# jayleicn/ClipBERT

Hardware: AMD Instinct MI355X
Metric: clips/sec/node (2×2 frames, 224px, L_txt=32) at 1/2/4/8 MI355X (higher is better)
Workload: dtype bf16; 1 GPU; MSRVTT retrieval training step (msrvtt_ret_base_resnet50.json; BASELINE configs[1]/[2] family) at the metric's shape: 16 videos x N_clip=2 x N_frame=2 uint8 frames 224px + 2 texts/video (pos+neg, r=2) L_txt=32 per GPU = 32 clips, 64 frames, 64 (text, clip) pairs per step; ImageNorm + fwd + lse-pooling loss + bwd + all-reduce + clip + AdamW in the timed step; clips folded into one forward; mode=train, videos_per_gpu=16, n_clips=2, n_frames=2, img_size=224, txt_len=32, texts_per_video=2, pairs_per_gpu=64, score_agg_func=lse, clips_folded=True, input=uint8 frames in HBM, parallelism=dp1, hip_graph=True, replay_plan=eager hyper-parameter upload + one hipGraph, n_graphs=1, dropout=True

## Files before the change

clipbert_amd/_lib.py:

```python
import ctypes as C
import os

HERE = os.path.dirname(os.path.abspath(__file__))
LIB_PATH = os.path.join(HERE, "lib", "libclipbert_hip.so")

CB_F32, CB_BF16 = 0, 1
ACT_NONE, ACT_RELU, ACT_GELU, ACT_TANH = 0, 1, 2, 3
SPLITK_WS_COUNTER_BYTES = 65536
ACT_GELU_SAVE_GRAD, ACT_SAVED_GRAD = 4, 5
ROWK, ROWK_GATHER, KROW, KROW_TAPS, KROW_GATHER = 0, 1, 2, 3, 4
(HP_LR, HP_BETA1, HP_BETA2, HP_EPS, HP_WD, HP_BC1, HP_BC2, HP_MAX_NORM, HP_GRAD_SCALE, HP_SKIP, HP_COUNT) = range(11)
OPT_ADAMW, OPT_ADAM, OPT_ADAMAX = 0, 1, 2

vp, i32, i64, f32, u64 = C.c_void_p, C.c_int32, C.c_int64, C.c_float, C.c_uint64


class GemmDesc(C.Structure):
    _fields_ = [
        ("dtype", i32), ("M", i32), ("N", i32), ("K", i32), ("a_mode", i32), ("b_mode", i32),
        ("A", vp), ("B", vp), ("lda", i64), ("ldb", i64), ("a_tab", vp), ("b_tab", vp),
        ("R", i32), ("S", i32), ("Cin", i32), ("H", i32), ("W", i32),
        ("sH", i64), ("sW", i64), ("flip_taps", i32), ("schedule", i32),
        ("C", vp), ("ldc", i64), ("c_rowmap", vp), ("c_f32", i32), ("accumulate", i32),
        ("split_k", i32), ("act", i32), ("scale", vp), ("shift", vp), ("residual", vp), ("ldr", i64),
        ("relu_after", i32), ("zero_fill_pitch", i32), ("mask", vp), ("ldm", i64), ("C2", vp), ("ldc2", i64),
        ("alpha", f32), ("dropout_p", f32), ("dropout_seed", u64), ("dropout_seed_ptr", vp), ("tile", i32),
        ("xcd_order", i32), ("a_bytes", i64), ("b_bytes", i64), ("gelu_grad_pre", vp), ("ld_gelu", i64), ("a_rowsum", vp),
        ("batch", i32), ("relu_bwd", i32), ("batch_stride_a", i64), ("batch_stride_b", i64), ("batch_stride_c", i64),
        ("batch_stride_rowsum", i64), ("post_scale", vp), ("post_scale2", vp), ("splitk_ws", vp), ("splitk_ws_bytes", i64),
        ("sq_slots", vp), ("sq_slots_n", i64),
    ]


class Res2Desc(C.Structure):
    _fields_ = [("x", vp), ("out", vp), ("w1", vp), ("w2", vp), ("w3", vp), ("wsc", vp),
                ("scale1", vp), ("shift1", vp), ("scale2", vp), ("shift2", vp), ("scale3", vp), ("shift3", vp),
                ("scale_sc", vp), ("shift_sc", vp), ("N", i32), ("H", i32), ("W", i32), ("cin", i32)]


_SIGNATURES = {
    "cb_gemm": [C.POINTER(GemmDesc), vp],
    "cb_res2_block": [C.POINTER(Res2Desc), vp],
    "cb_stem_pool": [vp, vp, vp, vp, vp, i32, i32, i32, i32, i32, i32, i32, vp],
    "cb_stem_pool_u8": [vp, vp, vp, vp, vp, vp, vp, i32, i32, i32, i32, i32, i32, i32, vp],
    "cb_gemm_plan": [vp, i32, vp],
    "cb_gemm_group": [vp, i32, vp],
    "cb_gemm_workspace_bytes": [vp, vp],
    "cb_build_pixel_table": [vp, i32, i32, i32, i32, i32, i64, i64, i64, vp],
    "cb_stem_pack": [i32, vp, i32, vp, vp, vp, i32, i32, i32, i32, i32, i32, vp],
    "cb_resize_pack_u8": [i32, vp, i64, vp, vp, i32, i32, vp, vp, vp, i32, i32, i32, i32, vp],
    "cb_image_norm": [vp, vp, vp, vp, i64, i64, vp],
    "cb_maxpool_fwd": [i32, vp, vp, i32, i32, i32, i32, i32, i32, i32, i32, i32, i32, vp],
    "cb_maxpool2_bwd": [i32, vp, vp, vp, vp, i32, i32, i32, i32, i32, i32, i32, vp],
    "cb_relu_scale_bwd": [i32, vp, vp, vp, vp, vp, vp, vp, i64, i32, vp],
    "cb_layernorm_fwd": [i32, vp, vp, vp, vp, vp, vp, i64, i32, f32, i32, i32, i32, vp],
    "cb_layernorm_bwd": [i32, vp, vp, vp, vp, vp, vp, vp, vp, i64, i32, vp, f32, u64, vp, i32, i32, i32, vp],
    "cb_layernorm_bwd_part": [i32, vp, vp, vp, vp, vp, vp, vp, i32, i64, i32, vp, f32, u64, vp, i32, i32, i32, vp],
    "cb_ln_partials_reduce": [vp, vp, vp, vp, i32, i32, i32, vp],
    "cb_comm_unique_id": [vp],
    "cb_comm_init": [i32, i32, vp],
    "cb_comm_info": [vp, vp],
    "cb_allreduce_bucket": [vp, i64, i32, vp],
    "cb_reduce_scatter_bucket": [vp, vp, i64, i32, vp],
    "cb_allgather_bucket": [vp, vp, i64, i32, vp],
    "cb_broadcast_bucket": [vp, i64, i32, i32, vp],
    "cb_comm_destroy": [],
    "cb_text_embed_fwd": [i32, vp, vp, vp, vp, vp, vp, vp, vp, vp, vp, i32, i32, i32, i32, f32, vp, vp, i32, vp],
    "cb_visual_embed_fwd": [i32, vp, vp, vp, vp, vp, vp, vp, vp, vp, vp, vp, vp, i32, i32, i32, i32, i32,
                            i32, i32, i32, f32, vp, vp],
    "cb_text_embed_bwd": [i32, vp, vp, vp, vp, vp, i32, i32, i32, i32, i64, i32, vp],
    "cb_head_loss": [i32, vp, vp, vp, vp, vp, i64, i32, f32, vp],
    "cb_retrieval_scores": [vp, vp, i64, i32, vp],
    "cb_sq_sum_fold": [vp, vp, i32, vp, i64, vp, vp, i32, vp],
    "cb_mean_fwd": [vp, i64, vp, vp],
    "cb_mean_bwd": [vp, i64, vp, vp],
    "cb_counter_add": [vp, i64, vp],
    "cb_zero": [vp, i64, vp],
    "cb_zero_ranges": [vp, vp, i32, vp],
    "cb_visual_embed_bwd": [i32, vp, vp, vp, vp, vp, vp, vp, i32, i32, i32, i32, i32, i32, i32, i32, vp],
    "cb_attention_fwd": [i32, vp, vp, vp, vp, i32, i32, i32, f32, u64, vp, vp],
    "cb_attention_bwd": [i32, vp, vp, vp, vp, vp, vp, vp, i32, i32, i32, f32, u64, vp, vp],
    "cb_cross_entropy": [vp, i64, vp, vp, vp, vp, i64, i32, i64, vp],
    "cb_colsum": [i32, vp, i64, vp, i64, i32, vp],
    "cb_cast": [i32, vp, i32, vp, i64, vp],
    "cb_act_bwd": [i32, i32, vp, vp, vp, i64, vp],
    "cb_adamw": [vp, vp, vp, vp, vp, i64, vp, vp, vp],
    "cb_dropout": [i32, vp, vp, i64, f32, u64, vp, vp],
    "cb_clip_aggregate_fwd": [vp, i32, i64, i32, vp, vp, vp],
    "cb_clip_aggregate_bwd": [vp, vp, vp, vp, i32, i64, i32, vp, vp],
    "cb_lse_loss": [vp, vp, i32, i32, i32, vp, vp, vp, vp],
    "cb_sq_sum": [vp, i64, vp, vp],
    "cb_sq_sum_det": [vp, i64, vp, vp, i32, vp],
    "cb_sq_sum_det_bf16": [vp, i64, vp, vp, i32, vp],
    "cb_adamw_g16": [vp, vp, vp, vp, vp, i64, vp, vp, vp],
    "cb_optim_step": [i32, i32, vp, vp, vp, vp, vp, i64, vp, vp, vp],
    "cb_elu_bn1d_fwd": [i32, vp, vp, vp, vp, vp, vp, vp, vp, i32, i32, i32, f32, f32, vp],
    "cb_elu_bn1d_bwd": [i32, vp, vp, vp, vp, vp, vp, vp, vp, i32, i32, i32, vp],
}

EXPORTED_SYMBOLS = tuple(_SIGNATURES) + ("cb_last_error", "cb_version")


def bind(cdll, strict: bool = True):
    for name, args in _SIGNATURES.items():
        if not strict and not hasattr(cdll, name):
            continue
        fn = getattr(cdll, name)
        fn.argtypes = args
        fn.restype = C.c_int
    cdll.cb_last_error.argtypes = []
    cdll.cb_last_error.restype = C.c_char_p
    cdll.cb_version.argtypes = []
    cdll.cb_version.restype = C.c_int
    return cdll


_LIB = None


def load(path: str = LIB_PATH):
    if not os.path.exists(path):
        raise RuntimeError(
            f"{path} not found: the HIP library is required (no fallback path exists). "
            "Build it with `python -m clipbert_amd.build`.")
    import torch
    return bind(C.CDLL(path))


# ... 13 lines not shown
```

clipbert_amd/csrc/common.hip:

```cpp
#include "common.h"

#include <stdarg.h>
#include <stdio.h>

namespace {
thread_local char g_err[512] = "";
}

int cb_fail(const char* fmt, ...) {
    va_list ap;
    va_start(ap, fmt);
    vsnprintf(g_err, sizeof(g_err), fmt, ap);
    va_end(ap);
    return -1;
}

int cb_launch_status(const char* what) {
    hipError_t e = hipGetLastError();
    if (e != hipSuccess) return cb_fail("%s: kernel launch failed: %s", what, hipGetErrorString(e));
    return 0;
}

extern "C" const char* cb_last_error(void) { return g_err; }
extern "C" int cb_version(void) { return 9; }
```

clipbert_amd/csrc/gemm.hip:

```cpp

#include "gemm8_impl.h"
#include "gemm_stream_impl.h"
#include <stdio.h>
#include <vector>

using namespace cbgemm;

namespace cbgemm {
extern template int launch_gemm<float, 64, 64, 2>(const GP&, bool, hipStream_t);
extern template int launch_gemm<bf16, 128, 128, 2>(const GP&, bool, hipStream_t);
extern template int launch_gemm<bf16, 128, 64, 2>(const GP&, bool, hipStream_t);
extern template int launch_gemm<bf16, 64, 64, 3>(const GP&, bool, hipStream_t);
extern template int launch_gemm<bf16, 128, 128, 1, 2>(const GP&, bool, hipStream_t);
extern template int launch_gemm_group<float, 64, 64, 2, 1>(const GroupArgs&, int, hipStream_t);
extern template int launch_gemm_group<bf16, 64, 64, 3, 1>(const GroupArgs&, int, hipStream_t);
extern template int launch_gemm_group<bf16, 128, 128, 1, 2>(const GroupArgs&, int, hipStream_t);
#define CB_G8_DECL(BM, BN, WGM, WGN, NST)                                                             \
    extern template int launch_gemm8_fwd<BM, BN, WGM, WGN, NST>(const GP&, int, float*, hipStream_t);   \
    extern template int launch_gemm8_dgrad<BM, BN, WGM, WGN, NST>(const GP&, int, float*, hipStream_t); \
    extern template int launch_gemm8_wgrad<BM, BN, WGM, WGN, NST>(const GP&, int, float*, hipStream_t);
CB_G8_DECL(256, 256, 2, 4, 2)
CB_G8_DECL(128, 256, 2, 4, 3)
CB_G8_DECL(256, 128, 4, 2, 3)
#undef CB_G8_DECL
int launch_gemm_skinny(const cb_gemm_desc* d, GP& p, hipStream_t st);
}

#include "gemm_choose.h"

#ifdef CB_STAMPS
#include <string>
namespace {
struct StampState {
    unsigned long long* buf = nullptr;
    int64_t areas = 0;
    std::vector<std::string> desc;
} g_stamps;
void stamp_assign(GP& p, const cb_gemm_desc* d, int tile, int split, int sched, int group_i, int group_n) {
    p.stamps = nullptr;
    if (!g_stamps.buf || (int64_t)g_stamps.desc.size() >= g_stamps.areas) return;
    p.stamps = g_stamps.buf + (int64_t)g_stamps.desc.size() * cbgemm::CB_STAMP_AREA;
    char line[512];
    snprintf(line, sizeof line,
             "{\"M\":%d,\"N\":%d,\"K\":%d,\"a_mode\":%d,\"b_mode\":%d,\"batch\":%d,\"tile\":%d,\"split\":%d,\"sched\":%d,\"taps\":%d,"
             "\"act\":%d,\"c2\":%d,\"residual\":%d,\"dropout\":%d,\"mask\":%d,\"gelu_grad\":%d,\"relu_bwd\":%d,\"c_f32\":%d,\"group_i\":%d,\"group_n\":%d}",
             d->M, d->N, d->K, d->a_mode, d->b_mode, d->batch > 1 ? d->batch : 1, tile, split, sched, (d->R > 0 ? d->R : 1) * (d->S > 0 ? d->S : 1), d->act,
             d->C2 != nullptr, d->residual != nullptr, d->dropout_p > 0.f, d->mask != nullptr, d->gelu_grad_pre != nullptr, d->relu_bwd != 0, d->c_f32, group_i, group_n);
    g_stamps.desc.push_back(line);
}
}
extern "C" int cb_debug_stamps_begin(void* buf, int64_t bytes) {
    g_stamps.buf = reinterpret_cast<unsigned long long*>(buf);
    g_stamps.areas = buf ? bytes / (8 * (int64_t)cbgemm::CB_STAMP_AREA) : 0;
    g_stamps.desc.clear();
    return 0;
}
extern "C" int64_t cb_debug_stamps_area_words() { return cbgemm::CB_STAMP_AREA; }
extern "C" int64_t cb_debug_stamps_count() { return (int64_t)g_stamps.desc.size(); }
extern "C" int cb_debug_stamps_desc(int64_t i, char* out, int64_t cap) {
    if (i < 0 || i >= (int64_t)g_stamps.desc.size() || cap <= 0) return -1;
    snprintf(out, (size_t)cap, "%s", g_stamps.desc[(size_t)i].c_str());
    return 0;
}
#define CB_STAMP_ASSIGN(p, d, tile, split, sched, gi, gn) stamp_assign(p, d, tile, split, sched, gi, gn)
#else
#define CB_STAMP_ASSIGN(p, d, tile, split, sched, gi, gn) do {} while (0)
#endif

namespace {

__global__ void __launch_bounds__(256) pixel_table_kernel(cb_pixel* tab, int total, int OH, int OW, int stride,
                                                          int pad, int64_t sN, int64_t sH, int64_t sW) {
    int m = blockIdx.x * 256 + threadIdx.x;
    if (m >= total) return;
    int ow = m % OW, t = m / OW;
    int oh = t % OH, n = t / OH;
    int ih0 = oh * stride - pad, iw0 = ow * stride - pad;
    cb_pixel px;
    px.off = (int32_t)((int64_t)n * sN + (int64_t)ih0 * sH + (int64_t)iw0 * sW);
    px.ih0 = (int16_t)ih0;
    px.iw0 = (int16_t)iw0;
    tab[m] = px;
}

__global__ void __launch_bounds__(256) splitk_reduce_kernel(GP p, const float* ws, int S) {
    using T = bf16;
    const int cpr = p.N >> 3;
    const int64_t total = (int64_t)p.M * cpr;
    const int64_t idx = (int64_t)blockIdx.x * 256 + threadIdx.x;
    if (p.batch > 1) {
        const int b = blockIdx.y;
        p.C = reinterpret_cast<unsigned char*>(p.C) + b * p.bs_c;
        ws += (int64_t)b * S * p.M * p.N;
    }
    if (idx >= total) return;
    if (p.dropout_p > 0.f && p.seed_ptr) p.seed += *p.seed_ptr;
    const int m = (int)(idx / cpr), n = (int)(idx - (int64_t)m * cpr) * 8;
    float v[8], t[8], sc[8], sh[8];
    const float* src = ws + (int64_t)m * p.N + n;
    load8(src, v);
    for (int s = 1; s < S; ++s) {
        load8(src + (int64_t)s * p.M * p.N, t);
#pragma unroll
        for (int r = 0; r < 8; ++r) v[r] += t[r];
    }
    if (p.scale) load8(p.scale + n, sc);
    if (p.shift) load8(p.shift + n, sh);
    const int64_t orow = p.c_rowmap ? (int64_t)p.c_rowmap[m] : (int64_t)m;
    epilogue8<T>(p, v, sc, sh, m, orow, n);
}

template <int BM, int BN, int WGM, int WGN, int NST>
int launch8(int form, const GP& p, int mode, float* ws, hipStream_t st) {
    if (form == 1) return launch_gemm8_fwd<BM, BN, WGM, WGN, NST>(p, mode, ws, st);
    if (form == 2) return launch_gemm8_dgrad<BM, BN, WGM, WGN, NST>(p, mode, ws, st);
    return launch_gemm8_wgrad<BM, BN, WGM, WGN, NST>(p, mode, ws, st);
}

int gemm_prepare(const cb_gemm_desc* d, Prepared& out) {
    CB_REQUIRE(d != nullptr, "cb_gemm: null descriptor");
    CB_REQUIRE(d->dtype == CB_F32 || d->dtype == CB_BF16, "cb_gemm: bad dtype %d", d->dtype);
    CB_REQUIRE(d->M >= 0 && d->N >= 0 && d->K >= 0, "cb_gemm: negative dims");
    CB_REQUIRE(d->A && d->B && d->C, "cb_gemm: null operand");
    const int esz = d->dtype == CB_BF16 ? 2 : 4;
    const int eps = 16 / esz;
    GP& p = out.p;
    p = GP{};
    p.A = d->A; p.B = d->B; p.C = d->C; p.C2 = d->C2; p.residual = d->residual; p.mask = d->mask;
    p.dact_pre = d->gelu_grad_pre; p.ldd = d->ld_gelu; p.a_rowsum = d->a_rowsum;
    p.relu_bwd = d->relu_bwd != 0; p.post_scale = d->post_scale; p.post_scale2 = d->post_scale2;
    if (p.relu_bwd) {
        CB_REQUIRE(d->mask && (!d->c_f32 || d->dtype == CB_F32) && !d->scale && !d->shift && d->act == CB_ACT_NONE && d->dropout_p <= 0.f && !d->relu_after &&
                   !d->gelu_grad_pre && (d->split_k <= 1),
                   "cb_gemm: relu_bwd needs a mask and excludes scale/shift/act/dropout/relu_after/gelu_grad_pre/split_k and an fp32 C next to bf16 operands");
        CB_REQUIRE((!d->post_scale || aligned16(d->post_scale)) && (!d->post_scale2 || aligned16(d->post_scale2)),
                   "cb_gemm: post_scale vectors must be 16-byte aligned");
    } else {
        CB_REQUIRE(!d->post_scale && !d->post_scale2, "cb_gemm: post_scale / post_scale2 need relu_bwd");
    }
    p.batch = d->batch > 1 ? d->batch : 1;
    p.bs_a = d->batch_stride_a * esz; p.bs_b = d->batch_stride_b * esz;
    p.bs_c = d->batch_stride_c * (d->c_f32 ? 4 : esz); p.bs_r = d->batch_stride_rowsum;
    if (p.batch > 1) {
        CB_REQUIRE(!d->C2 && !d->residual && !d->mask && !d->gelu_grad_pre && !d->a_tab && !d->b_tab && !d->c_rowmap,
                   "cb_gemm: batch > 1 supports plain operands only (no residual / mask / second output / gather / row map)");
        CB_REQUIRE((d->batch_stride_a * esz) % 16 == 0 && (d->batch_stride_b * esz) % 16 == 0 && (p.bs_c % 16) == 0,
                   "cb_gemm: batch strides must keep 16-byte alignment");
    }
    CB_REQUIRE(!d->a_rowsum || (d->a_mode == CB_KROW && d->b_mode == CB_KROW), "cb_gemm: a_rowsum needs the weight-gradient form (A and B both CB_KROW)");
    p.scale = d->scale; p.shift = d->shift; p.a_tab = d->a_tab; p.b_tab = d->b_tab; p.c_rowmap = d->c_rowmap; p.zfill = d->zero_fill_pitch;
    p.lda = d->lda; p.ldb = d->ldb; p.ldc = d->ldc; p.ldc2 = d->ldc2; p.ldr = d->ldr; p.ldm = d->ldm;
    p.sH = d->sH; p.sW = d->sW;
    p.M = d->M; p.N = d->N; p.K = d->K;
    p.a_mode = d->a_mode; p.b_mode = d->b_mode;
    p.R = d->R > 0 ? d->R : 1; p.S = d->S > 0 ? d->S : 1; p.Ct = d->Cin; p.H = d->H; p.W = d->W; p.flip = d->flip_taps;
    CB_REQUIRE(d->accumulate >= 0 && d->accumulate <= 2 && (d->accumulate != 2 || d->dtype == CB_BF16), "cb_gemm: bad accumulate %d (2 = first writer: bf16 problems)", d->accumulate);
    p.c_f32 = d->c_f32; p.accumulate = d->accumulate == 1; p.split_k = d->split_k > 0 ? d->split_k : 1;
    p.act = d->act; p.relu_after = d->relu_after;
    p.alpha = d->alpha == 0.f ? 1.f : d->alpha;
    p.dropout_p = d->dropout_p; p.seed = d->dropout_seed; p.seed_ptr = d->dropout_seed_ptr;
    const int bk = d->dtype == CB_BF16 ? Tr<bf16>::BK : Tr<float>::BK;
    p.ktiles = (d->K + bk - 1) / bk;
    {
        const bool ok = d->dtype == CB_BF16 && !d->c_f32 && (int64_t)d->M * (d->ldc > d->ldc2 ? d->ldc : d->ldc2) * 2 * (p.batch) < 0xffffffffll && !d->c_rowmap;
        p.wt = ok ? switches().wt : 0;
    }
    {
        const bool fe_off = switches().fast_epi_off;
        p.fast_epi = 0;
        auto rows_ok = [&](const void* q, int64_t ld) { return q == nullptr || (ld % 8 == 0 && aligned16(q) && (int64_t)d->M * ld * 2 < 0x7fffffffll); };
        const bool wg_store = !fe_off && d->dtype == CB_BF16 && d->c_f32 && d->a_mode == CB_KROW && d->accumulate != 1 && p.alpha == 1.f && !d->scale && !d->shift &&
                              d->act == CB_ACT_NONE && !d->C2 && !d->residual && !d->mask && !d->gelu_grad_pre && d->dropout_p <= 0.f && !d->relu_after && !d->c_rowmap &&
                              !d->zero_fill_pitch && !d->relu_bwd && d->N % 8 == 0 && d->ldc % 8 == 0 && aligned16(d->C) && (int64_t)d->M * d->ldc * 4 < 0xffffffffll;
        if (wg_store) p.fast_epi = FAST_EPI_F32;
        p.sq_slots = nullptr;
        if (d->sq_slots) {
            const int64_t need = (int64_t)((d->M + 63) / 64) * ((d->N + 63) / 64) * p.batch;
            CB_REQUIRE(wg_store, "cb_gemm: sq_slots needs a bf16 weight-gradient form storing an aligned fp32 C with a plain epilogue (accumulate 0 / 2)");
            CB_REQUIRE(d->sq_slots_n >= need, "cb_gemm: sq_slots_n %lld < %lld (one slot per 64x64 tile and batch member)", (long long)d->sq_slots_n, (long long)need);
            p.sq_slots = d->sq_slots;
        }
        const bool plain = !wg_store && !fe_off && p.wt == 1 && p.batch == 1 && d->accumulate != 1 && p.alpha == 1.f && !d->zero_fill_pitch && !d->a_rowsum &&
                           d->N % 8 == 0 && d->ldc % 8 == 0 && aligned16(d->C) && (!d->shift || aligned16(d->shift)) && (!d->scale || aligned16(d->scale)) &&
                           rows_ok(d->residual, d->ldr) && rows_ok(d->mask, d->ldm) && rows_ok(d->gelu_grad_pre, d->ld_gelu) &&
                           !(d->mask && d->gelu_grad_pre);
        if (plain && d->relu_bwd) {
            const bool ok = d->C2 && d->post_scale && d->ldc2 % 8 == 0 && aligned16(d->C2) && (int64_t)d->M * d->ldc2 * 2 < 0xffffffffll;
            const int flags = EF_RBWD | (d->residual ? EF_RES : 0) | (d->post_scale2 ? EF_PS2 : 0);
            if (ok)
                for (int i = 1; i < FAST_EPI_N; ++i)
                    if (FAST_EPI_COMBOS[i] == flags) { p.fast_epi = i; break; }
        } else if (plain) {
            int flags = 0;
            bool ok = true;
            if (d->scale) flags |= EF_SCALE;
            if (d->shift) flags |= EF_SHIFT;
            if (d->act == CB_ACT_RELU) flags |= EF_RELU;
            else if (d->act == CB_ACT_GELU_SAVE_GRAD && d->C2) flags |= EF_GELU2;
            else if (d->act == CB_ACT_GELU && !d->C2) flags |= EF_GELU1;
            else if (d->act == CB_ACT_SAVED_GRAD && d->gelu_grad_pre) flags |= EF_MULAUX;
            else if (d->act != CB_ACT_NONE) ok = false;
            if (d->C2 && !(flags & EF_GELU2)) ok = false;
            if (d->C2) ok = ok && d->ldc2 % 8 == 0 && aligned16(d->C2) && (int64_t)d->M * d->ldc2 * 2 < 0xffffffffll;
            if (d->gelu_grad_pre && !(flags & EF_MULAUX)) ok = false;
            if (d->dropout_p > 0.f) flags |= EF_DROP;
            if (d->residual) flags |= EF_RES;
            if (d->relu_after) flags |= EF_RELU_AFTER;
            if (d->mask) flags |= EF_MASK;
            if (ok)
                for (int i = 1; i < FAST_EPI_N; ++i)
                    if (FAST_EPI_COMBOS[i] == flags) { p.fast_epi = i; break; }
        }
    }
    const bool a_krow = d->a_mode == CB_KROW;
    const bool b_krow = d->b_mode == CB_KROW || d->b_mode == CB_KROW_TAPS || d->b_mode == CB_KROW_GATHER;
    CB_REQUIRE(d->a_mode == CB_ROWK || d->a_mode == CB_ROWK_GATHER || d->a_mode == CB_KROW, "cb_gemm: bad a_mode %d", d->a_mode);
    CB_REQUIRE(d->b_mode == CB_ROWK || b_krow, "cb_gemm: bad b_mode %d", d->b_mode);
    const int taps = p.R * p.S;
    const bool tapped = d->a_mode == CB_ROWK_GATHER || d->b_mode == CB_KROW_TAPS || d->b_mode == CB_KROW_GATHER;
    if (tapped) {
        CB_REQUIRE(p.Ct > 0, "cb_gemm: Cin (channels per tap) must be set for conv modes");
        CB_REQUIRE(p.Ct % eps == 0, "cb_gemm: channels per tap (%d) must be a multiple of %d", p.Ct, eps);
    }
    const int64_t lim = 0x7fffffffll;
    bool fast = d->a_bytes > 0 && d->b_bytes > 0 && d->a_bytes < lim && d->b_bytes < lim && aligned16(d->A) && aligned16(d->B);
    if (d->a_mode == CB_ROWK_GATHER) {
        CB_REQUIRE(d->a_tab, "cb_gemm: a_tab missing");
        CB_REQUIRE(d->K == taps * p.Ct, "cb_gemm: K (%d) != R*S*Cin (%d)", d->K, taps * p.Ct);
        fast = fast && (p.R == 1 || d->sH % eps == 0) && (p.S == 1 || d->sW % eps == 0);
    } else if (d->a_mode == CB_ROWK) {
        fast = fast && (d->lda % eps == 0) && (d->K % eps == 0);
    } else {
        const int64_t need = ((int64_t)(d->K - 1) * d->lda + (d->M + eps - 1) / eps * eps) * esz;
        fast = fast && (d->lda % eps == 0) && (d->M % eps == 0 || need <= d->a_bytes);
    }
    if (d->b_mode == CB_ROWK) {
        fast = fast && (d->ldb % eps == 0) && (d->K % eps == 0);
    } else if (d->b_mode == CB_KROW) {
        const int64_t need = ((int64_t)(d->K - 1) * d->ldb + (d->N + eps - 1) / eps * eps) * esz;
        fast = fast && (d->ldb % eps == 0) && (d->N % eps == 0 || need <= d->b_bytes);
    } else if (d->b_mode == CB_KROW_TAPS) {
        CB_REQUIRE(d->K == taps * p.Ct, "cb_gemm: K (%d) != R*S*Ct (%d)", d->K, taps * p.Ct);
        fast = fast && (d->ldb % eps == 0) && (d->N % eps == 0);
    } else {
        CB_REQUIRE(d->b_tab, "cb_gemm: b_tab missing");
        CB_REQUIRE(d->N == taps * p.Ct, "cb_gemm: N (%d) != R*S*Cin (%d)", d->N, taps * p.Ct);
        fast = fast && (p.R == 1 || d->sH % eps == 0) && (p.S == 1 || d->sW % eps == 0);
    }
    p.a_bytes = (uint32_t)(fast ? d->a_bytes : 0);
    p.b_bytes = (uint32_t)(fast ? d->b_bytes : 0);
    CB_REQUIRE(d->tile >= 0 && d->tile <= 9, "cb_gemm: bad tile %d", d->tile);
    CB_REQUIRE(d->xcd_order >= 0 && d->xcd_order <= 2, "cb_gemm: bad xcd_order %d", d->xcd_order);
    CB_REQUIRE(d->dropout_p >= 0.f && d->dropout_p < 1.f, "cb_gemm: dropout_p out of range");
    const int cesz = d->c_f32 ? 4 : esz;
    bool cv = (d->ldc % 4 == 0) && ((reinterpret_cast<uintptr_t>(d->C) % (4 * cesz)) == 0);
    if (d->C2) cv = cv && (d->ldc2 % 4 == 0) && ((reinterpret_cast<uintptr_t>(d->C2) % (4 * esz)) == 0);
    if (d->residual) cv = cv && (d->ldr % 4 == 0) && ((reinterpret_cast<uintptr_t>(d->residual) % (4 * esz)) == 0);
    if (d->mask) cv = cv && (d->ldm % 4 == 0) && ((reinterpret_cast<uintptr_t>(d->mask) % (4 * esz)) == 0);
    if (d->gelu_grad_pre) cv = cv && (d->ld_gelu % 4 == 0) && ((reinterpret_cast<uintptr_t>(d->gelu_grad_pre) % (4 * esz)) == 0);
    if (d->scale) cv = cv && aligned16(d->scale);
    if (d->shift) cv = cv && aligned16(d->shift);
    p.c_vec = cv;
    bool cv8 = cv && (d->N % 8 == 0) && (d->ldc % 8 == 0) && aligned16(d->C);
    if (d->C2) cv8 = cv8 && (d->ldc2 % 8 == 0) && aligned16(d->C2);
    if (d->residual) cv8 = cv8 && (d->ldr % 8 == 0) && aligned16(d->residual);
    if (d->mask) cv8 = cv8 && (d->ldm % 8 == 0) && aligned16(d->mask);
    if (d->gelu_grad_pre) cv8 = cv8 && (d->ld_gelu % 8 == 0) && aligned16(d->gelu_grad_pre);
    out.fast = fast; out.cv8 = cv8;
    out.form = operand_form(d->a_mode, d->b_mode, taps); out.taps = taps;
    out.epi_scale_only = !d->C2 && !d->residual && !d->mask && !d->gelu_grad_pre && d->act == CB_ACT_NONE && !d->relu_after && !d->shift && d->dropout_p <= 0.f;
    out.atomics_ok = out.epi_scale_only && d->c_f32 && d->accumulate == 1;
    return 0;
}

int gemm_validate(const cb_gemm_desc* d, Prepared& pr, bool& empty) {
    empty = false;
    CB_REQUIRE(d != nullptr, "cb_gemm: null descriptor");
    CB_REQUIRE(d->M >= 0 && d->N >= 0 && d->K >= 0, "cb_gemm: negative dims");
    empty = d->M == 0 || d->N == 0;
    return empty ? 0 : gemm_prepare(d, pr);
}

void trace_plan(const cb_gemm_desc* d, const Prepared& pr, const LaunchPlan& lp) {
    if (lp.tile == 9)
        fprintf(stderr, "cb_gemm: M=%d N=%d K=%d modes=%d/%d tile=9 (asked %d) few rows\n", d->M, d->N, d->K, d->a_mode, d->b_mode, d->tile);
    else if (lp.tile == 8)
        fprintf(stderr, "cb_gemm: M=%d N=%d K=%d modes=%d/%d tile=8 (asked %d) stream variant %d\n", d->M, d->N, d->K, d->a_mode, d->b_mode, d->tile, lp.sched);
    else
        fprintf(stderr, "cb_gemm: M=%d N=%d K=%d modes=%d/%d tile=%d (asked %d) form8=%d split=%d ws=%d\n", d->M, d->N, d->K, d->a_mode, d->b_mode,
                lp.picked, d->tile, lp.form8, lp.tile >= 5 ? lp.split_k : pr.p.split_k, (int)lp.slab);
}

int gemm_launch(const cb_gemm_desc* d, const Prepared& pr, const LaunchPlan& lp, hipStream_t st) {
    GP p = pr.p;
    if (lp.tile == 9) return launch_gemm_skinny(d, p, st);
    p.split_k = lp.split_k;
    p.c_vec8 = lp.c_vec8;
    p.xcd_remap = lp.xcd_remap;
    if (lp.tile == 8) return launch_gemm_stream(p, lp.sched, st);
    if (lp.tile >= 5) {
        float* ws = lp.slab ? reinterpret_cast<float*>(d->splitk_ws) : nullptr;
        CB_STAMP_ASSIGN(p, d, lp.tile, p.split_k, lp.sched, 0, 1);
        int rc;
        if (lp.tile == 5) rc = launch8<256, 256, 2, 4, 2>(lp.form8, p, lp.sched - 1, ws, st);
        else if (lp.tile == 6) rc = launch8<128, 256, 2, 4, 3>(lp.form8, p, lp.sched - 1, ws, st);
        else rc = launch8<256, 128, 4, 2, 3>(lp.form8, p, lp.sched - 1, ws, st);
        if (rc != 0 || !ws) return rc;
        GP q = p;
        q.split_k = 1;
        const int64_t chunks = (int64_t)d->M * (d->N / 8);
        hipLaunchKernelGGL(splitk_reduce_kernel, dim3((unsigned)((chunks + 255) / 256), (unsigned)p.batch), dim3(256), 0, st, q, ws, p.split_k);
        return cb_launch_status("cb_gemm (split-K reduce)");
    }
    if (d->dtype == CB_F32) return launch_gemm<float, 64, 64, 2>(p, pr.fast, st);
    CB_STAMP_ASSIGN(p, d, lp.tile, p.split_k, 0, 0, 1);
    if (lp.tile == 4) return launch_gemm<bf16, 128, 128, 1, 2>(p, pr.fast, st);
    if (lp.tile == 1) return launch_gemm<bf16, 128, 128, 2>(p, pr.fast, st);
    if (lp.tile == 3) return launch_gemm<bf16, 128, 64, 2>(p, pr.fast, st);
    return launch_gemm<bf16, 64, 64, 3>(p, pr.fast, st);
}

int gemm_run(const cb_gemm_desc* d, const Prepared& pr, void* stream) {
    LaunchPlan lp;
    const int rc = gemm_choose(d, pr, true, false, lp);
    if (lp.tile != 0 && switches().trace) trace_plan(d, pr, lp);
    return rc != 0 ? rc : gemm_launch(d, pr, lp, cb_stream(stream));
}
}

extern "C" int cb_gemm(const cb_gemm_desc* d, void* stream) {
    Prepared pr;
    bool empty;
    if (int rc = gemm_validate(d, pr, empty)) return rc;
    return empty ? 0 : gemm_run(d, pr, stream);
}

extern "C" int cb_gemm_plan(const cb_gemm_desc* d, int32_t use_table, int32_t* out4) {
    CB_REQUIRE(out4 != nullptr, "cb_gemm_plan: null output");
    out4[0] = out4[1] = out4[2] = out4[3] = 0;
    Prepared pr;
    LaunchPlan lp;
    bool empty;
    if (int rc = gemm_validate(d, pr, empty)) return rc;
    if (empty) return 0;
    if (int rc = gemm_choose(d, pr, use_table != 0, false, lp)) return rc;
    out4[0] = lp.tile; out4[1] = lp.split_k; out4[2] = lp.sched; out4[3] = lp.xcd_remap ? 1 : 2;
    return 0;
}

extern "C" int cb_gemm_workspace_bytes(const cb_gemm_desc* d, int64_t* bytes) {
    CB_REQUIRE(d != nullptr && bytes != nullptr, "cb_gemm_workspace_bytes: null argument");
    *bytes = 0;
    Prepared pr;
    LaunchPlan lp;
    bool empty;
    if (int rc = gemm_validate(d, pr, empty)) return rc;
    if (empty) return 0;
    if (int rc = gemm_choose(d, pr, true, true, lp)) return rc;
    if (lp.slab) *bytes = (int64_t)lp.split_k * pr.p.batch * d->M * d->N * 4 + CB_SPLITK_WS_COUNTER_BYTES;
    return 0;
}

namespace {
int group_class(const cb_gemm_desc* d, const Prepared& pr) {
    if (!pr.fast || d->zero_fill_pitch || d->tile >= 5 || d->tile == 1 || d->tile == 3) return -1;
    if (d->batch > 1 || d->a_rowsum) {
        const bool ok = d->dtype == CB_BF16 && pr.form == FORM_WGRAD && d->split_k <= 1 && d->tile != 2 && !d->c_rowmap;
        return ok ? GC_WGRAD_RS : -1;
    }
    return GROUP_CLASS_OF[pr.form];
}

struct GroupItem { const cb_gemm_desc* d; Prepared pr; int cls; };

bool group_split_free(const GroupItem& it) { return a_reduction_major(it.pr.form) && it.d->c_f32 && it.d->accumulate != 0 && it.pr.epi_scale_only; }
inline int64_t group_tiles(const cb_gemm_desc* d, int B) { return (int64_t)((d->M + B - 1) / B) * ((d->N + B - 1) / B); }

double group_cost(const std::vector<GroupItem*>& g, int tile, int s, int* splits) {
    const int B = tile == 4 ? 128 : 64;
    int maxkt = 1;
    for (auto* it : g) maxkt = it->pr.p.ktiles > maxkt ? it->pr.p.ktiles : maxkt;
    const int kt_target = (maxkt + s - 1) / s;
    int64_t W = 0;
    int kt_per_max = 1;
    double atom = 0.0;
    for (size_t i = 0; i < g.size(); ++i) {
        const cb_gemm_desc* d = g[i]->d;
        const int kt = g[i]->pr.p.ktiles;
        int si = g[i]->pr.p.split_k;
        if (group_split_free(*g[i])) {
            si = (kt + kt_target / 2) / kt_target;
            if (si < 1) si = 1;
            while (si > 1 && kt / si < 4) --si;
        }
        if (si > kt) si = kt > 0 ? kt : 1;
        splits[i] = si;
        W += group_tiles(d, B) * si;
        const int per = (kt + si - 1) / si;
        kt_per_max = per > kt_per_max ? per : kt_per_max;
        if (si > 1) atom += (double)d->M * d->N * 4.0 * si;
    }
    static const int cus = [] {
        int dev = 0, n = 0;
        return (hipGetDevice(&dev) == hipSuccess && hipDeviceGetAttribute(&n, hipDeviceAttributeMultiprocessorCount, dev) == hipSuccess && n > 0) ? n : 256;
    }();
    const int64_t per_cu = (W + cus - 1) / cus;
    double unit;
    if (tile == 4) unit = per_cu <= 1 ? 1.0 : 0.77;
    else unit = per_cu <= 1 ? 0.45 : (per_cu == 2 ? 0.35 : 0.30);
    return 8.0 + (double)per_cu * kt_per_max * unit + atom / 2.0e6;
}

struct GroupPlan {
    int tile = 2;
    int splits[GROUP_MAX];
    float* slab = nullptr;
    int* cnt = nullptr;
};
void group_choose(const std::vector<GroupItem*>& g, int dtype, int cls, GroupPlan& gp) {
    int* splits = gp.splits;
    auto callers_splits = [&] { for (size_t i = 0; i < g.size(); ++i) splits[i] = g[i]->pr.p.split_k; };
    if (dtype == CB_F32) {
        callers_splits();
    } else {
        const int asked = g[0]->d->tile;
        if (cls == GC_WGRAD_RS) {
            gp.tile = 4;
            for (size_t i = 0; i < g.size(); ++i) splits[i] = 1;
        } else if (asked == 2 || asked == 4) {
            gp.tile = asked;
            callers_splits();
        } else {
            static const int SPLITS[] = {1, 2, 3, 4, 6, 8, 12, 16, 24, 32};
            bool narrow = false, any_free = false;
            for (auto* it : g) { narrow = narrow || it->d->N <= 64; any_free = any_free || group_split_free(*it); }
            double best = 1e300;
            int tmp[GROUP_MAX];
            for (int t : {2, 4}) {
                if (t == 4 && narrow) continue;
                for (int s : SPLITS) {
                    if (s > 1 && !any_free) break;
                    const double c = group_cost(g, t, s, tmp);
                    if (c < best) { best = c; gp.tile = t; for (size_t i = 0; i < g.size(); ++i) splits[i] = tmp[i]; }
                }
            }
        }
    }
    if (dtype == CB_BF16 && !switches().group_slab_off && (cls == GC_WGRAD || cls == GC_WGRAD_GATHER)) {
// ... 125 lines not shown
```

clipbert_amd/csrc/gemm_choose.h:

```cpp
#pragma once
#include "gemm_impl.h"
#include <cmath>
#include "gemm_tuned.h"
#include "gemm_model.h"

namespace cbgemm {
bool skinny_covers(const cb_gemm_desc* d, const GP& p);
}
using namespace cbgemm;

namespace {
inline int env_int(const char* name, int dflt) { const char* v = getenv(name); return v != nullptr ? atoi(v) : dflt; }
struct Switches {
    bool trace = getenv("CB_GEMM_TRACE") != nullptr;
    bool no_tuned = getenv("CB_GEMM_NO_TUNED") != nullptr;
    bool no_model = getenv("CB_GEMM_NO_MODEL") != nullptr;
    bool no_xcd_remap = getenv("CB_GEMM_NO_XCD_REMAP") != nullptr;
    bool no_stream = getenv("CB_GEMM_NO_STREAM") != nullptr;
    bool no_group = getenv("CB_GEMM_NO_GROUP") != nullptr;
    bool no_skinny = getenv("CB_GEMM_NO_SKINNY") != nullptr;
    bool group_slab_off = env_int("CB_GROUP_SLAB", 1) == 0;
    bool fast_epi_off = env_int("CB_GEMM_FAST_EPI", 1) == 0;
    int wt = env_int("CB_GEMM_WT", 1);
};
inline const Switches& switches() { static const Switches s; return s; }

enum Form {
    FORM_FWD = 0,
    FORM_FWD_GATHER,
    FORM_DGRAD,
    FORM_DGRAD_TAPS,
    FORM_DGRAD_OTHER,
    FORM_WGRAD,
    FORM_WGRAD_GATHER,
    FORM_WGRAD_OTHER
};
Form operand_form(int a_mode, int b_mode, int taps) {
    if (a_mode == CB_KROW) return b_mode == CB_KROW ? FORM_WGRAD : (b_mode == CB_KROW_GATHER ? FORM_WGRAD_GATHER : FORM_WGRAD_OTHER);
    if (b_mode == CB_ROWK) return a_mode == CB_ROWK ? FORM_FWD : FORM_FWD_GATHER;
    if (a_mode == CB_ROWK && (b_mode == CB_KROW || (b_mode == CB_KROW_TAPS && taps == 1))) return FORM_DGRAD;
    if (a_mode == CB_ROWK_GATHER && b_mode == CB_KROW_TAPS) return FORM_DGRAD_TAPS;
    return FORM_DGRAD_OTHER;
}
inline bool a_reduction_major(Form f) { return f >= FORM_WGRAD; }
inline int model_form(Form f) { return f >= FORM_WGRAD ? 2 : (f >= FORM_DGRAD ? 1 : 0); }
const int FORM8_OF[8] = {1, 1, 2, 2, 0, 3, 3, 0};
const int GROUP_CLASS_OF[8] = {GC_FWD, GC_FWD_GATHER, -1, -1, -1, GC_WGRAD, GC_WGRAD_GATHER, -1};

struct Prepared {
    GP p;
    bool fast, cv8;
    Form form;
    int taps;
    bool epi_scale_only;
    bool atomics_ok;
};
constexpr int GROUP_COUNTERS = CB_SPLITK_WS_COUNTER_BYTES / (int)sizeof(int);
inline int64_t splitk_payload_bytes(int64_t ws_bytes) { return ws_bytes > CB_SPLITK_WS_COUNTER_BYTES ? ws_bytes - CB_SPLITK_WS_COUNTER_BYTES : 0; }
inline int* splitk_counters(void* ws, int64_t ws_bytes) {
    return ws && ws_bytes > CB_SPLITK_WS_COUNTER_BYTES ? reinterpret_cast<int*>(reinterpret_cast<unsigned char*>(ws) + (ws_bytes - CB_SPLITK_WS_COUNTER_BYTES)) : nullptr;
}

struct ModelPick { int tile = 0, split = 0, sched = 0; double us = 1e300; };
const int MODEL_TILE_ID[7] = {2, 3, 1, 4, 5, 6, 7};
const int MODEL_BM[7] = {64, 128, 128, 128, 256, 128, 256};
const int MODEL_BN[7] = {64, 64, 128, 128, 256, 256, 128};

double model_us(int ti, int form, int64_t M, int64_t N, int64_t K, int64_t batch, int s, bool taps, bool m2, int c_esz) {
    using namespace cbgemm;
    const double* g = MODEL_G;
    const int64_t wg = ((M + MODEL_BM[ti] - 1) / MODEL_BM[ti]) * ((N + MODEL_BN[ti] - 1) / MODEL_BN[ti]) * batch * s;
    const int64_t kt = ((K + 63) / 64 + s - 1) / s;
    const double r = (double)wg / (256.0 * MODEL_OCC[ti]);
    const double q = ti >= 4 ? g[7] : g[3];
    const double rounds = q * std::ceil(r - 1e-9) + (1.0 - q) * (r > 1.0 ? r : 1.0);
    const double ck = MODEL_C[ti][form] * (1.0 + g[4] * (taps ? 1 : 0)) * (1.0 + g[8] * (m2 ? 1 : 0));
    const double ab = (double)(M * K + N * K) * 2.0 * batch, cb = (double)M * N * batch * c_esz;
    const double red = (ti >= 4 && s > 1) ? (double)M * N * batch * s * 8.0 : 0.0;
    const double atom = (ti < 4 && s > 1) ? (double)M * N * batch * s * 4.0 : 0.0;
    return MODEL_A[ti] + rounds * (MODEL_B[ti][form] + kt * ck) + ab / (g[0] * 1e6) + cb / (g[5] * 1e6) + red / (g[1] * 1e6) + atom / (g[2] * 1e6) +
           g[6] * (m2 ? 1 : 0);
}

ModelPick model_pick(const cb_gemm_desc* d, const Prepared& pr, bool can8, int64_t ws_bytes, bool free_split) {
    const GP& p = pr.p;
    const int form = model_form(pr.form), split_caller = p.split_k;
    const bool taps = pr.taps > 1;
    const int c_esz = d->c_f32 ? 4 : 2;
    const int64_t M = d->M, N = d->N, K = d->K, batch = p.batch;
    ModelPick best;
    auto consider = [&](int ti, int s, int sched) {
        const double us = model_us(ti, form, M, N, K, batch, s, taps, sched == 3, c_esz);
        if (us < best.us) { best.us = us; best.tile = MODEL_TILE_ID[ti]; best.split = s; best.sched = sched; }
    };
    static const int SPLITS4[] = {1, 2, 3, 4, 6, 8, 12, 16, 24, 32, 48};
    for (int ti = 0; ti < 4; ++ti) {
        if (N <= 64 && ti >= 2) continue;
        consider(ti, split_caller, 0);
        if (free_split)
            for (int s : SPLITS4)
                if (s != split_caller && s <= (p.ktiles / 4 > 1 ? p.ktiles / 4 : 1)) consider(ti, s, 0);
    }
    if (can8)
        for (int ti = 4; ti < 7; ++ti) {
            const int64_t tiles = ((M + MODEL_BM[ti] - 1) / MODEL_BM[ti]) * ((N + MODEL_BN[ti] - 1) / MODEL_BN[ti]) * batch;
            int cand[3] = {1, 0, 0};
            int n = 1;
            for (int target : {256, 512}) {
                const int s = (int)std::lround((double)target / (double)tiles);
                if (s > 1 && p.ktiles / s >= 2 && (int64_t)s * batch * M * N * 4 <= ws_bytes && s != cand[1]) cand[n++] = s;
            }
            for (int i = 0; i < n; ++i) { consider(ti, cand[i], 1); consider(ti, cand[i], 3); }
        }
    return best;
}

int stream_variant(const cb_gemm_desc* d, const Prepared& pr) {
    const GP& p = pr.p;
    if (!pr.fast || !pr.cv8 || d->dtype != CB_BF16 || pr.form != FORM_FWD || p.batch > 1 || p.split_k > 1) return -1;
    if (d->c_f32 || d->accumulate || d->c_rowmap || d->zero_fill_pitch || d->a_rowsum || d->gelu_grad_pre || d->dropout_p > 0.f || d->mask || d->relu_bwd ||
        d->C2) return -1;
    if (d->K % 8 != 0 || d->M < 64) return -1;
    if ((int64_t)d->M * (d->N > d->K ? d->N : d->K) * 2 >= 0x7fffffffll) return -1;
    if (p.ktiles == 1 && d->N % 256 == 0) return 0;
    if (p.ktiles == 2 && d->N % 128 == 0) return 1;
    return -1;
}

struct LaunchPlan {
    int tile = 0;
    int split_k = 1;
    int sched = 0;
    bool xcd_remap = false;
    bool slab = false;
    bool c_vec8 = false;
    int form8 = 0;
    int picked = 0;
};
struct Pick { int tile = 0, split = 0, sched = 0; };
constexpr int64_t WS_UNLIMITED = (int64_t)1 << 60;
constexpr int STREAM_MIN_ROWS = 32768;

int gemm_choose(const cb_gemm_desc* d, const Prepared& pr, bool use_table, bool assume_ws, LaunchPlan& lp) {
    const Switches& sw = switches();
    const GP& p = pr.p;
    const bool bf = d->dtype == CB_BF16, explicit_tile = d->tile != 0;
    const int split_caller = p.split_k;
    lp = LaunchPlan{};
    const bool covers9 = skinny_covers(d, p);
    CB_REQUIRE(d->tile != 9 || covers9, "cb_gemm: tile 9 (few rows) does not cover this problem (bf16, A k-contiguous, B k-contiguous or aligned reduction-major, no batch / K split / row sums)");
    if (d->tile == 9 || (!explicit_tile && use_table && !sw.no_skinny && covers9 && d->M <= 64)) { lp.tile = 9; return 0; }
    const int sv = stream_variant(d, pr);
    CB_REQUIRE(d->tile != 8 || sv >= 0, "cb_gemm: tile 8 (streaming) does not cover this problem (M=%d N=%d K=%d modes %d/%d)", d->M, d->N, d->K, d->a_mode, d->b_mode);
    const cbgemm::TunedEntry* tabled =
        (bf && use_table && !sw.no_tuned) ? cbgemm::tuned_lookup(d->a_mode, d->b_mode, d->M, d->N, d->K, p.batch, pr.taps, split_caller) : nullptr;
    if (d->tile == 8 || (!explicit_tile && use_table && !sw.no_stream && !tabled && sv >= 0 && d->M >= STREAM_MIN_ROWS && d->N <= 512)) {
        lp.tile = 8; lp.sched = sv; lp.c_vec8 = true;
        return 0;
    }

    const int form8 = (bf && pr.fast && pr.cv8 && (pr.form != FORM_DGRAD_TAPS || p.Ct % 64 == 0)) ? FORM8_OF[pr.form] : 0;
    const int64_t ws_room = assume_ws ? splitk_payload_bytes(WS_UNLIMITED)
                                      : (d->splitk_ws && aligned16(d->splitk_ws) ? splitk_payload_bytes(d->splitk_ws_bytes) : 0);
    const bool free_split = !explicit_tile && a_reduction_major(pr.form) && pr.atomics_ok;
    const int xcd = d->xcd_order != 0 ? d->xcd_order : (tabled ? tabled->xcd : 0);
    auto model = [&](bool allow8) {
        Pick k;
        if (!bf || sw.no_model) return k;
        const ModelPick mp = model_pick(d, pr, allow8 && form8 != 0, ws_room, free_split && !d->a_rowsum && p.batch == 1);
        k.tile = mp.tile; k.split = (mp.tile >= 5 || mp.split != split_caller) ? mp.split : 0; k.sched = mp.sched;
        return k;
    };
    auto split8 = [&](const Pick& k) { return explicit_tile ? split_caller : (k.split > 0 ? k.split : 1); };
    Pick pick;
    if (explicit_tile) pick.tile = d->tile;
    else if (tabled) pick = Pick{tabled->tile, tabled->new_split, tabled->sched};
    if (pick.tile >= 5 && form8 == 0) pick = Pick{};
    if (pick.tile == 0) pick = model(true);
    if (pick.tile >= 5 && d->sq_slots && split8(pick) > 1) pick = model(false);
    if (pick.tile >= 5) {
        int split = split8(pick);
        if (split > p.ktiles) split = p.ktiles;
        if (split > 1) {
            const int per = (p.ktiles + split - 1) / split;
            split = (p.ktiles + per - 1) / per;
            if ((int64_t)split * p.batch * d->M * d->N * 4 > ws_room) {
                pick = model(!explicit_tile);
                split = pick.split > 0 ? pick.split : 1;
            }
        }
        if (pick.tile >= 5) {
            lp.tile = lp.picked = pick.tile; lp.form8 = form8;
            lp.split_k = split; lp.slab = split > 1;
            lp.sched = d->schedule > 0 ? d->schedule : (pick.sched > 0 ? pick.sched : 3);
            lp.c_vec8 = true;
            lp.xcd_remap = !sw.no_xcd_remap && xcd != 2;
            CB_REQUIRE(d->schedule >= 0 && d->schedule <= 3, "cb_gemm: bad schedule %d", d->schedule);
            return 0;
        }
    }

    lp.picked = pick.tile; lp.form8 = form8;
    lp.tile = pick.tile == 0 ? 2 : pick.tile;
    if (!bf) lp.tile = 2;
    else if ((lp.tile == 1 || lp.tile == 4) && d->N <= 64) lp.tile = 3;
    lp.xcd_remap = !sw.no_xcd_remap && xcd != 2;
    int split = split_caller;
    if (d->tile >= 5 && split > 1 && !pr.atomics_ok) split = 1;
    if (d->accumulate == 2 || d->sq_slots) split = 1;
    if (pick.split > 0 && free_split) split = pick.split;
    if (split > 1) {
        CB_REQUIRE(d->c_f32 && d->accumulate == 1, "cb_gemm: split_k > 1 needs an fp32 output that is accumulated into (accumulate = 1)");
        CB_REQUIRE(pr.epi_scale_only, "cb_gemm: split_k > 1 supports only scale/alpha in the epilogue");
        if (split > p.ktiles) split = p.ktiles;
    }
    lp.split_k = split;
    lp.c_vec8 = pr.cv8 && split == 1;
    if (d->zero_fill_pitch != 0)
        CB_REQUIRE(d->zero_fill_pitch > 0 && d->c_rowmap && lp.c_vec8 && d->batch <= 1,
                   "cb_gemm: zero_fill_pitch needs c_rowmap and 16-byte-aligned 8-column chunks (N, ldc %% 8 == 0)");
    return 0;
}
}
```

clipbert_amd/csrc/gemm_impl.h:

```cpp
#pragma once
#include "common.h"
#include <stdlib.h>
#include <type_traits>

namespace cbgemm {


constexpr int NTHREADS = 256;

template <typename T> struct Tr;
template <> struct Tr<bf16> { static constexpr int EPS = 8, BK = 64, SEGS = 8, ROWB = 128, RB = 8; };
template <> struct Tr<float> { static constexpr int EPS = 4, BK = 32, SEGS = 8, ROWB = 144, RB = 4; };

template <typename T> __device__ __forceinline__ int lds_off(int row, int seg);
template <> __device__ __forceinline__ int lds_off<bf16>(int row, int seg) { return row * 128 + ((seg ^ (row & 7)) << 4); }
template <> __device__ __forceinline__ int lds_off<float>(int row, int seg) { return row * 144 + (seg << 4); }

struct GP {
    const void* A; const void* B; void* C; void* C2; const void* residual; const void* mask;
    const void* dact_pre; float* a_rowsum; int64_t ldd;
    int relu_bwd; const float* post_scale; const float* post_scale2;
    int batch; int64_t bs_a, bs_b, bs_c, bs_r;
    const float* scale; const float* shift;
    const cb_pixel* a_tab; const cb_pixel* b_tab; const int32_t* c_rowmap;
    int64_t lda, ldb, ldc, ldc2, ldr, ldm, sH, sW;
    int M, N, K;
    int a_mode, b_mode;
    int R, S, Ct, H, W, flip;
    int c_f32, accumulate, split_k, act, relu_after;
    float alpha, dropout_p;
    uint64_t seed;
    const uint64_t* seed_ptr;
    short c_vec, c_vec8;
    short xcd_remap;
    short wt;
    int zfill;
    uint32_t a_bytes, b_bytes;
    int ktiles;
    int slab_base, cnt_base;
    int fast_epi;
    float* sq_slots;
#ifdef CB_STAMPS
    unsigned long long* stamps;
#endif
};

enum { EF_SCALE = 1, EF_SHIFT = 2, EF_RELU = 4, EF_GELU2 = 8, EF_DROP = 16, EF_RES = 32, EF_RELU_AFTER = 64, EF_MASK = 128, EF_MULAUX = 256,
       EF_RBWD = 512,
       EF_PS2 = 1024,
       EF_F32 = 2048,
       EF_GELU1 = 4096 };
constexpr int FAST_EPI_COMBOS[] = {
    -1,
    0,
    EF_SHIFT,
    EF_SHIFT | EF_GELU2,
    EF_SHIFT | EF_DROP | EF_RES,
    EF_SHIFT | EF_RES,
    EF_MULAUX,
    EF_RES,
    EF_SCALE | EF_SHIFT | EF_RELU,
    EF_SCALE | EF_SHIFT,
    EF_SCALE | EF_SHIFT | EF_RES | EF_RELU_AFTER,
    EF_SCALE | EF_MASK,
    EF_RBWD,
    EF_RBWD | EF_RES,
    EF_RBWD | EF_PS2,
    EF_RBWD | EF_PS2 | EF_RES,
    EF_F32,
    EF_SHIFT | EF_GELU1,
};
constexpr int FAST_EPI_F32 = 16;
constexpr int FAST_EPI_N = sizeof(FAST_EPI_COMBOS) / sizeof(int);

#ifdef CB_STAMPS
constexpr int CB_STAMP_WGS = 512, CB_STAMP_REC = 6, CB_STAMP_HDR = 3;
constexpr int CB_STAMP_AREA = CB_STAMP_HDR + CB_STAMP_WGS * CB_STAMP_REC;
struct Stamps {
    unsigned long long t[5];
    __device__ __forceinline__ void mark(int i) { t[i] = __builtin_amdgcn_s_memrealtime(); }
    __device__ __forceinline__ void flush(unsigned long long* area, unsigned lin, int tid) {
        if (!area || tid != 0) return;
        asm volatile("s_waitcnt vmcnt(0)" ::: "memory");
        const unsigned long long t4 = __builtin_amdgcn_s_memrealtime();
// ... 1234 lines not shown
                    const int64_t orow = p.c_rowmap ? (int64_t)p.c_rowmap[m] : (int64_t)m;
                    float v[8];
                    load8(reinterpret_cast<const float*>(smem + rl * SROW + cc * 32), v);
                    if constexpr (EPF == 2) {
                        if (use_pre) epilogue8<T, 2>(p, v, sc, sh, m, orow, n, rp, ap);
                        else epilogue8<T>(p, v, sc, sh, m, orow, n);
                    } else if constexpr (EPF == 1) {
                        if (use_pre) epilogue8<T, 1>(p, v, sc, sh, m, orow, n, bf16x8{}, ap);
                        else epilogue8<T>(p, v, sc, sh, m, orow, n);
                    } else epilogue8<T>(p, v, sc, sh, m, orow, n);
                }
            }
        }
    } else if (p.split_k > 1 && p.c_vec) {
        constexpr int SROW = BN * 4 + 16;
        static_assert(WM * SROW <= SMEM_BYTES, "staging does not fit");
        float* cbase = reinterpret_cast<float*>(p.C);
#pragma unroll
        for (int h = 0; h < 2; ++h) {
            __syncthreads();
            if (wm == h) {
#pragma unroll
                for (int i = 0; i < FM; ++i)
#pragma unroll
                    for (int j = 0; j < FN; ++j)
                        *reinterpret_cast<f32x4*>(smem + (i * 16 + (lane & 15)) * SROW + (wn * WN + j * 16 + 4 * (lane >> 4)) * 4) = acc[i][j];
            }
            __syncthreads();
#pragma unroll 4
            for (int idx = tid; idx < WM * BN; idx += NTHREADS) {
                const int rl = idx / BN, cl = idx % BN;
                const int m = m0 + h * WM + rl, n = n0 + cl;
                if (m < p.M && n < p.N) {
                    const int64_t orow = p.c_rowmap ? (int64_t)p.c_rowmap[m] : (int64_t)m;
                    float x = *reinterpret_cast<const float*>(smem + rl * SROW + cl * 4) * p.alpha;
                    if (p.scale) x *= p.scale[n];
#ifdef CB_EPI_NOATOMIC
                    cbase[orow * p.ldc + n] = x;
#else
                    atomicAdd(cbase + orow * p.ldc + n, x);
#endif
                }
            }
        }
    } else if (fast) {
#pragma unroll
        for (int i = 0; i < FM; ++i) {
            const int m = m0 + wm * WM + i * 16 + (lane & 15);
            const bool mok = m < p.M;
            const int64_t orow = (mok && p.c_rowmap) ? (int64_t)p.c_rowmap[m] : (int64_t)m;
#pragma unroll
            for (int j = 0; j < FN; ++j) {
                const int nb = n0 + wn * WN + j * 16 + 4 * (lane >> 4);
                if (mok) epilogue_vec<T>(p, acc[i][j], m, orow, nb);
            }
        }
    } else {
        float* stage = reinterpret_cast<float*>(smem);
        static_assert(WM * BN * 4 <= SMEM_BYTES, "staging does not fit");
#pragma unroll
        for (int h = 0; h < 2; ++h) {
            __syncthreads();
            if (wm == h) {
#pragma unroll
                for (int i = 0; i < FM; ++i)
#pragma unroll
                    for (int j = 0; j < FN; ++j)
                        *reinterpret_cast<f32x4*>(stage + (i * 16 + (lane & 15)) * BN + wn * WN + j * 16 + 4 * (lane >> 4)) = acc[i][j];
            }
            __syncthreads();
            for (int idx = tid; idx < WM * BN; idx += NTHREADS) {
                const int rl = idx / BN, cl = idx % BN;
                const int m = m0 + h * WM + rl, n = n0 + cl;
                if (m < p.M && n < p.N) {
                    const int64_t orow = p.c_rowmap ? (int64_t)p.c_rowmap[m] : (int64_t)m;
                    epilogue_elem<T>(p, stage[idx], m, orow, n);
                }
            }
        }
    }
}


template <typename T, int BM, int BN, typename LA, typename LB, int PF, bool RS, int OCC>
__device__ __forceinline__ void gemm_tile(GP& p, TileId bid, float* slab = nullptr, int* cnt = nullptr) {
    using X = Tr<T>;
    constexpr int BK = X::BK;
    constexpr int WM = BM / 2, WN = BN / 2, FM = WM / 16, FN = WN / 16;
    constexpr int TILE_A = BM * X::ROWB, TILE_B = BN * X::ROWB;
    constexpr int SMEM_BYTES = 2 * (TILE_A + TILE_B);
    __shared__ __attribute__((aligned(16))) unsigned char smem[SMEM_BYTES];

    const int tid = threadIdx.x, lane = tid & 63, wave = tid >> 6;
    const int wm = wave >> 1, wn = wave & 1;
    CB_STAMP_DECL();
    CB_STAMP(0);
#ifdef CB_STAMPS
    const unsigned stamp_lin = (unsigned)bid.bx + (unsigned)((p.N + BN - 1) / BN) * ((unsigned)bid.by + (unsigned)((p.M + BM - 1) / BM) * (unsigned)bid.bz);
#endif
    const int tile_lin = ((p.batch > 1 ? bid.bz / p.split_k : 0) * ((p.M + BM - 1) / BM) + bid.by) * ((p.N + BN - 1) / BN) + bid.bx;
    apply_batch(p, bid);
    const int m0 = bid.by * BM, n0 = bid.bx * BN;
    const int kt_per = (p.ktiles + p.split_k - 1) / p.split_k;
    const int kt0 = bid.bz * kt_per;
    const int nt = ((kt0 + kt_per < p.ktiles) ? kt0 + kt_per : p.ktiles) - kt0;
    if (nt <= 0) return;

    LA la;
    LB lb;
    {
        Opnd oa = {p.A, p.a_tab, p.lda, p.a_mode, p.a_bytes};
        Opnd ob = {p.B, p.b_tab, p.ldb, p.b_mode, p.b_bytes};
        la.init(p, oa, m0, p.M, kt0, tid);
        lb.init(p, ob, n0, p.N, kt0, tid);
    }
    typename LA::Stage sa[PF];
    typename LB::Stage sb[PF];

    auto load_tiles = [&](typename LA::Stage& xa, typename LB::Stage& xb) {
        la.template load<false>(xa, p);
        lb.template load<false>(xb, p);
    };
    auto load_tiles_checked = [&](typename LA::Stage& xa, typename LB::Stage& xb) {
        la.template load<true>(xa, p);
        lb.template load<true>(xb, p);
    };
    auto store_tiles = [&](const typename LA::Stage& xa, const typename LB::Stage& xb, int buf) {
        unsigned char* As = smem + buf * (TILE_A + TILE_B);
        la.store(xa, As, tid);
        lb.store(xb, As + TILE_A, tid);
    };

    f32x4 acc[FM][FN];
#pragma unroll
    for (int i = 0; i < FM; ++i)
#pragma unroll
        for (int j = 0; j < FN; ++j) { f32x4 z = {0.f, 0.f, 0.f, 0.f}; acc[i][j] = z; }
    f32x4 accr[RS ? FM : 1];
#pragma unroll
    for (int i = 0; i < (RS ? FM : 1); ++i) { f32x4 z = {0.f, 0.f, 0.f, 0.f}; accr[i] = z; }
    const bool rs_on = RS && p.a_rowsum != nullptr && bid.bx == 0 && wn == 0;

#pragma unroll
    for (int s = 0; s < PF; ++s)
        if (s < nt) load_tiles_checked(sa[s], sb[s]);
    constexpr bool DGRAD = sizeof(T) == 2 && !LA::KROW && LB::KROW;
    constexpr int EPF = !DGRAD ? 0 : (BM * BN <= 128 * 64 ? 2 : (OCC >= 2 ? 1 : 0));
    EpiPre<BM, BN, EPF != 1> epre;
    const bool epf_on = EPF != 0 && p.c_vec8 && (EPF == 2 ? p.relu_bwd != 0 : (p.dact_pre != nullptr && !p.relu_bwd));
    if constexpr (EPF != 0) {
        if (epf_on) epi_prefetch<T, BM, BN, EPF != 1>(p, epre, m0, n0, tid);
    }
    store_tiles(sa[0], sb[0], 0);
    if (PF < nt) load_tiles_checked(sa[0], sb[0]);
    __syncthreads();
    CB_STAMP(1);

    auto compute_tile = [&](int buf) {
        const unsigned char* As = smem + buf * (TILE_A + TILE_B);
        const unsigned char* Bs = As + TILE_A;
        if constexpr (sizeof(T) == 2) {
#pragma unroll
            for (int kk = 0; kk < BK / 32; ++kk) {
                bf16x8 af[FM], bfr[FN];
#pragma unroll
                for (int i = 0; i < FM; ++i) {
                    if constexpr (LA::TR) af[i] = tr_frag<BM>(As, wm * WM + i * 16, kk, lane);
                    else af[i] = *reinterpret_cast<const bf16x8*>(As + lds_off<T>(wm * WM + i * 16 + (lane & 15), kk * 4 + (lane >> 4)));
// ... 49 lines not shown
        for (int s = 0; s < PF; ++s) {
            const int S1 = (s + 1) % PF;
            compute_tile(t & 1);
            store_tiles(sa[S1], sb[S1], (t + 1) & 1);
            load_tiles(sa[S1], sb[S1]);
            __syncthreads();
            ++t;
        }
    }
    while (t < nt) {
#pragma unroll
        for (int s = 0; s < PF; ++s) {
            if (t < nt) {
                const int S1 = (s + 1) % PF;
                compute_tile(t & 1);
                if (t + 1 < nt) {
                    store_tiles(sa[S1], sb[S1], (t + 1) & 1);
                    if (t + 1 + PF < nt) load_tiles_checked(sa[S1], sb[S1]);
                }
                __syncthreads();
                ++t;
            }
        }
    }

    if constexpr (RS) {
        if (rs_on && (lane >> 4) == 0) {
#pragma unroll
            for (int i = 0; i < FM; ++i) {
                const int m = m0 + wm * WM + i * 16 + lane;
                if (m < p.M) atomicAdd(p.a_rowsum + m, accr[i][0]);
            }
        }
    }
    CB_STAMP(2);
    if (slab != nullptr && p.split_k > 1) {
        __shared__ int s_last;
        constexpr int SC1 = 16;
        const int tile_lin = bid.by * ((p.N + BN - 1) / BN) + bid.bx;
        const int parts = (p.ktiles + kt_per - 1) / kt_per;
        float* const base = slab + ((int64_t)p.slab_base + (int64_t)tile_lin * p.split_k) * (BM * BN);
        {
            const rsrc_t rs = __builtin_amdgcn_make_buffer_rsrc(base + (int64_t)bid.bz * (BM * BN), (short)0, BM * BN * 4, 0x00020000);
#pragma unroll
            for (int i = 0; i < BM / 32; ++i)
#pragma unroll
                for (int j = 0; j < BN / 32; ++j) {
                    union { f32x4 f; u32x4 r; } u;
                    u.f = acc[i][j];
                    __builtin_amdgcn_raw_buffer_store_b128(u.r, rs, (uint32_t)(((i * (BN / 32) + j) * NTHREADS + tid) * 16), 0, SC1);
                }
        }
        __builtin_amdgcn_s_waitcnt(0x0f70);
        __syncthreads();
        if (tid == 0) s_last = atomicAdd(cnt + p.cnt_base + tile_lin, 1) == parts - 1;
        __syncthreads();
        if (!s_last) {
            CB_STAMP(3);
            CB_STAMP_FLUSH(p, stamp_lin, tid);
            return;
        }
#pragma unroll
        for (int i = 0; i < BM / 32; ++i)
#pragma unroll
            for (int j = 0; j < BN / 32; ++j) { f32x4 z = {0.f, 0.f, 0.f, 0.f}; acc[i][j] = z; }
#pragma unroll 2
        for (int z = 0; z < parts; ++z) {
            const rsrc_t rs = __builtin_amdgcn_make_buffer_rsrc(base + (int64_t)z * (BM * BN), (short)0, BM * BN * 4, 0x00020000);
#pragma unroll
            for (int i = 0; i < BM / 32; ++i)
#pragma unroll
                for (int j = 0; j < BN / 32; ++j) {
                    union { u32x4 r; f32x4 f; } u;
                    u.r = __builtin_amdgcn_raw_buffer_load_b128(rs, (uint32_t)(((i * (BN / 32) + j) * NTHREADS + tid) * 16), 0, SC1);
                    acc[i][j] += u.f;
                }
        }
        if (tid == 0) atomicExch(cnt + p.cnt_base + tile_lin, 0);
        p.split_k = 1;
    }
    constexpr int FORM_ = LA::KROW ? 0 : (LB::KROW ? 2 : 1);
    if constexpr (EPF != 0) tile_epilogue<T, BM, BN, SMEM_BYTES, EPF, false, FORM_>(p, acc, smem, m0, n0, tid, epre, epf_on);
    else tile_epilogue<T, BM, BN, SMEM_BYTES, 0, LA::KROW, FORM_>(p, acc, smem, m0, n0, tid, EpiPre<BM, BN, true>{}, false, tile_lin);
    CB_STAMP(3);
    CB_STAMP_FLUSH(p, stamp_lin, tid);
}

template <typename T, int BM, int BN, typename LA, typename LB, int PF, bool RS = false, int OCC = 1>
__global__ void __launch_bounds__(256, OCC) gemm_kernel(GP p) {
    gemm_tile<T, BM, BN, LA, LB, PF, RS, OCC>(p, tile_id(p));
}

#ifdef CB_STAMPS
constexpr int GROUP_MAX = 9;
#else
constexpr int GROUP_MAX = 10;
#endif
struct GroupArgs {
    int n, xcd_remap;
    int tile_end[GROUP_MAX];
    float* slab;
    int* cnt;
    GP g[GROUP_MAX];
};
static_assert(sizeof(GroupArgs) + 256 <= 4096, "kernel arguments (+ the hidden ones) are limited to 4 KiB");

template <int BM, int BN>
__device__ __forceinline__ int group_locate(const GroupArgs& ga, TileId& bid) {
    const unsigned total = gridDim.x;
    unsigned lin = blockIdx.x;
    if (ga.xcd_remap) {
        const unsigned xcd = lin & 7u, i = lin >> 3;
        const unsigned q = total >> 3, r = total & 7u;
        lin = (xcd < r ? xcd * (q + 1) : r * (q + 1) + (xcd - r) * q) + i;
    }
    int pi = 0;
    while (pi + 1 < ga.n && lin >= (unsigned)ga.tile_end[pi]) ++pi;
    const unsigned local = lin - (pi > 0 ? (unsigned)ga.tile_end[pi - 1] : 0u);
    const unsigned gx = (unsigned)((ga.g[pi].N + BN - 1) / BN), gy = (unsigned)((ga.g[pi].M + BM - 1) / BM);
    bid.bx = (int)(local % gx);
    const unsigned rest = local / gx;
    bid.by = (int)(rest % gy);
    bid.bz = (int)(rest / gy);
    return pi;
}

template <typename T, int BM, int BN, typename LA, typename LB, int PF, bool RS = false, int OCC = 1>
__global__ void __launch_bounds__(256, OCC) gemm_group_kernel(GroupArgs ga) {
    TileId bid;
    const int pi = group_locate<BM, BN>(ga, bid);
    GP p = ga.g[pi];
    gemm_tile<T, BM, BN, LA, LB, PF, RS, OCC>(p, bid, ga.slab, ga.cnt);
}

__device__ __forceinline__ void dma16(rsrc_t rs, unsigned char* lds_wave_base, uint32_t voff) {
    __builtin_amdgcn_raw_ptr_buffer_load_lds(rs, (__attribute__((address_space(3))) void*)lds_wave_base, 16, voff, 0, 0, 0);
}
#define CB_WAIT_VMCNT(N) __builtin_amdgcn_s_waitcnt((((N) & 15) | (7 << 4) | (15 << 8) | ((((N) >> 4) & 3) << 14)))

#define CB_LDS_BARRIER() do { asm volatile("" ::: "memory"); __builtin_amdgcn_s_waitcnt(0xc07f); __builtin_amdgcn_s_barrier(); asm volatile("" ::: "memory"); } while (0)

template <int ROWS, bool GATHER> struct RowkDma {
    using X = Tr<bf16>;
    static constexpr bool TR = false;
    static constexpr int NI = ROWS / 8 / 4;
    rsrc_t rs;
    uint32_t voff[NI];
    int ih[NI], iw[NI];
    int c, rr, ss, krem;

    __device__ __forceinline__ void init(const GP& p, const Opnd& o, int row0, int bound, int kt0, int tid) {
        rs = make_rsrc(o.base, o.bytes);
        const int lane = tid & 63, wave = tid >> 6;
        const int rin = lane >> 3;
        const int lseg = (lane & 7) ^ rin;
        const int k = kt0 * X::BK + lseg * 8;
        c = k; rr = 0; ss = 0; krem = p.K - k;
        if constexpr (GATHER) {
            int tap = k / p.Ct;
            c = k - tap * p.Ct;
            rr = tap / p.S; ss = tap - rr * p.S;
        }
#pragma unroll
        for (int i = 0; i < NI; ++i) {
            const int row = row0 + (i * 4 + wave) * 8 + rin;
            const bool ok = row < bound;
            ih[i] = 0; iw[i] = 0;
            if constexpr (GATHER) {
                cb_pixel px = {0, 0, 0};
                if (ok) px = o.tab[row];
                ih[i] = px.ih0; iw[i] = px.iw0;
                voff[i] = ok ? (uint32_t)px.off * 2u : OOB;
            } else {
// ... 2 lines not shown
        }
    }
    template <bool CHECK> __device__ __forceinline__ void issue(const GP& p, unsigned char* tile, int wave) {
        if constexpr (GATHER) {
            const bool kv = rr < p.R;
            const uint32_t koff = (uint32_t)(rr * (int)p.sH + ss * (int)p.sW + c) * 2u;
#pragma unroll
            for (int i = 0; i < NI; ++i) {
                const bool v = kv && (unsigned)(ih[i] + rr) < (unsigned)p.H && (unsigned)(iw[i] + ss) < (unsigned)p.W;
                dma16(rs, tile + (i * 4 + wave) * 1024, v ? voff[i] + koff : OOB);
            }
            if (p.Ct >= X::BK) {
                c += X::BK;
                if (c >= p.Ct) { c -= p.Ct; if (++ss == p.S) { ss = 0; ++rr; } }
            } else {
                ss += X::BK / p.Ct;
                while (ss >= p.S) { ss -= p.S; ++rr; }
            }
        } else {
#pragma unroll
            for (int i = 0; i < NI; ++i) {
                uint32_t o32 = voff[i];
                if (CHECK && krem <= 0) o32 = OOB;
                dma16(rs, tile + (i * 4 + wave) * 1024, o32);
                voff[i] += X::BK * 2u;
            }
            krem -= X::BK;
        }
    }
};

inline bool aligned16(const void* p) { return (reinterpret_cast<uintptr_t>(p) & 15) == 0; }

template <typename T, int BM, int BN, int PF, int OCC, typename LA, typename LB, bool RS = false>
int launch_k(const GP& p, hipStream_t st) {
    dim3 grid((p.N + BN - 1) / BN, (p.M + BM - 1) / BM, p.split_k * (p.batch > 1 ? p.batch : 1));
    hipLaunchKernelGGL((gemm_kernel<T, BM, BN, LA, LB, PF, RS, OCC>), grid, dim3(NTHREADS), 0, st, p);
    return cb_launch_status("cb_gemm");
}
template <typename T, int BM, int BN, int PF, int OCC, typename LA, typename LB>
int launch_wgrad(const GP& p, hipStream_t st) {
    if (p.a_rowsum) return launch_k<T, BM, BN, PF, OCC, LA, LB, true>(p, st);
    return launch_k<T, BM, BN, PF, OCC, LA, LB, false>(p, st);
}

template <typename T, int BM, int BN, int PF, int OCC = 1>
int launch_gemm(const GP& p, bool fast, hipStream_t st) {
    const bool a_krow = p.a_mode == CB_KROW;
    const bool b_krow = p.b_mode != CB_ROWK;
    if (a_krow && !b_krow) return cb_fail("cb_gemm: unsupported operand mode combination (A KROW with B ROWK)");
    if (fast) {
        const int taps = p.R * p.S;
        if constexpr (sizeof(T) == 2) {
            if constexpr (BN < 128) {
                if (p.a_mode == CB_ROWK && (p.b_mode == CB_KROW || (p.b_mode == CB_KROW_TAPS && taps == 1)))
                    return launch_k<T, BM, BN, PF, OCC, RowkFast<T, BM, false>, KrowTr<BN, KM_PLAIN>>(p, st);
                if (p.a_mode == CB_ROWK_GATHER && p.b_mode == CB_KROW_TAPS && p.Ct % Tr<bf16>::BK == 0)
                    return launch_k<T, BM, BN, PF, OCC, RowkFast<T, BM, true>, KrowTr<BN, KM_TAPS>>(p, st);
            }
            if (p.a_mode == CB_KROW && p.b_mode == CB_KROW)
                return launch_wgrad<T, BM, BN, PF, OCC, KrowTr<BM, KM_PLAIN>, KrowTr<BN, KM_PLAIN>>(p, st);
            if (p.a_mode == CB_KROW && p.b_mode == CB_KROW_GATHER)
                return launch_k<T, BM, BN, PF, OCC, KrowTr<BM, KM_PLAIN>, KrowTr<BN, KM_GATHER>>(p, st);
        }
        if (p.a_mode == CB_ROWK && p.b_mode == CB_ROWK)
            return launch_k<T, BM, BN, PF, OCC, RowkFast<T, BM, false>, RowkFast<T, BN, false>>(p, st);
        if (p.a_mode == CB_ROWK_GATHER && p.b_mode == CB_ROWK)
            return launch_k<T, BM, BN, PF, OCC, RowkFast<T, BM, true>, RowkFast<T, BN, false>>(p, st);
        constexpr int KB1B = BN >= 128 ? 4 : 2;
        constexpr int KB2A = BM >= 128 ? 8 : 4, KB2B = BN >= 128 ? 8 : 4;
        if (p.a_mode == CB_ROWK && (p.b_mode == CB_KROW || (p.b_mode == CB_KROW_TAPS && taps == 1)))
            return launch_k<T, BM, BN, PF, OCC, RowkFast<T, BM, false>, KrowFast<T, BN, KM_PLAIN, KB1B, 0>>(p, st);
        if (p.a_mode == CB_ROWK_GATHER && p.b_mode == CB_KROW_TAPS)
            return launch_k<T, BM, BN, PF, OCC, RowkFast<T, BM, true>, KrowFast<T, BN, KM_TAPS, KB1B, 0>>(p, st);
        if (p.a_mode == CB_KROW && p.b_mode == CB_KROW)
            return launch_wgrad<T, BM, BN, PF, OCC, KrowFast<T, BM, KM_PLAIN, KB2A, 0>, KrowFast<T, BN, KM_PLAIN, KB2B, 128>>(p, st);
        if (p.a_mode == CB_KROW && p.b_mode == CB_KROW_GATHER)
            return launch_k<T, BM, BN, PF, OCC, KrowFast<T, BM, KM_PLAIN, KB2A, 0>, KrowFast<T, BN, KM_GATHER, KB2B, 128>>(p, st);
    }
    if (!a_krow && !b_krow) return launch_k<T, BM, BN, PF, OCC, RowkLoader<T, BM, false>, RowkLoader<T, BN, false>>(p, st);
    if (!a_krow) return launch_k<T, BM, BN, PF, OCC, RowkLoader<T, BM, false>, KrowLoader<T, BN, false>>(p, st);
    if (p.b_mode == CB_KROW) return launch_wgrad<T, BM, BN, PF, OCC, KrowLoader<T, BM, false>, KrowLoader<T, BN, false>>(p, st);
    return launch_k<T, BM, BN, PF, OCC, KrowLoader<T, BM, false>, KrowLoader<T, BN, false>>(p, st);
}

enum { GC_WGRAD = 0,
       GC_WGRAD_GATHER = 1,
       GC_FWD = 2,
       GC_FWD_GATHER = 3,
       GC_WGRAD_RS = 4,
       GC_COUNT = 5 };

template <typename T, int BM, int BN, int PF, int OCC>
int launch_gemm_group(const GroupArgs& ga, int cls, hipStream_t st) {
    const dim3 grid((unsigned)ga.tile_end[ga.n - 1]);
    if constexpr (sizeof(T) == 2 && BM == 128 && BN == 128 && OCC == 2) {
        if (cls == GC_WGRAD_RS) {
            hipLaunchKernelGGL((gemm_group_kernel<T, BM, BN, KrowTr<BM, KM_PLAIN>, KrowTr<BN, KM_PLAIN>, PF, true, OCC>), grid, dim3(NTHREADS), 0, st, ga);
            return cb_launch_status("cb_gemm_group");
        }
    }
#define CB_LAUNCH_GROUP(LA_, LB_)                                                                                     \
    do {                                                                                                              \
        hipLaunchKernelGGL((gemm_group_kernel<T, BM, BN, LA_, LB_, PF, false, OCC>), grid, dim3(NTHREADS), 0, st, ga); \
        return cb_launch_status("cb_gemm_group");                                                                     \
    } while (0)
    using RA0 = RowkFast<T, BM, false>; using RA1 = RowkFast<T, BM, true>; using RB0 = RowkFast<T, BN, false>;
    if constexpr (sizeof(T) == 2) {
        using KA = KrowTr<BM, KM_PLAIN>; using KB0 = KrowTr<BN, KM_PLAIN>; using KB2 = KrowTr<BN, KM_GATHER>;
        if (cls == GC_WGRAD) CB_LAUNCH_GROUP(KA, KB0);
        if (cls == GC_WGRAD_GATHER) CB_LAUNCH_GROUP(KA, KB2);
    } else {
        constexpr int KB2A = BM >= 128 ? 8 : 4, KB2B = BN >= 128 ? 8 : 4;
        using KA = KrowFast<T, BM, KM_PLAIN, KB2A, 0>; using KB0 = KrowFast<T, BN, KM_PLAIN, KB2B, 128>; using KB2 = KrowFast<T, BN, KM_GATHER, KB2B, 128>;
        if (cls == GC_WGRAD) CB_LAUNCH_GROUP(KA, KB0);
        if (cls == GC_WGRAD_GATHER) CB_LAUNCH_GROUP(KA, KB2);
    }
    if (cls == GC_FWD) CB_LAUNCH_GROUP(RA0, RB0);
    if (cls == GC_FWD_GATHER) CB_LAUNCH_GROUP(RA1, RB0);
#undef CB_LAUNCH_GROUP
    return cb_fail("cb_gemm_group: unknown kernel class %d", cls);
}

}
```

clipbert_amd/csrc/gemm_inst_bf16_128x64.hip:

```cpp
#include "gemm_impl.h"

namespace cbgemm {
template int launch_gemm<bf16, 128, 64, 2>(const GP&, bool, hipStream_t);
}
```

clipbert_amd/csrc/gemm_inst_bf16_64x64.hip:

```cpp
#include "gemm_impl.h"

namespace cbgemm {
template int launch_gemm<bf16, 64, 64, 3>(const GP&, bool, hipStream_t);
template int launch_gemm_group<bf16, 64, 64, 3, 1>(const GroupArgs&, int, hipStream_t);
}
```

clipbert_amd/csrc/norm.hip:

```cpp
#include "common.h"

#include <stdlib.h>

namespace {

constexpr int MAXD = 2048;

template <int MAXCH, typename T>
__device__ __forceinline__ void load_row(const T* p, int D, int lane, f32x4 (&v)[MAXCH]) {
#pragma unroll
    for (int c = 0; c < MAXCH; ++c) {
        int e = (lane + 64 * c) * 4;
        f32x4 z = {0.f, 0.f, 0.f, 0.f};
        v[c] = (e < D) ? load4(p + e) : z;
    }
}

template <int MAXCH>
__device__ __forceinline__ void row_stats(const f32x4 (&v)[MAXCH], int D, int lane, float eps, float& mean, float& rstd) {
    float s = 0.f;
#pragma unroll
    for (int c = 0; c < MAXCH; ++c) s += v[c][0] + v[c][1] + v[c][2] + v[c][3];
    mean = wave_sum(s) / (float)D;
    float q = 0.f;
#pragma unroll
    for (int c = 0; c < MAXCH; ++c) {
        int e = (lane + 64 * c) * 4;
        if (e < D) {
#pragma unroll
            for (int i = 0; i < 4; ++i) { float d = v[c][i] - mean; q += d * d; }
        }
    }
    rstd = rsqrtf(wave_sum(q) / (float)D + eps);
}

template <int MAXCH, typename T>
__device__ __forceinline__ void norm_store(const f32x4 (&v)[MAXCH], const float* gamma, const float* beta, T* y, int D,
                                           int lane, float mean, float rstd) {
#pragma unroll
    for (int c = 0; c < MAXCH; ++c) {
        int e = (lane + 64 * c) * 4;
        if (e < D) {
            f32x4 g = load4(gamma + e), b = load4(beta + e), o;
#pragma unroll
            for (int i = 0; i < 4; ++i) o[i] = (v[c][i] - mean) * rstd * g[i] + b[i];
            store4(y + e, o);
        }
    }
}

template <typename T, int MAXCH, bool FULL = false>
__global__ void __launch_bounds__(256) layernorm_fwd_kernel(const T* x, const float* gamma, const float* beta, T* y,
                                                            float* mean_out, float* rstd_out, int64_t rows, int D, float eps,
                                                            int seg_len, int seg_stride, int seg_off) {
    const int lane = threadIdx.x & 63;
    int64_t row = (int64_t)blockIdx.x * 4 + (threadIdx.x >> 6);
    if (row >= rows) return;
    if (seg_len > 0) row = (row / seg_len) * seg_stride + seg_off + row % seg_len;
    f32x4 v[MAXCH];
    if constexpr (FULL) {
        f32x4 gm[MAXCH], bt[MAXCH];
        load_row(x + row * D, MAXCH * 256, lane, v);
#pragma unroll
        for (int c = 0; c < MAXCH; ++c) { gm[c] = load4(gamma + (lane + 64 * c) * 4); bt[c] = load4(beta + (lane + 64 * c) * 4); }
        float s = 0.f;
#pragma unroll
        for (int c = 0; c < MAXCH; ++c) s += v[c][0] + v[c][1] + v[c][2] + v[c][3];
        const float inv_d = 1.0f / (float)(MAXCH * 256);
        const float mean = wave_sum(s) * inv_d;
        float q = 0.f;
#pragma unroll
        for (int c = 0; c < MAXCH; ++c)
#pragma unroll
            for (int i = 0; i < 4; ++i) { const float d = v[c][i] - mean; q += d * d; }
        const float rstd = rsqrtf(wave_sum(q) * inv_d + eps);
#pragma unroll
        for (int c = 0; c < MAXCH; ++c) {
            f32x4 o;
#pragma unroll
            for (int i = 0; i < 4; ++i) o[i] = (v[c][i] - mean) * rstd * gm[c][i] + bt[c][i];
            store4(y + row * D + (lane + 64 * c) * 4, o);
        }
        if (lane == 0) {
            if (mean_out) mean_out[row] = mean;
            if (rstd_out) rstd_out[row] = rstd;
        }
        return;
    }
    load_row(x + row * D, D, lane, v);
    float mean, rstd;
    row_stats(v, D, lane, eps, mean, rstd);
    norm_store(v, gamma, beta, y + row * D, D, lane, mean, rstd);
    if (lane == 0) {
        if (mean_out) mean_out[row] = mean;
        if (rstd_out) rstd_out[row] = rstd;
    }
}

template <typename T, int MAXCH, int NW>
__global__ void __launch_bounds__(NW * 64) layernorm_bwd_kernel(const T* dy, const T* x, const float* gamma, const float* mean,
                                                               const float* rstd, T* dx, float* dgamma, float* dbeta,
                                                               int64_t rows, int D, T* dx2, float drop_p, uint64_t seed,
                                                               const uint64_t* seed_ptr, int seg_len, int seg_stride, int seg_off,
                                                               float* part) {
    __shared__ float red[2][NW][256];
    if (dx2 && seed_ptr) seed += *seed_ptr;
    const int lane = threadIdx.x & 63, wave = threadIdx.x >> 6;
    f32x4 ag[MAXCH], ab[MAXCH];
#pragma unroll
    for (int c = 0; c < MAXCH; ++c) { f32x4 z = {0.f, 0.f, 0.f, 0.f}; ag[c] = z; ab[c] = z; }
    const int64_t stride = (int64_t)gridDim.x * NW;
    auto phys = [&](int64_t lrow) { return seg_len > 0 ? (lrow / seg_len) * seg_stride + seg_off + lrow % seg_len : lrow; };
    int64_t lrow = (int64_t)blockIdx.x * NW + wave;
    f32x4 g[MAXCH], xv[MAXCH], gn[MAXCH], xn[MAXCH];
    float mu = 0.f, rs = 0.f, mun = 0.f, rsn = 0.f;
    int64_t row = 0, rown = 0;
    if (lrow < rows) {
        row = phys(lrow);
        load_row(dy + row * D, D, lane, g);
        load_row(x + row * D, D, lane, xv);
        mu = mean[row]; rs = rstd[row];
    }
    for (; lrow < rows; lrow += stride) {
        const bool more = lrow + stride < rows;
        if (more) {
            rown = phys(lrow + stride);
            load_row(dy + rown * D, D, lane, gn);
            load_row(x + rown * D, D, lane, xn);
            mun = mean[rown]; rsn = rstd[rown];
        }
        float s1 = 0.f, s2 = 0.f;
#pragma unroll
        for (int c = 0; c < MAXCH; ++c) {
            int e = (lane + 64 * c) * 4;
            if (e < D) {
                f32x4 gm = load4(gamma + e);
#pragma unroll
                for (int i = 0; i < 4; ++i) {
                    float xh = (xv[c][i] - mu) * rs;
                    float dg = g[c][i] * gm[i];
                    ag[c][i] += g[c][i] * xh;
                    ab[c][i] += g[c][i];
                    s1 += dg; s2 += dg * xh;
                    xv[c][i] = xh; g[c][i] = dg;
                }
            }
        }
        const float c1 = wave_sum(s1) / (float)D, c2 = wave_sum(s2) / (float)D;
#pragma unroll
        for (int c = 0; c < MAXCH; ++c) {
            int e = (lane + 64 * c) * 4;
            if (e < D) {
                f32x4 o;
#pragma unroll
                for (int i = 0; i < 4; ++i) o[i] = rs * (g[c][i] - c1 - xv[c][i] * c2);
                store4(dx + row * D + e, o);
                if (dx2) {
                    o = o * dropout_mult4(seed, ((uint64_t)row * D + e) >> 2, drop_p);
                    store4(dx2 + row * D + e, o);
                }
            }
        }
        if (more) {
#pragma unroll
            for (int c = 0; c < MAXCH; ++c) { g[c] = gn[c]; xv[c] = xn[c]; }
// ... 1 lines not shown
        }
    }
#pragma unroll
    for (int c = 0; c < MAXCH; ++c) {
        if (c * 256 >= D) break;
        __syncthreads();
#pragma unroll
        for (int i = 0; i < 4; ++i) {
            red[0][wave][lane * 4 + i] = ag[c][i];
            red[1][wave][lane * 4 + i] = ab[c][i];
        }
        __syncthreads();
        if constexpr (NW * 64 >= 512) {
            if (threadIdx.x < 512) {
                const int e = threadIdx.x & 255, kind = threadIdx.x >> 8;
                const int col = c * 256 + e;
                if (col < D) {
                    float sacc = 0.f;
#pragma unroll
                    for (int w = 0; w < NW; ++w) sacc += red[kind][w][e];
                    if (part) part[((int64_t)blockIdx.x * 2 + kind) * D + col] = sacc;
                    else atomicAdd((kind ? dbeta : dgamma) + col, sacc);
                }
            }
        } else {
            const int e = threadIdx.x, col = c * 256 + e;
            if (col < D) {
                float sg = 0.f, sb = 0.f;
#pragma unroll
                for (int w = 0; w < NW; ++w) { sg += red[0][w][e]; sb += red[1][w][e]; }
                if (part) {
                    part[((int64_t)blockIdx.x * 2 + 0) * D + col] = sg;
                    part[((int64_t)blockIdx.x * 2 + 1) * D + col] = sb;
                } else {
                    atomicAdd(dgamma + col, sg);
                    atomicAdd(dbeta + col, sb);
                }
            }
        }
    }
}

template <typename T, int MAXCH, int NW, int RPW, bool FULL>
__global__ void __launch_bounds__(NW * 64) layernorm_bwd_rows_kernel(const T* dy, const T* x, const float* gamma, const float* mean,
                                                                    const float* rstd, T* dx, float* dgamma, float* dbeta,
                                                                    int64_t rows, int D, T* dx2, float drop_p, uint64_t seed,
                                                                    const uint64_t* seed_ptr, int seg_len, int seg_stride, int seg_off,
                                                                    float* part) {
    constexpr int GC = MAXCH < 4 ? MAXCH : 4;
    __shared__ float red[2][NW][GC * 256];
    if (dx2 && seed_ptr) seed += *seed_ptr;
    const int lane = threadIdx.x & 63, wave = threadIdx.x >> 6;
    f32x4 ag[MAXCH], ab[MAXCH], gm[MAXCH];
#pragma unroll
    for (int c = 0; c < MAXCH; ++c) {
        f32x4 z = {0.f, 0.f, 0.f, 0.f};
        ag[c] = z; ab[c] = z;
        const int e = (lane + 64 * c) * 4;
        gm[c] = (FULL || e < D) ? load4(gamma + e) : z;
    }
    auto phys = [&](int64_t lrow) { return seg_len > 0 ? (lrow / seg_len) * seg_stride + seg_off + lrow % seg_len : lrow; };
    constexpr int RPB = NW * RPW;
    const float inv_d = 1.0f / (float)D;
    for (int64_t base = (int64_t)blockIdx.x * RPB; base < rows; base += (int64_t)gridDim.x * RPB) {
        f32x4 g[RPW][MAXCH], xv[RPW][MAXCH];
        float mu[RPW], rs[RPW];
        int64_t row[RPW];
        bool ok[RPW];
#pragma unroll
        for (int j = 0; j < RPW; ++j) {
            const int64_t lrow = base + wave + NW * j;
            ok[j] = lrow < rows;
            row[j] = ok[j] ? phys(lrow) : 0;
            if (ok[j]) {
                load_row(dy + row[j] * D, FULL ? MAXCH * 256 : D, lane, g[j]);
                load_row(x + row[j] * D, FULL ? MAXCH * 256 : D, lane, xv[j]);
                mu[j] = mean[row[j]]; rs[j] = rstd[row[j]];
            } else {
#pragma unroll
                for (int c = 0; c < MAXCH; ++c) { f32x4 z = {0.f, 0.f, 0.f, 0.f}; g[j][c] = z; xv[j][c] = z; }
                mu[j] = 0.f; rs[j] = 0.f;
            }
        }
        float s1[RPW], s2[RPW];
#pragma unroll
        for (int j = 0; j < RPW; ++j) {
            s1[j] = 0.f; s2[j] = 0.f;
#pragma unroll
            for (int c = 0; c < MAXCH; ++c) {
                const int e = (lane + 64 * c) * 4;
                if (FULL || e < D) {
#pragma unroll
                    for (int i = 0; i < 4; ++i) {
                        const float xh = (xv[j][c][i] - mu[j]) * rs[j];
                        const float dgv = g[j][c][i] * gm[c][i];
                        ag[c][i] += g[j][c][i] * xh;
                        ab[c][i] += g[j][c][i];
                        s1[j] += dgv; s2[j] += dgv * xh;
                        xv[j][c][i] = xh; g[j][c][i] = dgv;
                    }
                }
            }
        }
#pragma unroll
        for (int o = 32; o > 0; o >>= 1) {
#pragma unroll
            for (int j = 0; j < RPW; ++j) { s1[j] += __shfl_xor(s1[j], o); s2[j] += __shfl_xor(s2[j], o); }
        }
#pragma unroll
        for (int j = 0; j < RPW; ++j) {
            if (!ok[j]) continue;
            const float c1 = s1[j] * inv_d, c2 = s2[j] * inv_d;
#pragma unroll
            for (int c = 0; c < MAXCH; ++c) {
                const int e = (lane + 64 * c) * 4;
                if (FULL || e < D) {
                    f32x4 o;
#pragma unroll
                    for (int i = 0; i < 4; ++i) o[i] = rs[j] * (g[j][c][i] - c1 - xv[j][c][i] * c2);
                    store4(dx + row[j] * D + e, o);
                    if (dx2) {
                        o = o * dropout_mult4(seed, ((uint64_t)row[j] * D + e) >> 2, drop_p);
                        store4(dx2 + row[j] * D + e, o);
                    }
                }
            }
        }
    }
#pragma unroll
    for (int c0 = 0; c0 < MAXCH; c0 += GC) {
        if (c0 * 256 >= D) break;
        if (c0 > 0) __syncthreads();
#pragma unroll
        for (int c = 0; c < GC; ++c) {
            if (c0 + c < MAXCH) {
                *reinterpret_cast<f32x4*>(&red[0][wave][c * 256 + lane * 4]) = ag[c0 + c];
                *reinterpret_cast<f32x4*>(&red[1][wave][c * 256 + lane * 4]) = ab[c0 + c];
            }
        }
        __syncthreads();
        for (int idx = threadIdx.x; idx < 2 * GC * 256; idx += NW * 64) {
            const int kind = idx / (GC * 256), e = idx - kind * (GC * 256);
            const int col = c0 * 256 + e;
            if (col < D) {
                float sacc = 0.f;
#pragma unroll
                for (int w = 0; w < NW; ++w) sacc += red[kind][w][e];
                if (part) part[((int64_t)blockIdx.x * 2 + kind) * D + col] = sacc;
                else atomicAdd((kind ? dbeta : dgamma) + col, sacc);
            }
        }
    }
}

__global__ void __launch_bounds__(1024) ln_partials_reduce_kernel(const float* part, float* grad, const int64_t* off_gamma,
                                                                  const int64_t* off_beta, int nblocks, int D) {
    __shared__ float red[16][256];
    const int lane = threadIdx.x & 63, wave = threadIdx.x >> 6;
    const int kind = blockIdx.y, job = blockIdx.z;
    const int col = blockIdx.x * 256 + lane * 4;
    f32x4 s = {0.f, 0.f, 0.f, 0.f};
    if (col < D) {
        const float* q = part + ((int64_t)job * nblocks * 2 + kind) * D + col;
        int b = wave;
        for (; b + 48 < nblocks; b += 64) {
            f32x4 v0 = load4(q + (int64_t)(b + 0) * 2 * D), v1 = load4(q + (int64_t)(b + 16) * 2 * D);
            f32x4 v2 = load4(q + (int64_t)(b + 32) * 2 * D), v3 = load4(q + (int64_t)(b + 48) * 2 * D);
            s = s + ((v0 + v1) + (v2 + v3));
        }
        for (; b < nblocks; b += 16) s = s + load4(q + (int64_t)b * 2 * D);
    }
#pragma unroll
    for (int i = 0; i < 4; ++i) red[wave][lane * 4 + i] = s[i];
    __syncthreads();
    if (threadIdx.x < 256) {
        const int c = blockIdx.x * 256 + threadIdx.x;
        if (c < D) {
            float t = 0.f;
#pragma unroll
            for (int w = 0; w < 16; ++w) t += red[w][threadIdx.x];
            grad[(kind ? off_beta : off_gamma)[job] + c] += t;
        }
    }
}

template <typename T, int MAXCH>
__global__ void __launch_bounds__(256) text_embed_fwd_kernel(const int64_t* ids, const T* word, const T* pos, const T* type0,
                                                             const float* gamma, const float* beta, T* out, T* pre,
                                                             float* mean_out, float* rstd_out, int B, int Lt, int Ltot, int D,
                                                             float eps, const int64_t* attn_mask, float* key_mask, int period) {
    const int lane = threadIdx.x & 63;
    const int64_t tok = (int64_t)blockIdx.x * 4 + (threadIdx.x >> 6);
    if (tok >= (int64_t)B * Lt) return;
    const int b = (int)(tok / Lt), t = (int)(tok % Lt);
    const int64_t orow = (int64_t)b * Ltot + t;
    const int64_t irow = (int64_t)(b % period) * Lt + t;
    const int64_t id = ids[irow];
    if (key_mask && lane == 0) key_mask[orow] = attn_mask ? (float)attn_mask[irow] : 1.0f;
    f32x4 v[MAXCH], a[MAXCH];
    load_row(word + id * D, D, lane, v);
    load_row(pos + (int64_t)t * D, D, lane, a);
#pragma unroll
    for (int c = 0; c < MAXCH; ++c) v[c] = v[c] + a[c];
    load_row(type0, D, lane, a);
#pragma unroll
    for (int c = 0; c < MAXCH; ++c) v[c] = v[c] + a[c];
    if (pre) {
#pragma unroll
        for (int c = 0; c < MAXCH; ++c) { int e = (lane + 64 * c) * 4; if (e < D) store4(pre + orow * D + e, v[c]); }
    }
    float mean, rstd;
    row_stats(v, D, lane, eps, mean, rstd);
    norm_store(v, gamma, beta, out + orow * D, D, lane, mean, rstd);
    if (lane == 0) {
        if (mean_out) mean_out[orow] = mean;
        if (rstd_out) rstd_out[orow] = rstd;
    }
}

template <typename T, int MAXCH>
__global__ void __launch_bounds__(256) visual_embed_fwd_kernel(const T* grid, const int32_t* src_row, const int32_t* sel,
                                                               const T* row_emb, const T* col_emb, const T* type0,
                                                               const float* gamma, const float* beta, T* out, T* pre,
                                                               float* mean_out, float* rstd_out, int B, int Tf, int Hg, int Wg,
                                                               int Lv, int Lt, int Ltot, int D, float eps, float* key_mask) {
    const int lane = threadIdx.x & 63;
    const int64_t tok = (int64_t)blockIdx.x * 4 + (threadIdx.x >> 6);
    if (tok >= (int64_t)B * Lv) return;
    const int b = (int)(tok / Lv), pidx = (int)(tok % Lv);
    const int q = sel ? sel[pidx] : pidx;
    const int h = q / Wg, w = q % Wg;
    const int64_t src = src_row ? src_row[b] : b;
    const int64_t orow = (int64_t)b * Ltot + Lt + pidx;
    if (key_mask && lane == 0) key_mask[orow] = 1.0f;
    f32x4 v[MAXCH], a[MAXCH];
// ... 256 lines not shown
```

clipbert_amd/modeling/encoder.py:

```python
from collections import namedtuple
from types import SimpleNamespace
from typing import Optional

import numpy as np
import torch
from torch import nn

from .. import ops
from ..ops import ACT_GELU, ACT_TANH, KROW
from .modules import BertEmbeddings, BertEncoder, BertPooler, VisualInputEmbedding, _cfg_get, as_config
from .runtime import _SITE_ATTN, _SITE_EMB, _SITE_OUT, _SITE_POOL, _SITE_SELF_OUT, Runtime, _pick_split, _seed


class ClipBertBaseModel(nn.Module):
    def __init__(self, config):
        super().__init__()
        config = as_config(config)
        assert _cfg_get(config, "hidden_act", "gelu") == "gelu", "only the exact-erf GELU of base_model.json is implemented"
        assert config.hidden_size // config.num_attention_heads == 64, "attention kernels are built for head size 64"
        self.config = config
        self.embeddings = BertEmbeddings(config)
        self.visual_embeddings = VisualInputEmbedding(config)
        self.encoder = BertEncoder(config)
        self.pooler = BertPooler(config)
        self.rt: Optional[Runtime] = None

    def get_input_embeddings(self):
        return self.embeddings.word_embeddings

    def forward(self, text_input_ids, visual_inputs, attention_mask, src_row=None, pooled_dropout=False, text_repeat=1):
        seq, pooled = _EncoderFn.apply(self.rt.anchor, visual_inputs, self, text_input_ids, attention_mask, src_row,
                                       pooled_dropout, text_repeat)
        b = text_input_ids.shape[0] * text_repeat
        return seq.view(b, -1, self.config.hidden_size), pooled


_LayerSaved = namedtuple("_LayerSaved", "qkv ctx lse a_pre mean1 rstd1 hsave o_pre mean2 rstd2")


def _drop_p(model, training, key="hidden_dropout_prob"):
    return float(_cfg_get(model.config, key, 0.0)) if training else 0.0


def encoder_forward(model: ClipBertBaseModel, grid, ids, mask, src_row, pooled_dropout, save, text_repeat=1):
    rt, cfg = model.rt, model.config
    bank, dt, dev = rt.bank, rt.dtype, ids.device
    d, nh, eps = cfg.hidden_size, cfg.num_attention_heads, cfg.layer_norm_eps
    training = model.training
    p_h = _drop_p(model, training)
    p_a = _drop_p(model, training, "attention_probs_dropout_prob")
    fwd_i = 0
    if p_h > 0 or p_a > 0:
        fwd_i = rt.forward_count
        rt.forward_count += 1
    bsz, lt = ids.shape[0] * text_repeat, ids.shape[1]
    bv, t, hg, wg, _ = grid.shape
    sel = None
    lv = hg * wg
    nsamp = int(_cfg_get(cfg, "pixel_random_sampling_size", 0) or 0)
    if nsamp > 0 and training and nsamp < lv:
        idx = np.sort(np.random.choice(lv, size=nsamp, replace=False))
        sel = torch.from_numpy(idx.astype(np.int32)).to(dev)
        lv = nsamp
    L = lt + lv
    M = bsz * L
    if src_row is None:
        assert bv == bsz, "visual batch and text batch differ: pass src_row (n_examples_list)"
    key_mask = torch.empty(bsz, L, dtype=torch.float32, device=dev)
    mask_c = mask if (mask.dtype == torch.int64 and mask.is_contiguous()) else mask.to(torch.int64).contiguous()
    nl, ff = len(model.encoder.layer), cfg.intermediate_size
    stk = None
    if save:
        stk = SimpleNamespace(x=torch.empty(nl, M, d, dtype=dt, device=dev), ctx=torch.empty(nl, M, d, dtype=dt, device=dev),
                              a=torch.empty(nl, M, d, dtype=dt, device=dev), hact=torch.empty(nl, M, ff, dtype=dt, device=dev))
    x = stk.x[0] if save else torch.empty(M, d, dtype=dt, device=dev)
    pre = torch.empty(M, d, dtype=dt, device=dev) if save else None
    mean0, rstd0 = torch.empty(2, M, dtype=torch.float32, device=dev) if save else (None, None)
    emb, vemb = model.embeddings, model.visual_embeddings
    ids_c = ids.contiguous()
    ops.text_embed_fwd(ids_c, bank.compute(emb.word_embeddings.weight), bank.compute(emb.position_embeddings.weight),
                       bank.compute(emb.token_type_embeddings.weight)[0], emb.LayerNorm.weight, emb.LayerNorm.bias, x, pre,
                       mean0, rstd0, lt, L, eps, attn_mask=mask_c, key_mask=key_mask, repeat=text_repeat)
    grid_c = grid.contiguous()
    ops.visual_embed_fwd(grid_c, src_row, sel, bank.compute(vemb.row_position_embeddings.weight),
                         bank.compute(vemb.col_position_embeddings.weight), bank.compute(vemb.token_type_embeddings.weight)[0],
                         vemb.LayerNorm.weight, vemb.LayerNorm.bias, x, pre, mean0, rstd0, bsz, lv, lt, L, eps, key_mask=key_mask)
    if p_h > 0:
        ops.dropout(x, p_h, _seed(_SITE_EMB, 0, fwd_i), rt.seed_dev, out=x)
    layers = []
    for li, layer in enumerate(model.encoder.layer):
        att, so, it, ou = layer.attention.self, layer.attention.output, layer.intermediate, layer.output
        wqkv = bank.compute_span(att.query.weight, att.value.weight, (3 * d, d))
        bqkv = bank.master_span(att.query.bias, att.value.bias, (3 * d,))
        qkv = torch.empty(M, 3 * d, dtype=dt, device=dev)
        ops.gemm(x, wqkv, M, 3 * d, d, out=qkv, shift=bqkv)
        ctx, lse = ops.attention_fwd(qkv, key_mask, bsz, L, nh, save_lse=save, dropout_p=p_a,
                                     dropout_seed=_seed(_SITE_ATTN, li, fwd_i), seed_ptr=rt.seed_dev, out=stk.ctx[li] if save else None)
        a_pre = torch.empty(M, d, dtype=dt, device=dev)
        ops.gemm(ctx, bank.compute(so.dense.weight), M, d, d, out=a_pre, shift=so.dense.bias, residual=x, dropout_p=p_h,
                 dropout_seed=_seed(_SITE_SELF_OUT, li, fwd_i), seed_ptr=rt.seed_dev)
        a, mean1, rstd1 = ops.layernorm_fwd(a_pre, so.LayerNorm.weight, so.LayerNorm.bias, eps, save_stats=save,
                                            out=stk.a[li] if save else None)
        hact = stk.hact[li] if save else torch.empty(M, ff, dtype=dt, device=dev)
        hsave = torch.empty(M, ff, dtype=dt, device=dev) if save else None
        ops.gemm(a, bank.compute(it.dense.weight), M, ff, d, out=hact, shift=it.dense.bias,
                 act=ops.ACT_GELU_SAVE_GRAD if save else ACT_GELU, out2=hsave)
        o_pre = torch.empty(M, d, dtype=dt, device=dev)
        ops.gemm(hact, bank.compute(ou.dense.weight), M, d, ff, out=o_pre, shift=ou.dense.bias, residual=a, dropout_p=p_h,
                 dropout_seed=_seed(_SITE_OUT, li, fwd_i), seed_ptr=rt.seed_dev)
        out, mean2, rstd2 = ops.layernorm_fwd(o_pre, ou.LayerNorm.weight, ou.LayerNorm.bias, eps, save_stats=save,
                                              out=stk.x[li + 1] if (save and li + 1 < nl) else None)
        if save:
            layers.append(_LayerSaved(qkv, ctx, lse, a_pre, mean1, rstd1, hsave, o_pre, mean2, rstd2))
        x = out
    pooled = torch.empty(bsz, d, dtype=dt, device=dev)
    p_pool = p_h if pooled_dropout else 0.0
    pooled_raw = torch.empty(bsz, d, dtype=dt, device=dev) if (save and p_pool > 0) else None
    pw = model.pooler.dense
    drop = dict(dropout_p=p_pool, dropout_seed=_seed(_SITE_POOL, 0, fwd_i), seed_ptr=rt.seed_dev) if pooled_raw is None else {}
    ops.gemm(x, bank.compute(pw.weight), bsz, d, d, out=pooled if pooled_raw is None else pooled_raw, lda=L * d, shift=pw.bias, act=ACT_TANH, **drop)
    if pooled_raw is not None:
        ops.dropout(pooled_raw, p_pool, _seed(_SITE_POOL, 0, fwd_i), rt.seed_dev, out=pooled)
    pack = None
    if save:
        pack = SimpleNamespace(layers=layers, x_final=x, pooled=pooled, pooled_raw=pooled_raw, p_pool=p_pool, pre=pre,
                               mean0=mean0, rstd0=rstd0, ids=ids_c, key_mask=key_mask, src_row=src_row, sel=sel, bsz=bsz,
                               lt=lt, lv=lv, L=L, grid_shape=tuple(grid.shape), p_h=p_h, p_a=p_a, stk=stk, fwd_i=fwd_i, text_repeat=text_repeat)
    return x, pooled, pack


def _linear_wgrad(g, x, m, n, k, gw, gb, ldx=None, gather=None, defer_bias=False):
    rides = gw is not None and gather is None
    if gw is not None:
        split, tile = _pick_split(n, k, m)
        xkw = gather if gather is not None else dict(b_mode=KROW, ldb=ldx if ldx is not None else x.stride(0), a_rowsum=gb)
        ops.gemm(g, x, n, k, m, out=gw, a_mode=KROW, lda=g.stride(0), **xkw, accumulate=True, split_k=split, tile=tile)
    owed = None if rides else gb
    if owed is not None and not defer_bias:
        ops.colsum(g, owed, m, n)
        owed = None
    return owed


def _uniform_stride(tensors):
    if any(t is None for t in tensors):
        return None
    if len(tensors) == 1:
        return 0
    steps = {b.data_ptr() - a.data_ptr() for a, b in zip(tensors, tensors[1:])}
    step, esz = steps.pop(), tensors[0].element_size()
    return step // esz if (not steps and step > 0 and step % esz == 0) else None


def _encoder_wgrads(model, pk, gs, M):
    rt, cfg = model.rt, model.config
    bank = rt.bank
    d, ff = cfg.hidden_size, cfg.intermediate_size
    layers = list(model.encoder.layer)
    nl, stk = len(layers), pk.stk

    def qkv(l, name, shape):
        q, v = getattr(l.attention.self.query, name), getattr(l.attention.self.value, name)
        return bank.grad_span(q, v, shape) if bank.is_trainable(q) else None

    def imgs(lin):
        return [bank.grad_image(lin(l).weight) for l in layers], [bank.grad_image(lin(l).bias) for l in layers]

    kinds = [
        (gs.out, stk.hact, d, ff, imgs(lambda l: l.output.dense), "out"),
        (gs.hp, stk.a, ff, d, imgs(lambda l: l.intermediate.dense), "ffn"),
        (gs.att, stk.ctx, d, d, imgs(lambda l: l.attention.output.dense), "att"),
        (gs.qkv, stk.x, 3 * d, d, ([qkv(l, "weight", (3 * d, d)) for l in layers], [qkv(l, "bias", (3 * d,)) for l in layers]), "qkv"),
    ]
    def batch_strides(n, k, gws, gbs):
        st = (_uniform_stride(gws), _uniform_stride(gbs))
        return st if (None not in st and n % 8 == 0 and k % 8 == 0) else None

    strides = [batch_strides(n, k, *im) for _g, _x, n, k, im, _kd in kinds]
    all_batched = None not in strides
    fresh = bank.take_fresh()
    if fresh and not all_batched:
        a, b = bank.lazy_span
        bank.grad[a:b].zero_()
        fresh = False
    if not fresh:
        bank.fold_invalidate()
    bf16 = rt.dtype == torch.bfloat16
    group = [] if (all_batched and bf16) else None
    for (g, x, n, k, (gws, gbs), kind), st in zip(kinds, strides):
        if st is None:
            for li in range(nl):
                _linear_wgrad(g[li], x[li], M, n, k, gws[li], gbs[li])
            continue
        slots = bank.fold_take(ops.sq_slot_count(n, k, nl), "enc:" + kind) if (fresh and bf16) else None
        desc = dict(out=gws[0], a_mode=KROW, lda=n, b_mode=KROW, ldb=k, ldc=k, accumulate=not fresh, a_rowsum=gbs[0], batch=nl,
                    batch_strides=(M * n, M * k, *st), sq_slots=slots)
        if group is None:
            ops.gemm(g, x, n, k, M, **desc)
        else:
            group.append(ops.gemm_desc(g, x, n, k, M, tile=4, **desc))
    if group:
        ops.gemm_group(group, gs.out)


def _ln_offsets(model, dev):
    rt = model.rt
    cached = rt._ln_off
    if cached is not None and cached[0] is rt.bank:
        return cached[1]
    bank, offs = rt.bank, ([], [])
    for layer in model.encoder.layer:
        for ln in (layer.attention.output.LayerNorm, layer.output.LayerNorm):
            gw, gb = bank.grad_image(ln.weight), bank.grad_image(ln.bias)
            if gw is None or gb is None:
                rt._ln_off = (bank, None)
                return None
            offs[0].append((gw.data_ptr() - bank.grad.data_ptr()) // 4)
            offs[1].append((gb.data_ptr() - bank.grad.data_ptr()) // 4)
    t = torch.tensor(offs, dtype=torch.int64).to(dev)
    rt._ln_off = (bank, t)
    return t


def encoder_backward(model: ClipBertBaseModel, pk, d_seq, d_pooled):
    rt, cfg = model.rt, model.config
    bank, dt = rt.bank, rt.dtype
    d, nh, ff = cfg.hidden_size, cfg.num_attention_heads, cfg.intermediate_size
    bsz, L, lt, lv = pk.bsz, pk.L, pk.lt, pk.lv
    M = bsz * L
    dev = pk.x_final.device
    if d_seq is None:
        dx = ops.zeros((M, d), dt, dev)
    else:
        dx = d_seq.reshape(M, d)
        if dx.dtype != dt or not dx.is_contiguous():
            dx = ops.cast(dx.contiguous(), torch.empty(M, d, dtype=dt, device=dev))
    if d_pooled is not None:
        g = d_pooled.to(dt).contiguous()
        if pk.pooled_raw is not None:
            g = ops.dropout(g, pk.p_pool, _seed(_SITE_POOL, 0, pk.fwd_i), rt.seed_dev)
            g = ops.act_bwd(ACT_TANH, g, pk.pooled_raw)
        else:
            g = ops.act_bwd(ACT_TANH, g, pk.pooled)
        pw = model.pooler.dense
        _linear_wgrad(g, pk.x_final, bsz, d, d, bank.grad_image(pw.weight), bank.grad_image(pw.bias), ldx=L * d)
        ops.gemm(g, bank.compute(pw.weight), bsz, d, d, out=dx, b_mode=KROW, ldc=L * d, accumulate=True)
    nl, stk = len(pk.layers), pk.stk
    ln_off = _ln_offsets(model, dev)
    nb = ops.ln_part_blocks(M)
    ln_part = torch.empty(2 * nl, nb, 2, d, dtype=torch.float32, device=dev) if ln_off is not None else None

    def ln_bwd(slot, dy, xpre, ln, mean, rstd, seed, g_out):
        keep = dict(dx2=g_out) if pk.p_h > 0 else dict(dx=g_out)
        if ln_part is not None:
            d_pre, d_drop = ops.layernorm_bwd_part(dy, xpre, ln.weight, mean, rstd, ln_part[slot], pk.p_h, seed, rt.seed_dev, **keep)
        else:
            d_pre, d_drop = ops.layernorm_bwd(dy, xpre, ln.weight, mean, rstd, bank.grad_image(ln.weight), bank.grad_image(ln.bias), pk.p_h,
                                              seed, rt.seed_dev, **keep)
        return d_pre, d_drop if d_drop is not None else d_pre

    gs = SimpleNamespace(out=torch.empty(nl, M, d, dtype=dt, device=dev), hp=torch.empty(nl, M, ff, dtype=dt, device=dev),
                         att=torch.empty(nl, M, d, dtype=dt, device=dev), qkv=torch.empty(nl, M, 3 * d, dtype=dt, device=dev))
    for li in range(nl - 1, -1, -1):
        layer = model.encoder.layer[li]
        att, so, it, ou = layer.attention.self, layer.attention.output, layer.intermediate, layer.output
        sv = pk.layers[li]
        d_o_pre, g = ln_bwd(2 * li + 1, dx, sv.o_pre, ou.LayerNorm, sv.mean2, sv.rstd2, _seed(_SITE_OUT, li, pk.fwd_i), gs.out[li])
        dhp = gs.hp[li]
        ops.gemm(g, bank.compute(ou.dense.weight), M, ff, d, out=dhp, b_mode=KROW, gelu_grad_pre=sv.hsave,
                 act=ops.ACT_SAVED_GRAD)
        da = torch.empty(M, d, dtype=dt, device=dev)
        ops.gemm(dhp, bank.compute(it.dense.weight), M, d, ff, out=da, b_mode=KROW, residual=d_o_pre)
        d_a_pre, g = ln_bwd(2 * li, da, sv.a_pre, so.LayerNorm, sv.mean1, sv.rstd1, _seed(_SITE_SELF_OUT, li, pk.fwd_i), gs.att[li])
        dctx = torch.empty(M, d, dtype=dt, device=dev)
        ops.gemm(g, bank.compute(so.dense.weight), M, d, d, out=dctx, b_mode=KROW)
        dqkv = ops.attention_bwd(sv.qkv, pk.key_mask, sv.ctx, dctx, sv.lse, bsz, L, nh, pk.p_a, _seed(_SITE_ATTN, li, pk.fwd_i), rt.seed_dev,
                                 out=gs.qkv[li])
        wqkv = bank.compute_span(att.query.weight, att.value.weight, (3 * d, d))
        dx = torch.empty(M, d, dtype=dt, device=dev)
        ops.gemm(dqkv, wqkv, M, d, 3 * d, out=dx, b_mode=KROW, residual=d_a_pre)
    if ln_part is not None:
        ops.ln_partials_reduce(ln_part, bank.grad, ln_off[0], ln_off[1])
    _encoder_wgrads(model, pk, gs, M)
    if pk.p_h > 0:
        dx = ops.dropout(dx, pk.p_h, _seed(_SITE_EMB, 0, pk.fwd_i), rt.seed_dev)
    emb, vemb = model.embeddings, model.visual_embeddings
    dpre = torch.empty(M, d, dtype=dt, device=dev)
    ops.layernorm_bwd(dx, pk.pre, emb.LayerNorm.weight, pk.mean0, pk.rstd0, bank.grad_image(emb.LayerNorm.weight),
                      bank.grad_image(emb.LayerNorm.bias), dx=dpre, rows=bsz * lt, seg=(lt, L, 0))
    ops.layernorm_bwd(dx, pk.pre, vemb.LayerNorm.weight, pk.mean0, pk.rstd0, bank.grad_image(vemb.LayerNorm.weight),
                      bank.grad_image(vemb.LayerNorm.bias), dx=dpre, rows=bsz * lv, seg=(lv, L, lt))
    we = emb.word_embeddings
    ops.text_embed_bwd(dpre, pk.ids, bank.grad_image(we.weight), bank.grad_image(emb.position_embeddings.weight),
                       bank.grad_image(emb.token_type_embeddings.weight)[0], lt, L,
                       we.padding_idx if we.padding_idx is not None else -1, repeat=pk.text_repeat)
    dgrid = ops.zeros(pk.grid_shape, torch.float32, dev)
    ops.visual_embed_bwd(dpre, pk.src_row, pk.sel, dgrid, bank.grad_image(vemb.row_position_embeddings.weight),
                         bank.grad_image(vemb.col_position_embeddings.weight), bank.grad_image(vemb.token_type_embeddings.weight)[0],
                         bsz, lv, lt, L)
    return dgrid if dt == torch.float32 else ops.cast(dgrid, torch.empty(pk.grid_shape, dtype=dt, device=dev))


class _EncoderFn(torch.autograd.Function):
    @staticmethod
    def forward(ctx, anchor, grid, model, ids, mask, src_row, pooled_dropout, text_repeat=1):
        save = ctx.needs_input_grad[0]
        ctx.set_materialize_grads(False)
        seq, pooled, pack = encoder_forward(model, grid, ids, mask, src_row, pooled_dropout, save, text_repeat)
        ctx.model, ctx.pack = model, pack
        if save:
            model.rt.pending_encoder_nodes += 1
        return seq, pooled

    @staticmethod
    def backward(ctx, d_seq, d_pooled):
        dgrid = encoder_backward(ctx.model, ctx.pack, d_seq, d_pooled)
        ctx.pack = None
        ctx.model.rt.node_done("encoder", fire=True)
        return None, dgrid, None, None, None, None, None, None
```

clipbert_amd/modeling/runtime.py:

```python
from typing import Optional

import torch

from .. import ops
from ..params import ParamBank

_HOOK = {"encoder": "after_encoder_backward", "cnn": "after_res5_backward"}


class Runtime:
    def __init__(self):
        self.bank: Optional[ParamBank] = None
        self.dtype = torch.bfloat16
        self.tables = {}
        self.rowmaps = {}
        self.seed_dev: Optional[torch.Tensor] = None
        self.anchor: Optional[torch.Tensor] = None
        self.stem_w = None
        self.after_encoder_backward = None
        self.pending_encoder_nodes = 0
        self.after_res5_backward = None
        self.pending_cnn_nodes = 0
        self.prepare_args = None
        self._ln_off = None
        self.forward_count = 0

    def begin_step(self):
        self.pending_encoder_nodes = self.pending_cnn_nodes = 0

    def fire_if_last(self, kind, left=1):
        hook = getattr(self, _HOOK[kind])
        if hook is not None and getattr(self, f"pending_{kind}_nodes") <= left:
            hook()

    def node_done(self, kind, fire=False):
        setattr(self, f"pending_{kind}_nodes", max(0, getattr(self, f"pending_{kind}_nodes") - 1))
        if fire:
            self.fire_if_last(kind, left=0)

    def table(self, n, oh, ow, stride, pad, sN, sH, sW, device):
        key = (n, oh, ow, stride, pad, sN, sH, sW, str(device))
        t = self.tables.get(key)
        if t is None:
            t = ops.build_pixel_table(n, oh, ow, stride, pad, sN, sH, sW, device)
            self.tables[key] = t
        return t

    def strided_rowmap(self, n, h, w, oh, ow, stride, device):
        key = (n, h, w, oh, ow, stride, str(device))
        t = self.rowmaps.get(key)
        if t is None:
            t = (torch.arange(n).view(n, 1, 1) * (h * w) + (torch.arange(oh) * stride).view(1, oh, 1) * w
                 + (torch.arange(ow) * stride).view(1, 1, ow)).reshape(-1).to(torch.int32).to(device)
            self.rowmaps[key] = t
        return t


def _pick_split(mo, no, kred):
    ktiles = (kred + 63) // 64
    b64 = ((mo + 63) // 64) * ((no + 63) // 64)
    if b64 >= 200 or ktiles < 64:
        return 1, 0
    split = max(1, min(ktiles // 8, (400 + b64 // 2) // b64))
    return split, 0


_SITE_EMB, _SITE_ATTN, _SITE_SELF_OUT, _SITE_OUT, _SITE_POOL, _SITE_REG = 1, 2, 3, 4, 5, 6


def _seed(site, layer=0, fwd=0):
    return ((site * 1000003 + layer * 7919) * 2654435761 + fwd * 0x9E3779B97F4A7C15) % (1 << 62)
```

clipbert_amd/ops.py:

```python
import ctypes as C
import os
from typing import Optional

import torch

from . import _lib
from ._lib import (ACT_GELU, ACT_GELU_SAVE_GRAD, ACT_NONE, ACT_RELU, ACT_SAVED_GRAD, ACT_TANH, CB_BF16, CB_F32, KROW, KROW_GATHER,
                   KROW_TAPS, ROWK, ROWK_GATHER, GemmDesc)

_ALLOW_HOST_POINTERS = False


def dtype_code(t: torch.dtype) -> int:
    if t == torch.bfloat16:
        return CB_BF16
    if t == torch.float32:
        return CB_F32
    raise TypeError(f"unsupported dtype {t}")


def _ptr(t: Optional[torch.Tensor]):
    if t is None:
        return None
    if not t.is_cuda and not _ALLOW_HOST_POINTERS:
        raise RuntimeError("clipbert_amd ops need CUDA(HIP) tensors: there is no CPU path")
    return t.data_ptr()


def _extent_bytes(t: torch.Tensor) -> int:
    return t.untyped_storage().nbytes() - t.storage_offset() * t.element_size()


def _stream(t: torch.Tensor):
    if t.is_cuda:
        return torch.cuda.current_stream(t.device).cuda_stream
    return None


def _chk(rc, what):
    _lib.check(rc, what)


def gemm_desc(a: torch.Tensor, b: torch.Tensor, M: int, N: int, K: int, *, out: torch.Tensor, a_mode=ROWK,
              b_mode=ROWK, lda=None, ldb=None, ldc=None, a_tab=None, b_tab=None, R=1, S=1, Cin=0, H=0, W=0,
              sH=0, sW=0, flip_taps=False, c_rowmap=None, accumulate=False, split_k=1, act=ACT_NONE,
              scale=None, shift=None, residual=None, ldr=None, relu_after=False, mask=None, ldm=None,
              out2=None, ldc2=None, alpha=1.0, dropout_p=0.0, dropout_seed=0, seed_ptr=None, tile=0, gelu_grad_pre=None, a_rowsum=None, batch=1, batch_strides=None,
              relu_bwd=False, post_scale=None, post_scale2=None, xcd_order=0, zero_fill_pitch=0, splitk_ws=None, schedule=0, sq_slots=None) -> GemmDesc:
    d = GemmDesc()
    d.dtype = dtype_code(a.dtype)
    assert b.dtype == a.dtype
    d.M, d.N, d.K = M, N, K
    d.a_mode, d.b_mode = a_mode, b_mode
    d.A, d.B = _ptr(a), _ptr(b)
    d.lda = lda if lda is not None else a.stride(0)
    d.ldb = ldb if ldb is not None else b.stride(0)
    d.a_tab, d.b_tab = _ptr(a_tab), _ptr(b_tab)
    d.R, d.S, d.Cin, d.H, d.W, d.sH, d.sW = R, S, Cin, H, W, sH, sW
    d.flip_taps = int(flip_taps)
    d.C = _ptr(out)
    d.ldc = ldc if ldc is not None else out.stride(0)
    d.c_rowmap = _ptr(c_rowmap)
    d.zero_fill_pitch = zero_fill_pitch
    d.c_f32 = int(out.dtype == torch.float32)
    d.accumulate = int(accumulate)
    d.split_k = split_k
    d.act = act
    d.scale, d.shift = _ptr(scale), _ptr(shift)
    d.residual = _ptr(residual)
    d.ldr = (ldr if ldr is not None else residual.stride(0)) if residual is not None else 0
    d.relu_after = int(relu_after)
    d.mask = _ptr(mask)
    d.ldm = (ldm if ldm is not None else mask.stride(0)) if mask is not None else 0
    d.C2 = _ptr(out2)
    d.ldc2 = (ldc2 if ldc2 is not None else out2.stride(0)) if out2 is not None else 0
    d.alpha = alpha
    d.dropout_p = dropout_p
    d.dropout_seed = dropout_seed
    d.dropout_seed_ptr = _ptr(seed_ptr)
    if _KEY_LOG is not None:
        _KEY_LOG.append((a_mode, b_mode, M, N, K, batch, R * S, split_k))
    if tile == 0 and _LAUNCH_OVERRIDE:
        ov = _LAUNCH_OVERRIDE.get((a_mode, b_mode, M, N, K, batch, R * S, split_k))
        if ov is not None:
            tile, xcd_order, schedule = ov[0], ov[1], ov[3]
            d.split_k = ov[2] if ov[2] > 0 else split_k
    d.tile = tile
    d.schedule = schedule
    d.xcd_order = xcd_order
    d.a_bytes = _extent_bytes(a)
    d.b_bytes = _extent_bytes(b)
    if gelu_grad_pre is not None:
        d.gelu_grad_pre, d.ld_gelu = _ptr(gelu_grad_pre), gelu_grad_pre.stride(0)
    if a_rowsum is not None:
        assert a_rowsum.dtype == torch.float32
        d.a_rowsum = _ptr(a_rowsum)
    if relu_bwd:
        d.relu_bwd = 1
        d.post_scale, d.post_scale2 = _ptr(post_scale), _ptr(post_scale2)
    if batch > 1:
        d.batch = batch
        d.batch_stride_a, d.batch_stride_b, d.batch_stride_c, d.batch_stride_rowsum = batch_strides
    if splitk_ws is None and d.dtype == CB_BF16 and not _SPLITK_OFF:
        splitk_ws = splitk_workspace(a.device)
    if splitk_ws is not None:
        d.splitk_ws, d.splitk_ws_bytes = _ptr(splitk_ws), splitk_ws.numel() * splitk_ws.element_size()
    if sq_slots is not None:
        assert sq_slots.dtype == torch.float32 and sq_slots.is_contiguous()
        d.sq_slots, d.sq_slots_n = _ptr(sq_slots), sq_slots.numel()
    d._refs = (a, b, out, a_tab, b_tab, c_rowmap, scale, shift, residual, mask, out2, seed_ptr, gelu_grad_pre, a_rowsum, post_scale,
               post_scale2, splitk_ws, sq_slots)
    return d


def gemm(a: torch.Tensor, b: torch.Tensor, M: int, N: int, K: int, *, out: torch.Tensor, **kw):
    d = gemm_desc(a, b, M, N, K, out=out, **kw)
    _chk(_lib.get().cb_gemm(C.byref(d), _stream(a)), "cb_gemm")
    return out


def gemm_plan(a: torch.Tensor, b: torch.Tensor, M: int, N: int, K: int, *, out: torch.Tensor, use_table: bool = True, **kw):
    d = gemm_desc(a, b, M, N, K, out=out, **kw)
    plan = (C.c_int32 * 4)()
    _chk(_lib.get().cb_gemm_plan(C.byref(d), 1 if use_table else 0, plan), "cb_gemm_plan")
    return tuple(plan)


def gemm_group(descs, like: torch.Tensor):
    n = len(descs)
    if n == 0:
        return
    arr = (GemmDesc * n)()
    for i, d in enumerate(descs):
        C.memmove(C.byref(arr[i]), C.byref(d), C.sizeof(GemmDesc))
    _chk(_lib.get().cb_gemm_group(C.cast(arr, C.c_void_p), n, _stream(like)), "cb_gemm_group")


_KEY_LOG = None
_LAUNCH_OVERRIDE = {}
_TILE_ID = {"128x128": 1, "64x64": 2, "128x64": 3, "128x128o2": 4, "8w256x256": 5, "8w128x256": 6, "8w256x128": 7}


def parse_launch_config(name: str):
    parts = name.split("/")
    tile = _TILE_ID[parts[0]]
    xcd = 1 if parts[1] == "xcd" else 2
    split = ([int(x[1:]) for x in parts[2:] if x[0] == "s"] or [0])[0]
    sched = ([int(x[1:]) + 1 for x in parts[2:] if x[0] == "m"] or [0])[0]
    return (tile, xcd, split or (1 if tile >= 5 else 0), sched)


for _item in filter(None, os.environ.get("CB_LAUNCH_OVERRIDE", "").split(";")):
    _k, _, _c = _item.partition("=")
    _LAUNCH_OVERRIDE[tuple(int(x) for x in _k.split(","))] = parse_launch_config(_c)
_SPLITK_WS = {}
_SPLITK_OFF = False
SPLITK_WS_BYTES = 128 << 20


def splitk_workspace(device) -> torch.Tensor:
    dev = torch.device(device)
    key = str(dev)
    ws = _SPLITK_WS.get(key)
    if ws is None:
        if dev.type == "cuda" and torch.cuda.is_current_stream_capturing():
            return None
        ws = new_splitk_workspace(device)
        _SPLITK_WS[key] = ws
    return ws


def new_splitk_workspace(device, nbytes: int = SPLITK_WS_BYTES) -> torch.Tensor:
    assert nbytes % 16 == 0 and nbytes > _lib.SPLITK_WS_COUNTER_BYTES
    ws = torch.empty(nbytes // 4, dtype=torch.float32, device=device)
    ws[-(_lib.SPLITK_WS_COUNTER_BYTES // 4):].zero_()
    return ws


def build_pixel_table(n: int, oh: int, ow: int, stride: int, pad: int, sN: int, sH: int, sW: int,
                      device) -> torch.Tensor:
    tab = torch.empty(n * oh * ow, dtype=torch.int64, device=device)
    _chk(_lib.get().cb_build_pixel_table(_ptr(tab), n, oh, ow, stride, pad, sN, sH, sW, _stream(tab)),
         "cb_build_pixel_table")
    return tab


def _f3(vals):
    return (C.c_float * 3)(*[float(v) for v in vals])


def stem_pack(src: torch.Tensor, dtype: torch.dtype, pad: int = 3, mean=None, std=None, extra_w: int = 0) -> torch.Tensor:
    n, c, h, w = src.shape
    assert c == 3 and src.is_contiguous()
    hp, wp = h + 2 * pad, w + 2 * pad + extra_w
    dst = torch.empty(n, hp, wp, 4, dtype=dtype, device=src.device)
    u8 = src.dtype == torch.uint8
    assert u8 or src.dtype == torch.float32
    m3 = _f3(mean) if u8 else None
    s3 = _f3(std) if u8 else None
    _chk(_lib.get().cb_stem_pack(dtype_code(dtype), _ptr(src), int(u8), m3, s3, _ptr(dst), n, h, w, hp, wp, pad,
                                 _stream(src)), "cb_stem_pack")
    return dst


def resize_pack_u8(flat_u8: torch.Tensor, table: torch.Tensor, n: int, size: int, dtype: torch.dtype, mean, std, hwc: bool = True,
                   pad: int = 3, extra_w: int = 0, host_table: Optional[torch.Tensor] = None) -> torch.Tensor:
    assert flat_u8.dtype == torch.uint8 and flat_u8.dim() == 1 and flat_u8.is_contiguous()
    assert table.dtype == torch.int64 and tuple(table.shape) == (n, 5) and table.is_contiguous() and table.device == flat_u8.device
# ... 380 lines not shown
```

include/clipbert_hip.h:

```cpp
#ifndef CLIPBERT_HIP_H
#define CLIPBERT_HIP_H

#include <stddef.h>
#include <stdint.h>

#ifdef __cplusplus
extern "C" {
#endif

enum { CB_F32 = 0, CB_BF16 = 1 };
enum { CB_SPLITK_WS_COUNTER_BYTES = 65536 };
enum { CB_ACT_NONE = 0, CB_ACT_RELU = 1, CB_ACT_GELU = 2, CB_ACT_TANH = 3,
       CB_ACT_GELU_SAVE_GRAD = 4,
       CB_ACT_SAVED_GRAD = 5 };

enum {
    CB_ROWK = 0,
    CB_ROWK_GATHER = 1,
    CB_KROW = 2,
    CB_KROW_TAPS = 3,
    CB_KROW_GATHER = 4
};

typedef struct { int32_t off; int16_t ih0; int16_t iw0; } cb_pixel;

typedef struct {
    int32_t dtype;
    int32_t M, N, K;
    int32_t a_mode, b_mode;
    const void* A; const void* B;
    int64_t lda, ldb;
    const cb_pixel* a_tab;
    const cb_pixel* b_tab;
    int32_t R, S, Cin;
    int32_t H, W;
    int64_t sH, sW;
    int32_t flip_taps;
    int32_t schedule;
    void* C; int64_t ldc;
    const int32_t* c_rowmap;
    int32_t c_f32;
    int32_t accumulate;
    int32_t split_k;
    int32_t act;
    const float* scale;
    const float* shift;
    const void* residual; int64_t ldr;
    int32_t relu_after;
    int32_t zero_fill_pitch;
    const void* mask; int64_t ldm;
    void* C2; int64_t ldc2;
    float alpha;
    float dropout_p;
    uint64_t dropout_seed;
    const uint64_t* dropout_seed_ptr;
    int32_t tile;
    int32_t xcd_order;
    int64_t a_bytes, b_bytes;
    const void* gelu_grad_pre; int64_t ld_gelu;
    float* a_rowsum;
    int32_t batch;
    int32_t relu_bwd;
    int64_t batch_stride_a, batch_stride_b, batch_stride_c, batch_stride_rowsum;
    const float* post_scale; const float* post_scale2;
    void* splitk_ws;
    int64_t splitk_ws_bytes;
    float* sq_slots;
    int64_t sq_slots_n;
} cb_gemm_desc;

int cb_gemm(const cb_gemm_desc* d, void* stream);
int cb_gemm_plan(const cb_gemm_desc* d, int32_t use_table, int32_t* out4);
int cb_gemm_workspace_bytes(const cb_gemm_desc* d, int64_t* bytes);
int cb_gemm_group(const cb_gemm_desc* descs, int32_t n, void* stream);

int cb_build_pixel_table(cb_pixel* tab, int32_t N, int32_t OH, int32_t OW, int32_t stride, int32_t pad,
                         int64_t sN, int64_t sH, int64_t sW, void* stream);

int cb_stem_pack(int32_t dtype, const void* src, int32_t src_u8, const float* mean3, const float* std3,
                 void* dst, int32_t N, int32_t H, int32_t W, int32_t Hp, int32_t Wp, int32_t pad,
                 void* stream);

int cb_resize_pack_u8(int32_t dtype, const uint8_t* flat, int64_t flat_bytes, const int64_t* table, const int64_t* table_host, int32_t N,
                      int32_t hwc, const float* mean3, const float* std3, void* dst, int32_t S, int32_t Hp, int32_t Wp, int32_t pad,
                      void* stream);

int cb_image_norm(const uint8_t* src, float* dst, const float* mean3, const float* std3,
                  int64_t n_images, int64_t hw, void* stream);

int cb_maxpool_fwd(int32_t dtype, const void* x, void* y, int32_t N, int32_t H, int32_t W, int32_t C,
                   int32_t OH, int32_t OW, int32_t k, int32_t stride, int32_t pad, int32_t relu,
                   void* stream);
int cb_maxpool2_bwd(int32_t dtype, const void* x, const void* y, const void* dy, void* dx, int32_t N,
                    int32_t H, int32_t W, int32_t C, int32_t OH, int32_t OW, int32_t relu, void* stream);

int cb_stem_pool(const void* packed, const void* weight, const float* scale, const float* shift, void* out, int32_t N, int32_t Hp,
                 int32_t Wp, int32_t OH, int32_t OW, int32_t PH, int32_t PW, void* stream);
int cb_stem_pool_u8(const uint8_t* frames, const float* mean3, const float* std3, const void* weight, const float* scale, const float* shift,
                    void* out, int32_t N, int32_t H, int32_t W, int32_t OH, int32_t OW, int32_t PH, int32_t PW, void* stream);

typedef struct cb_res2_desc {
    const void* x; void* out;
    const void* w1; const void* w2; const void* w3; const void* wsc;
    const float* scale1; const float* shift1; const float* scale2; const float* shift2; const float* scale3; const float* shift3;
    const float* scale_sc; const float* shift_sc;
    int32_t N, H, W, cin;
} cb_res2_desc;
int cb_res2_block(const cb_res2_desc* desc, void* stream);

int cb_relu_scale_bwd(int32_t dtype, const void* dy, const void* y, const float* scale, void* g,
                      void* dz, const float* scale2, void* g2, int64_t rows, int32_t C, void* stream);

int cb_layernorm_fwd(int32_t dtype, const void* x, const float* gamma, const float* beta, void* y,
                     float* mean, float* rstd, int64_t rows, int32_t D, float eps, int32_t seg_len,
                     int32_t seg_stride, int32_t seg_off, void* stream);
int cb_layernorm_bwd(int32_t dtype, const void* dy, const void* x, const float* gamma, const float* mean,
                     const float* rstd, void* dx, float* dgamma, float* dbeta, int64_t rows, int32_t D,
                     void* dx2, float dropout_p, uint64_t dropout_seed, const uint64_t* dropout_seed_ptr,
                     int32_t seg_len, int32_t seg_stride, int32_t seg_off, void* stream);
int cb_layernorm_bwd_part(int32_t dtype, const void* dy, const void* x, const float* gamma, const float* mean,
                          const float* rstd, void* dx, float* part, int32_t nblocks, int64_t rows, int32_t D,
                          void* dx2, float dropout_p, uint64_t dropout_seed, const uint64_t* dropout_seed_ptr,
                          int32_t seg_len, int32_t seg_stride, int32_t seg_off, void* stream);
int cb_ln_partials_reduce(const float* part, float* grad, const int64_t* off_gamma, const int64_t* off_beta,
                          int32_t njobs, int32_t nblocks, int32_t D, void* stream);

int cb_text_embed_fwd(int32_t dtype, const int64_t* ids, const void* word, const void* pos, const void* type0,
                      const float* gamma, const float* beta, void* out, void* pre, float* mean, float* rstd,
                      int32_t B, int32_t Lt, int32_t L_total, int32_t D, float eps, const int64_t* attn_mask,
                      float* key_mask, int32_t rows_period, void* stream);
int cb_visual_embed_fwd(int32_t dtype, const void* grid, const int32_t* src_row, const int32_t* sel,
                        const void* row_emb, const void* col_emb, const void* type0, const float* gamma,
                        const float* beta, void* out, void* pre, float* mean, float* rstd, int32_t B,
                        int32_t T, int32_t Hg, int32_t Wg, int32_t Lv, int32_t Lt, int32_t L_total, int32_t D,
                        float eps, float* key_mask, void* stream);
int cb_text_embed_bwd(int32_t dtype, const void* dpre, const int64_t* ids, float* dword, float* dpos,
                      float* dtype0, int32_t B, int32_t Lt, int32_t L_total, int32_t D, int64_t pad_id,
                      int32_t rows_period, void* stream);
int cb_visual_embed_bwd(int32_t dtype, const void* dpre, const int32_t* src_row, const int32_t* sel,
                        float* dgrid, float* drow, float* dcol, float* dtype0, int32_t B, int32_t T,
                        int32_t Hg, int32_t Wg, int32_t Lv, int32_t Lt, int32_t L_total, int32_t D,
                        void* stream);

int cb_attention_fwd(int32_t dtype, const void* qkv, const float* key_mask, void* ctx, float* lse,
                     int32_t B, int32_t L, int32_t H, float dropout_p, uint64_t dropout_seed,
                     const uint64_t* dropout_seed_ptr, void* stream);
int cb_attention_bwd(int32_t dtype, const void* qkv, const float* key_mask, const void* ctx, const void* dctx,
                     const float* lse, float* dsum_ws, void* dqkv, int32_t B, int32_t L, int32_t H,
                     float dropout_p, uint64_t dropout_seed, const uint64_t* dropout_seed_ptr, void* stream);

int cb_cross_entropy(const float* logits, int64_t ld, const int64_t* labels, float* loss, float* dlogits,
                     const float* dloss, int64_t rows, int32_t C, int64_t ignore_index, void* stream);

int cb_colsum(int32_t dtype, const void* g, int64_t ldg, float* out, int64_t M, int32_t N, void* stream);

// ... 62 lines not shown
```

Baseline: 4170 clips/s.

## Fuse LayerNorm forward and backward into the preceding GEMM epilogue via row-panel tail

Adds a row_op option to the GEMM descriptor so the last tile finishing a row panel (tracked with split-k workspace counters) runs LayerNorm forward, or LayerNorm backward with column partial sums, on the freshly written rows. The BERT encoder forward and backward paths route the N=768 dense GEMMs through this, skipping separate LayerNorm kernel launches and a re-read of C from HBM. A fallback runs the standalone LN kernel when fusion isn't eligible. The cost is extra tail work and counter synchronisation inside the GEMM, plus added complexity in layer ordering, such as hoisting the previous layer's LN backward into the QKV dgrad GEMM.

```diff
diff --git a/clipbert_amd/_lib.py b/clipbert_amd/_lib.py
--- a/clipbert_amd/_lib.py
+++ b/clipbert_amd/_lib.py
@@ -9,6 +9,7 @@
 SPLITK_WS_COUNTER_BYTES = 65536
 ACT_GELU_SAVE_GRAD, ACT_SAVED_GRAD = 4, 5
 ROWK, ROWK_GATHER, KROW, KROW_TAPS, KROW_GATHER = 0, 1, 2, 3, 4
+ROWOP_NONE, ROWOP_LN_FWD, ROWOP_LN_BWD = 0, 1, 2
 (HP_LR, HP_BETA1, HP_BETA2, HP_EPS, HP_WD, HP_BC1, HP_BC2, HP_MAX_NORM, HP_GRAD_SCALE, HP_SKIP, HP_COUNT) = range(11)
 OPT_ADAMW, OPT_ADAM, OPT_ADAMAX = 0, 1, 2
 
@@ -29,6 +30,8 @@
         ("batch", i32), ("relu_bwd", i32), ("batch_stride_a", i64), ("batch_stride_b", i64), ("batch_stride_c", i64),
         ("batch_stride_rowsum", i64), ("post_scale", vp), ("post_scale2", vp), ("splitk_ws", vp), ("splitk_ws_bytes", i64),
         ("sq_slots", vp), ("sq_slots_n", i64),
+        ("row_op", i32), ("ln_eps", f32), ("ln_gamma", vp), ("ln_beta", vp), ("ln_out", vp), ("ln_out2", vp), ("ln_mean", vp), ("ln_rstd", vp),
+        ("ln_x", vp), ("ln_part", vp), ("ln_dropout_p", f32), ("ln_reserved", i32), ("ln_dropout_seed", u64), ("ln_dropout_seed_ptr", vp),
     ]
 
 
@@ -44,6 +47,7 @@
     "cb_stem_pool": [vp, vp, vp, vp, vp, i32, i32, i32, i32, i32, i32, i32, vp],
     "cb_stem_pool_u8": [vp, vp, vp, vp, vp, vp, vp, i32, i32, i32, i32, i32, i32, i32, vp],
     "cb_gemm_plan": [vp, i32, vp],
+    "cb_gemm_plan_rowop": [vp, i32, vp],
     "cb_gemm_group": [vp, i32, vp],
     "cb_gemm_workspace_bytes": [vp, vp],
     "cb_build_pixel_table": [vp, i32, i32, i32, i32, i32, i64, i64, i64, vp],
diff --git a/clipbert_amd/csrc/common.hip b/clipbert_amd/csrc/common.hip
--- a/clipbert_amd/csrc/common.hip
+++ b/clipbert_amd/csrc/common.hip
@@ -22,4 +22,4 @@
 }
 
 extern "C" const char* cb_last_error(void) { return g_err; }
-extern "C" int cb_version(void) { return 9; }
+extern "C" int cb_version(void) { return 10; }
diff --git a/clipbert_amd/csrc/gemm.hip b/clipbert_amd/csrc/gemm.hip
--- a/clipbert_amd/csrc/gemm.hip
+++ b/clipbert_amd/csrc/gemm.hip
@@ -12,6 +12,8 @@
 extern template int launch_gemm<bf16, 128, 64, 2>(const GP&, bool, hipStream_t);
 extern template int launch_gemm<bf16, 64, 64, 3>(const GP&, bool, hipStream_t);
 extern template int launch_gemm<bf16, 128, 128, 1, 2>(const GP&, bool, hipStream_t);
+extern template int launch_gemm_rowop<64, 64, 3>(const GP&, const RowOp&, hipStream_t);
+extern template int launch_gemm_rowop<128, 64, 2>(const GP&, const RowOp&, hipStream_t);
 extern template int launch_gemm_group<float, 64, 64, 2, 1>(const GroupArgs&, int, hipStream_t);
 extern template int launch_gemm_group<bf16, 64, 64, 3, 1>(const GroupArgs&, int, hipStream_t);
 extern template int launch_gemm_group<bf16, 128, 128, 1, 2>(const GroupArgs&, int, hipStream_t);
@@ -115,6 +117,49 @@
     if (form == 1) return launch_gemm8_fwd<BM, BN, WGM, WGN, NST>(p, mode, ws, st);
     if (form == 2) return launch_gemm8_dgrad<BM, BN, WGM, WGN, NST>(p, mode, ws, st);
     return launch_gemm8_wgrad<BM, BN, WGM, WGN, NST>(p, mode, ws, st);
+}
+
+inline int64_t part_rows(const cb_gemm_desc* d) { return ((int64_t)d->M + 63) / 64; }
+int rowop_prepare(const cb_gemm_desc* d, Prepared& out) {
+    RowOp& ro = out.ro;
+    ro = RowOp{};
+    if (d->row_op == CB_ROWOP_NONE) return 0;
+    const bool bwd = d->row_op == CB_ROWOP_LN_BWD;
+    CB_REQUIRE(d->row_op == CB_ROWOP_LN_FWD || bwd, "cb_gemm: bad row_op %d", d->row_op);
+    CB_REQUIRE(d->dtype == CB_BF16 && !d->c_f32, "cb_gemm: row_op needs bf16 operands and a bf16 C");
+    CB_REQUIRE(d->N == ROWOP_D && d->ldc == d->N, "cb_gemm: row_op needs N == ldc == %d (one LayerNorm row), got N %d ldc %lld", ROWOP_D, d->N, (long long)d->ldc);
+    CB_REQUIRE(d->accumulate == 0 && d->split_k <= 1 && d->batch <= 1 && !d->c_rowmap && d->K > 0,
+               "cb_gemm: row_op excludes accumulate, split_k > 1, batch > 1, c_rowmap and K == 0");
+    CB_REQUIRE((int64_t)d->M * d->N * 2 < 0x7fffffffll, "cb_gemm: row_op needs C below 2 GiB");
+    CB_REQUIRE(d->ln_gamma && d->ln_out && aligned16(d->ln_gamma) && (reinterpret_cast<uintptr_t>(d->ln_out) & 7) == 0, "cb_gemm: row_op needs ln_gamma (16-byte aligned) and ln_out (8-byte aligned)");
+    if (bwd) {
+        CB_REQUIRE(d->ln_x && d->ln_mean && d->ln_rstd && d->ln_part, "cb_gemm: CB_ROWOP_LN_BWD needs ln_x, ln_mean, ln_rstd and ln_part");
+        CB_REQUIRE((reinterpret_cast<uintptr_t>(d->ln_x) & 7) == 0 && (reinterpret_cast<uintptr_t>(d->ln_out2) & 7) == 0, "cb_gemm: ln_x / ln_out2 must be 8-byte aligned");
+        CB_REQUIRE(d->ln_dropout_p >= 0.f && d->ln_dropout_p < 1.f && (!d->ln_out2 || d->ln_dropout_p > 0.f), "cb_gemm: ln_dropout_p out of range, or ln_out2 without it");
+        CB_REQUIRE(part_rows(d) <= 1024, "cb_gemm: CB_ROWOP_LN_BWD covers at most 65536 rows");
+    } else {
+        CB_REQUIRE(d->ln_beta && aligned16(d->ln_beta) && !d->ln_out2, "cb_gemm: CB_ROWOP_LN_FWD needs ln_beta (16-byte aligned) and takes no ln_out2");
+    }
+    struct Span { const void* p; int64_t n; };
+    auto span_rows = [&](const void* q, int64_t ld, int64_t esz) { return Span{q, q ? ((int64_t)(d->M - 1) * ld + d->N) * esz : 0}; };
+    const Span ins[] = {{d->A, d->a_bytes > 0 ? d->a_bytes : (d->a_mode == CB_KROW ? ((int64_t)(d->K - 1) * d->lda + d->M) * 2 : ((int64_t)(d->M - 1) * d->lda + d->K) * 2)},
+                        {d->B, d->b_bytes > 0 ? d->b_bytes : (d->b_mode == CB_ROWK ? ((int64_t)(d->N - 1) * d->ldb + d->K) * 2 : ((int64_t)(d->K - 1) * d->ldb + d->N) * 2)},
+                        span_rows(d->residual, d->ldr, 2), span_rows(d->mask, d->ldm, 2), span_rows(d->C, d->ldc, 2)};
+    const Span outs[] = {span_rows(d->ln_out, d->N, 2), span_rows(d->ln_out2, d->N, 2),
+                         {bwd ? nullptr : d->ln_mean, (int64_t)d->M * 4}, {bwd ? nullptr : d->ln_rstd, (int64_t)d->M * 4},
+                         {bwd ? d->ln_part : nullptr, part_rows(d) * 2 * d->N * 4}};
+    for (const Span& o : outs)
+        for (const Span& i : ins) {
+            if (!o.p || !i.p) continue;
+            const char* a = static_cast<const char*>(o.p); const char* b = static_cast<const char*>(i.p);
+            CB_REQUIRE(a + o.n <= b || b + i.n <= a, "cb_gemm: a row_op output overlaps A, B, residual, mask or C");
+        }
+    ro.kind = d->row_op; ro.eps = d->ln_eps; ro.drop_p = d->ln_dropout_p;
+    ro.gamma = d->ln_gamma; ro.beta = d->ln_beta;
+    ro.out = static_cast<bf16*>(d->ln_out); ro.out2 = static_cast<bf16*>(d->ln_out2);
+    ro.mean = d->ln_mean; ro.rstd = d->ln_rstd; ro.x = static_cast<const bf16*>(d->ln_x); ro.part = d->ln_part;
+    ro.seed = d->ln_dropout_seed; ro.seed_ptr = d->ln_dropout_seed_ptr;
+    return 0;
 }
 
 int gemm_prepare(const cb_gemm_desc* d, Prepared& out) {
@@ -270,7 +315,7 @@
     out.form = operand_form(d->a_mode, d->b_mode, taps); out.taps = taps;
     out.epi_scale_only = !d->C2 && !d->residual && !d->mask && !d->gelu_grad_pre && d->act == CB_ACT_NONE && !d->relu_after && !d->shift && d->dropout_p <= 0.f;
     out.atomics_ok = out.epi_scale_only && d->c_f32 && d->accumulate == 1;
-    return 0;
+    return rowop_prepare(d, out);
 }
 
 int gemm_validate(const cb_gemm_desc* d, Prepared& pr, bool& empty) {
@@ -291,7 +336,7 @@
                 lp.picked, d->tile, lp.form8, lp.tile >= 5 ? lp.split_k : pr.p.split_k, (int)lp.slab);
 }
 
-int gemm_launch(const cb_gemm_desc* d, const Prepared& pr, const LaunchPlan& lp, hipStream_t st) {
+int gemm_launch_product(const cb_gemm_desc* d, const Prepared& pr, const LaunchPlan& lp, hipStream_t st) {
     GP p = pr.p;
     if (lp.tile == 9) return launch_gemm_skinny(d, p, st);
     p.split_k = lp.split_k;
@@ -320,6 +365,23 @@
     return launch_gemm<bf16, 64, 64, 3>(p, pr.fast, st);
 }
 
+int gemm_launch(const cb_gemm_desc* d, const Prepared& pr, const LaunchPlan& lp, hipStream_t st) {
+    if (lp.rowop_fused) {
+        GP p = pr.p;
+        p.split_k = 1; p.c_vec8 = lp.c_vec8; p.xcd_remap = lp.xcd_remap;
+        RowOp ro = pr.ro;
+        ro.cnt = splitk_counters(d->splitk_ws, d->splitk_ws_bytes);
+        return lp.tile == 3 ? launch_gemm_rowop<128, 64, 2>(p, ro, st) : launch_gemm_rowop<64, 64, 3>(p, ro, st);
+    }
+    if (int rc = gemm_launch_product(d, pr, lp, st)) return rc;
+    if (d->row_op == CB_ROWOP_LN_FWD)
+        return cb_layernorm_fwd(CB_BF16, d->C, d->ln_gamma, d->ln_beta, d->ln_out, d->ln_mean, d->ln_rstd, d->M, d->N, d->ln_eps, 0, 0, 0, st);
+    if (d->row_op == CB_ROWOP_LN_BWD)
+        return cb_layernorm_bwd_part(CB_BF16, d->C, d->ln_x, d->ln_gamma, d->ln_mean, d->ln_rstd, d->ln_out, d->ln_part, (int32_t)part_rows(d), d->M, d->N,
+                                     d->ln_out2, d->ln_dropout_p, d->ln_dropout_seed, d->ln_dropout_seed_ptr, 0, 0, 0, st);
+    return 0;
+}
+
 int gemm_run(const cb_gemm_desc* d, const Prepared& pr, void* stream) {
     LaunchPlan lp;
     const int rc = gemm_choose(d, pr, true, false, lp);
@@ -348,6 +410,20 @@
     return 0;
 }
 
+extern "C" int cb_gemm_plan_rowop(const cb_gemm_desc* d, int32_t use_table, int32_t* out2) {
+    CB_REQUIRE(out2 != nullptr, "cb_gemm_plan_rowop: null output");
+    out2[0] = out2[1] = 0;
+    Prepared pr;
+    LaunchPlan lp;
+    bool empty;
+    if (int rc = gemm_validate(d, pr, empty)) return rc;
+    if (empty) return 0;
+    if (int rc = gemm_choose(d, pr, use_table != 0, false, lp)) return rc;
+    out2[0] = lp.rowop_fused ? 1 : 0;
+    out2[1] = d->row_op == CB_ROWOP_LN_BWD ? (int32_t)part_rows(d) : 0;
+    return 0;
+}
+
 extern "C" int cb_gemm_workspace_bytes(const cb_gemm_desc* d, int64_t* bytes) {
     CB_REQUIRE(d != nullptr && bytes != nullptr, "cb_gemm_workspace_bytes: null argument");
     *bytes = 0;
@@ -363,7 +439,7 @@
 
 namespace {
 int group_class(const cb_gemm_desc* d, const Prepared& pr) {
-    if (!pr.fast || d->zero_fill_pitch || d->tile >= 5 || d->tile == 1 || d->tile == 3) return -1;
+    if (!pr.fast || d->zero_fill_pitch || d->tile >= 5 || d->tile == 1 || d->tile == 3 || d->row_op != CB_ROWOP_NONE) return -1;
     if (d->batch > 1 || d->a_rowsum) {
         const bool ok = d->dtype == CB_BF16 && pr.form == FORM_WGRAD && d->split_k <= 1 && d->tile != 2 && !d->c_rowmap;
         return ok ? GC_WGRAD_RS : -1;
diff --git a/clipbert_amd/csrc/gemm_choose.h b/clipbert_amd/csrc/gemm_choose.h
--- a/clipbert_amd/csrc/gemm_choose.h
+++ b/clipbert_amd/csrc/gemm_choose.h
@@ -54,6 +54,7 @@
     int taps;
     bool epi_scale_only;
     bool atomics_ok;
+    RowOp ro;
 };
 constexpr int GROUP_COUNTERS = CB_SPLITK_WS_COUNTER_BYTES / (int)sizeof(int);
 inline int64_t splitk_payload_bytes(int64_t ws_bytes) { return ws_bytes > CB_SPLITK_WS_COUNTER_BYTES ? ws_bytes - CB_SPLITK_WS_COUNTER_BYTES : 0; }
@@ -136,7 +137,17 @@
     bool c_vec8 = false;
     int form8 = 0;
     int picked = 0;
-};
+    bool rowop_fused = false;
+};
+
+inline bool rowop_fuses(const cb_gemm_desc* d, const Prepared& pr, const LaunchPlan& lp) {
+    if (pr.ro.kind == CB_ROWOP_NONE || (lp.tile != 2 && lp.tile != 3) || d->dtype != CB_BF16) return false;
+    if (!pr.fast || !lp.c_vec8 || pr.p.wt != 1 || lp.split_k != 1 || d->relu_bwd || d->zero_fill_pitch) return false;
+    if (d->a_mode != CB_ROWK || (d->b_mode != CB_ROWK && d->b_mode != CB_KROW)) return false;
+    const int bm = lp.tile == 3 ? 128 : 64;
+    return splitk_counters(d->splitk_ws, d->splitk_ws_bytes) != nullptr && d->splitk_ws_bytes % 4 == 0 &&
+           (reinterpret_cast<uintptr_t>(d->splitk_ws) & 3) == 0 && (d->M + bm - 1) / bm <= GROUP_COUNTERS;
+}
 struct Pick { int tile = 0, split = 0, sched = 0; };
 constexpr int64_t WS_UNLIMITED = (int64_t)1 << 60;
 constexpr int STREAM_MIN_ROWS = 32768;
@@ -219,6 +230,7 @@
     if (d->zero_fill_pitch != 0)
         CB_REQUIRE(d->zero_fill_pitch > 0 && d->c_rowmap && lp.c_vec8 && d->batch <= 1,
                    "cb_gemm: zero_fill_pitch needs c_rowmap and 16-byte-aligned 8-column chunks (N, ldc %% 8 == 0)");
+    lp.rowop_fused = rowop_fuses(d, pr, lp);
     return 0;
 }
 }
diff --git a/clipbert_amd/csrc/gemm_impl.h b/clipbert_amd/csrc/gemm_impl.h
--- a/clipbert_amd/csrc/gemm_impl.h
+++ b/clipbert_amd/csrc/gemm_impl.h
@@ -1,5 +1,6 @@
 #pragma once
 #include "common.h"
+#include "ln_row.h"
 #include <stdlib.h>
 #include <type_traits>
 
@@ -1400,8 +1401,127 @@
 }
 
 
-template <typename T, int BM, int BN, typename LA, typename LB, int PF, bool RS, int OCC>
-__device__ __forceinline__ void gemm_tile(GP& p, TileId bid, float* slab = nullptr, int* cnt = nullptr) {
+struct RowOp {
+    int kind;
+    float eps, drop_p;
+    const float* gamma; const float* beta;
+    bf16* out; bf16* out2;
+    float* mean; float* rstd;
+    const bf16* x;
+    float* part;
+    uint64_t seed; const uint64_t* seed_ptr;
+    int* cnt;
+};
+constexpr int ROWOP_D = 768, ROWOP_NCH = ROWOP_D / 256;
+template <int BM> struct RowOpRows { static constexpr int FWD = BM >= 128 ? 8 : 4, BWD = BM >= 128 ? 2 : 1; };
+
+__device__ __forceinline__ void rowop_request(rsrc_t rc, uint32_t m, int lane, bool ok, u32x4 (&raw)[ROWOP_NCH]) {
+#pragma unroll
+    for (int c = 0; c < ROWOP_NCH; ++c)
+        raw[c] = __builtin_amdgcn_raw_buffer_load_b128(rc, ok ? (m * (uint32_t)ROWOP_D + (uint32_t)((lane + 64 * c) >> 1) * 8u) * 2u : OOB, 0, 16 );
+}
+__device__ __forceinline__ void rowop_unpack(const u32x4 (&raw)[ROWOP_NCH], int lane, f32x4 (&v)[ROWOP_NCH]) {
+#pragma unroll
+    for (int c = 0; c < ROWOP_NCH; ++c) {
+        union { u32x2 r; bf16x4 x; } u;
+        u.r = (lane & 1) ? u32x2{raw[c][2], raw[c][3]} : u32x2{raw[c][0], raw[c][1]};
+        v[c] = f32x4{(float)u.x[0], (float)u.x[1], (float)u.x[2], (float)u.x[3]};
+    }
+}
+
+template <int BM, int RIF>
+__device__ __forceinline__ void rowop_ln_fwd(const GP& p, const RowOp& ro, int m0, int tid) {
+    constexpr int NCH = ROWOP_NCH, D = ROWOP_D;
+    const int lane = tid & 63, wave = tid >> 6;
+    const int nrows = p.M - m0 < BM ? p.M - m0 : BM;
+    const rsrc_t rc = make_rsrc(p.C, (uint32_t)((int64_t)p.M * D * 2));
+    f32x4 gm[NCH], bt[NCH];
+#pragma unroll
+    for (int c = 0; c < NCH; ++c) { gm[c] = load4(ro.gamma + (lane + 64 * c) * 4); bt[c] = load4(ro.beta + (lane + 64 * c) * 4); }
+#pragma unroll 1
+    for (int r0 = wave; r0 < nrows; r0 += 4 * RIF) {
+        u32x4 raw[RIF][NCH];
+#pragma unroll
+        for (int j = 0; j < RIF; ++j) rowop_request(rc, (uint32_t)(m0 + r0 + 4 * j), lane, r0 + 4 * j < nrows, raw[j]);
+#pragma unroll
+        for (int j = 0; j < RIF; ++j) {
+            if (r0 + 4 * j >= nrows) break;
+            const int64_t row = m0 + r0 + 4 * j;
+            f32x4 v[NCH];
+            rowop_unpack(raw[j], lane, v);
+            float mean, rstd;
+            cbln::fwd_row_full(v, gm, bt, ro.eps, lane, ro.out + row * D, mean, rstd);
+            if (lane == 0) {
+                if (ro.mean) ro.mean[row] = mean;
+                if (ro.rstd) ro.rstd[row] = rstd;
+            }
+        }
+    }
+}
+
+template <int BM, int RPW>
+__device__ __forceinline__ void rowop_ln_bwd(const GP& p, const RowOp& ro, int m0, int tid, unsigned char* smem) {
+    constexpr int NCH = ROWOP_NCH, D = ROWOP_D;
+    const int lane = tid & 63, wave = tid >> 6;
+    const rsrc_t rc = make_rsrc(p.C, (uint32_t)((int64_t)p.M * D * 2));
+    uint64_t seed = ro.seed;
+    if (ro.out2 && ro.seed_ptr) seed += *ro.seed_ptr;
+    f32x4 gm[NCH];
+#pragma unroll
+    for (int c = 0; c < NCH; ++c) gm[c] = load4(ro.gamma + (lane + 64 * c) * 4);
+    const float inv_d = 1.0f / (float)D;
+#pragma unroll 1
+    for (int base = m0; base < m0 + BM && base < p.M; base += 64) {
+        const int nrows = p.M - base < 64 ? p.M - base : 64;
+        f32x4 ag[NCH], ab[NCH];
+#pragma unroll
+        for (int c = 0; c < NCH; ++c) { f32x4 z = {0.f, 0.f, 0.f, 0.f}; ag[c] = z; ab[c] = z; }
+#pragma unroll 1
+        for (int r0 = wave; r0 < nrows; r0 += 4 * RPW) {
+            u32x4 raw[RPW][NCH];
+            f32x4 g[RPW][NCH], xv[RPW][NCH];
+            float mu[RPW], rs[RPW];
+            int64_t row[RPW];
+            bool ok[RPW];
+#pragma unroll
+            for (int j = 0; j < RPW; ++j) {
+                ok[j] = r0 + 4 * j < nrows;
+                row[j] = ok[j] ? base + r0 + 4 * j : 0;
+                rowop_request(rc, (uint32_t)row[j], lane, ok[j], raw[j]);
+                if (ok[j]) {
+                    cbln::load_row(ro.x + row[j] * D, D, lane, xv[j]);
+                    mu[j] = ro.mean[row[j]]; rs[j] = ro.rstd[row[j]];
+                } else {
+#pragma unroll
+                    for (int c = 0; c < NCH; ++c) { f32x4 z = {0.f, 0.f, 0.f, 0.f}; xv[j][c] = z; }
+                    mu[j] = 0.f; rs[j] = 0.f;
+                }
+            }
+#pragma unroll
+            for (int j = 0; j < RPW; ++j) rowop_unpack(raw[j], lane, g[j]);
+            cbln::bwd_rows<bf16, NCH, RPW, true>(g, xv, mu, rs, ok, row, gm, ag, ab, lane, D, inv_d, ro.out, ro.out2, seed, ro.drop_p);
+        }
+        if (base > m0) __syncthreads();
+        cbln::colsum_flush<NCH, 4>(reinterpret_cast<float*>(smem), ag, ab, tid, D, ro.part + (int64_t)(base >> 6) * 2 * D, nullptr, nullptr);
+    }
+}
+
+template <int KIND, int BM, int BN, int SMEM_BYTES>
+__device__ __forceinline__ void rowop_tail(const GP& p, const RowOp& ro, int panel, int m0, int tid, unsigned char* smem) {
+    static_assert(2 * 4 * ROWOP_D * 4 <= SMEM_BYTES, "column sums do not fit the staging area");
+    __shared__ int s_rowop_last;
+    __builtin_amdgcn_s_waitcnt(0x0f70);
+    __syncthreads();
+    if (tid == 0) s_rowop_last = atomicAdd(ro.cnt + panel, 1) == (p.N + BN - 1) / BN - 1;
+    __syncthreads();
+    if (!s_rowop_last) return;
+    if (tid == 0) atomicExch(ro.cnt + panel, 0);
+    if constexpr (KIND == CB_ROWOP_LN_FWD) rowop_ln_fwd<BM, RowOpRows<BM>::FWD>(p, ro, m0, tid);
+    else rowop_ln_bwd<BM, RowOpRows<BM>::BWD>(p, ro, m0, tid, smem);
+}
+
+template <typename T, int BM, int BN, typename LA, typename LB, int PF, bool RS, int OCC, int ROP = CB_ROWOP_NONE>
+__device__ __forceinline__ void gemm_tile(GP& p, TileId bid, float* slab = nullptr, int* cnt = nullptr, const RowOp* ro = nullptr) {
     using X = Tr<T>;
     constexpr int BK = X::BK;
     constexpr int WM = BM / 2, WN = BN / 2, FM = WM / 16, FN = WN / 16;
@@ -1617,6 +1737,7 @@
     constexpr int FORM_ = LA::KROW ? 0 : (LB::KROW ? 2 : 1);
     if constexpr (EPF != 0) tile_epilogue<T, BM, BN, SMEM_BYTES, EPF, false, FORM_>(p, acc, smem, m0, n0, tid, epre, epf_on);
     else tile_epilogue<T, BM, BN, SMEM_BYTES, 0, LA::KROW, FORM_>(p, acc, smem, m0, n0, tid, EpiPre<BM, BN, true>{}, false, tile_lin);
+    if constexpr (ROP != CB_ROWOP_NONE) rowop_tail<ROP, BM, BN, SMEM_BYTES>(p, *ro, bid.by, m0, tid, smem);
     CB_STAMP(3);
     CB_STAMP_FLUSH(p, stamp_lin, tid);
 }
@@ -1624,6 +1745,11 @@
 template <typename T, int BM, int BN, typename LA, typename LB, int PF, bool RS = false, int OCC = 1>
 __global__ void __launch_bounds__(256, OCC) gemm_kernel(GP p) {
     gemm_tile<T, BM, BN, LA, LB, PF, RS, OCC>(p, tile_id(p));
+}
+
+template <int KIND, int BM, int BN, typename LA, typename LB, int PF, int OCC>
+__global__ void __launch_bounds__(256, OCC) gemm_rowop_kernel(GP p, RowOp ro) {
+    gemm_tile<bf16, BM, BN, LA, LB, PF, false, OCC, KIND>(p, tile_id(p), nullptr, nullptr, &ro);
 }
 
 #ifdef CB_STAMPS
@@ -1792,6 +1918,21 @@
     if (!a_krow) return launch_k<T, BM, BN, PF, OCC, RowkLoader<T, BM, false>, KrowLoader<T, BN, false>>(p, st);
     if (p.b_mode == CB_KROW) return launch_wgrad<T, BM, BN, PF, OCC, KrowLoader<T, BM, false>, KrowLoader<T, BN, false>>(p, st);
     return launch_k<T, BM, BN, PF, OCC, KrowLoader<T, BM, false>, KrowLoader<T, BN, false>>(p, st);
+}
+
+template <int BM, int BN, int PF, int OCC = 1>
+int launch_gemm_rowop(const GP& p, const RowOp& ro, hipStream_t st) {
+    dim3 grid((p.N + BN - 1) / BN, (p.M + BM - 1) / BM, 1);
+    using RA = RowkFast<bf16, BM, false>; using RB = RowkFast<bf16, BN, false>; using KB = KrowTr<BN, KM_PLAIN>;
+    const bool fwd = ro.kind == CB_ROWOP_LN_FWD;
+    if (p.b_mode == CB_ROWK) {
+        if (fwd) hipLaunchKernelGGL((gemm_rowop_kernel<CB_ROWOP_LN_FWD, BM, BN, RA, RB, PF, OCC>), grid, dim3(NTHREADS), 0, st, p, ro);
+        else hipLaunchKernelGGL((gemm_rowop_kernel<CB_ROWOP_LN_BWD, BM, BN, RA, RB, PF, OCC>), grid, dim3(NTHREADS), 0, st, p, ro);
+    } else {
+        if (fwd) hipLaunchKernelGGL((gemm_rowop_kernel<CB_ROWOP_LN_FWD, BM, BN, RA, KB, PF, OCC>), grid, dim3(NTHREADS), 0, st, p, ro);
+        else hipLaunchKernelGGL((gemm_rowop_kernel<CB_ROWOP_LN_BWD, BM, BN, RA, KB, PF, OCC>), grid, dim3(NTHREADS), 0, st, p, ro);
+    }
+    return cb_launch_status("cb_gemm (row operation)");
 }
 
 enum { GC_WGRAD = 0,
diff --git a/clipbert_amd/csrc/gemm_inst_bf16_128x64.hip b/clipbert_amd/csrc/gemm_inst_bf16_128x64.hip
--- a/clipbert_amd/csrc/gemm_inst_bf16_128x64.hip
+++ b/clipbert_amd/csrc/gemm_inst_bf16_128x64.hip
@@ -2,4 +2,5 @@
 
 namespace cbgemm {
 template int launch_gemm<bf16, 128, 64, 2>(const GP&, bool, hipStream_t);
+template int launch_gemm_rowop<128, 64, 2>(const GP&, const RowOp&, hipStream_t);
 }
diff --git a/clipbert_amd/csrc/gemm_inst_bf16_64x64.hip b/clipbert_amd/csrc/gemm_inst_bf16_64x64.hip
--- a/clipbert_amd/csrc/gemm_inst_bf16_64x64.hip
+++ b/clipbert_amd/csrc/gemm_inst_bf16_64x64.hip
@@ -3,4 +3,5 @@
 namespace cbgemm {
 template int launch_gemm<bf16, 64, 64, 3>(const GP&, bool, hipStream_t);
 template int launch_gemm_group<bf16, 64, 64, 3, 1>(const GroupArgs&, int, hipStream_t);
+template int launch_gemm_rowop<64, 64, 3>(const GP&, const RowOp&, hipStream_t);
 }
diff --git a/clipbert_amd/csrc/ln_row.h b/clipbert_amd/csrc/ln_row.h
--- /dev/null
+++ b/clipbert_amd/csrc/ln_row.h
@@ -0,0 +1,121 @@
+#pragma once
+#include "common.h"
+
+namespace cbln {
+
+template <int MAXCH, typename T>
+__device__ __forceinline__ void load_row(const T* p, int D, int lane, f32x4 (&v)[MAXCH]) {
+#pragma unroll
+    for (int c = 0; c < MAXCH; ++c) {
+        int e = (lane + 64 * c) * 4;
+        f32x4 z = {0.f, 0.f, 0.f, 0.f};
+        v[c] = (e < D) ? load4(p + e) : z;
+    }
+}
+
+template <typename T, int MAXCH>
+__device__ __forceinline__ void fwd_row_full(const f32x4 (&v)[MAXCH], const f32x4 (&gm)[MAXCH], const f32x4 (&bt)[MAXCH], float eps, int lane,
+                                             T* yrow, float& mean, float& rstd) {
+    float s = 0.f;
+#pragma unroll
+    for (int c = 0; c < MAXCH; ++c) s += v[c][0] + v[c][1] + v[c][2] + v[c][3];
+    const float inv_d = 1.0f / (float)(MAXCH * 256);
+    mean = wave_sum(s) * inv_d;
+    float q = 0.f;
+#pragma unroll
+    for (int c = 0; c < MAXCH; ++c)
+#pragma unroll
+        for (int i = 0; i < 4; ++i) { const float d = v[c][i] - mean; q += d * d; }
+    rstd = rsqrtf(wave_sum(q) * inv_d + eps);
+#pragma unroll
+    for (int c = 0; c < MAXCH; ++c) {
+        f32x4 o;
+#pragma unroll
+        for (int i = 0; i < 4; ++i) o[i] = (v[c][i] - mean) * rstd * gm[c][i] + bt[c][i];
+        store4(yrow + (lane + 64 * c) * 4, o);
+    }
+}
+
+template <typename T, int MAXCH, int RPW, bool FULL>
+__device__ __forceinline__ void bwd_rows(f32x4 (&g)[RPW][MAXCH], f32x4 (&xv)[RPW][MAXCH], const float (&mu)[RPW], const float (&rs)[RPW],
+                                         const bool (&ok)[RPW], const int64_t (&row)[RPW], const f32x4 (&gm)[MAXCH], f32x4 (&ag)[MAXCH],
+                                         f32x4 (&ab)[MAXCH], int lane, int D, float inv_d, T* dx, T* dx2, uint64_t seed, float drop_p) {
+    float s1[RPW], s2[RPW];
+#pragma unroll
+    for (int j = 0; j < RPW; ++j) {
+        s1[j] = 0.f; s2[j] = 0.f;
+#pragma unroll
+        for (int c = 0; c < MAXCH; ++c) {
+            const int e = (lane + 64 * c) * 4;
+            if (FULL || e < D) {
+#pragma unroll
+                for (int i = 0; i < 4; ++i) {
+                    const float xh = (xv[j][c][i] - mu[j]) * rs[j];
+                    const float dgv = g[j][c][i] * gm[c][i];
+                    ag[c][i] += g[j][c][i] * xh;
+                    ab[c][i] += g[j][c][i];
+                    s1[j] += dgv; s2[j] += dgv * xh;
+                    xv[j][c][i] = xh; g[j][c][i] = dgv;
+                }
+            }
+        }
+    }
+#pragma unroll
+    for (int o = 32; o > 0; o >>= 1) {
+#pragma unroll
+        for (int j = 0; j < RPW; ++j) { s1[j] += __shfl_xor(s1[j], o); s2[j] += __shfl_xor(s2[j], o); }
+    }
+#pragma unroll
+    for (int j = 0; j < RPW; ++j) {
+        if (!ok[j]) continue;
+        const float c1 = s1[j] * inv_d, c2 = s2[j] * inv_d;
+#pragma unroll
+        for (int c = 0; c < MAXCH; ++c) {
+            const int e = (lane + 64 * c) * 4;
+            if (FULL || e < D) {
+                f32x4 o;
+#pragma unroll
+                for (int i = 0; i < 4; ++i) o[i] = rs[j] * (g[j][c][i] - c1 - xv[j][c][i] * c2);
+                store4(dx + row[j] * D + e, o);
+                if (dx2) {
+                    o = o * dropout_mult4(seed, ((uint64_t)row[j] * D + e) >> 2, drop_p);
+                    store4(dx2 + row[j] * D + e, o);
+                }
+            }
+        }
+    }
+}
+
+template <int MAXCH, int NW>
+__device__ __forceinline__ void colsum_flush(float* red, const f32x4 (&ag)[MAXCH], const f32x4 (&ab)[MAXCH], int tid, int D, float* part_row,
+                                             float* dgamma, float* dbeta) {
+    constexpr int GC = MAXCH < 4 ? MAXCH : 4;
+    const int lane = tid & 63, wave = tid >> 6;
+    auto at = [&](int kind, int w, int e) -> float& { return red[(kind * NW + w) * (GC * 256) + e]; };
+#pragma unroll
+    for (int c0 = 0; c0 < MAXCH; c0 += GC) {
+        if (c0 * 256 >= D) break;
+        if (c0 > 0) __syncthreads();
+#pragma unroll
+        for (int c = 0; c < GC; ++c) {
+            if (c0 + c < MAXCH) {
+                *reinterpret_cast<f32x4*>(&at(0, wave, c * 256 + lane * 4)) = ag[c0 + c];
+                *reinterpret_cast<f32x4*>(&at(1, wave, c * 256 + lane * 4)) = ab[c0 + c];
+            }
+        }
+        __syncthreads();
+        for (int idx = tid; idx < 2 * GC * 256; idx += NW * 64) {
+            const int kind = idx / (GC * 256), e = idx - kind * (GC * 256);
+            const int col = c0 * 256 + e;
+            if (col < D) {
+                float sacc = 0.f;
+#pragma unroll
+                for (int w = 0; w < NW; ++w) sacc += at(kind, w, e);
+                if (part_row) part_row[(int64_t)kind * D + col] = sacc;
+                else atomicAdd((kind ? dbeta : dgamma) + col, sacc);
+            }
+        }
+    }
+}
+
+}
diff --git a/clipbert_amd/csrc/norm.hip b/clipbert_amd/csrc/norm.hip
--- a/clipbert_amd/csrc/norm.hip
+++ b/clipbert_amd/csrc/norm.hip
@@ -1,20 +1,12 @@
 #include "common.h"
+#include "ln_row.h"
 
 #include <stdlib.h>
 
 namespace {
+using cbln::load_row;
 
 constexpr int MAXD = 2048;
-
-template <int MAXCH, typename T>
-__device__ __forceinline__ void load_row(const T* p, int D, int lane, f32x4 (&v)[MAXCH]) {
-#pragma unroll
-    for (int c = 0; c < MAXCH; ++c) {
-        int e = (lane + 64 * c) * 4;
-        f32x4 z = {0.f, 0.f, 0.f, 0.f};
-        v[c] = (e < D) ? load4(p + e) : z;
-    }
-}
 
 template <int MAXCH>
 __device__ __forceinline__ void row_stats(const f32x4 (&v)[MAXCH], int D, int lane, float eps, float& mean, float& rstd) {
@@ -63,24 +55,8 @@
         load_row(x + row * D, MAXCH * 256, lane, v);
 #pragma unroll
         for (int c = 0; c < MAXCH; ++c) { gm[c] = load4(gamma + (lane + 64 * c) * 4); bt[c] = load4(beta + (lane + 64 * c) * 4); }
-        float s = 0.f;
-#pragma unroll
-        for (int c = 0; c < MAXCH; ++c) s += v[c][0] + v[c][1] + v[c][2] + v[c][3];
-        const float inv_d = 1.0f / (float)(MAXCH * 256);
-        const float mean = wave_sum(s) * inv_d;
-        float q = 0.f;
-#pragma unroll
-        for (int c = 0; c < MAXCH; ++c)
-#pragma unroll
-            for (int i = 0; i < 4; ++i) { const float d = v[c][i] - mean; q += d * d; }
-        const float rstd = rsqrtf(wave_sum(q) * inv_d + eps);
-#pragma unroll
-        for (int c = 0; c < MAXCH; ++c) {
-            f32x4 o;
-#pragma unroll
-            for (int i = 0; i < 4; ++i) o[i] = (v[c][i] - mean) * rstd * gm[c][i] + bt[c][i];
-            store4(y + row * D + (lane + 64 * c) * 4, o);
-        }
+        float mean, rstd;
+        cbln::fwd_row_full(v, gm, bt, eps, lane, y + row * D, mean, rstd);
         if (lane == 0) {
             if (mean_out) mean_out[row] = mean;
             if (rstd_out) rstd_out[row] = rstd;
@@ -248,75 +224,9 @@
                 mu[j] = 0.f; rs[j] = 0.f;
             }
         }
-        float s1[RPW], s2[RPW];
-#pragma unroll
-        for (int j = 0; j < RPW; ++j) {
-            s1[j] = 0.f; s2[j] = 0.f;
-#pragma unroll
-            for (int c = 0; c < MAXCH; ++c) {
-                const int e = (lane + 64 * c) * 4;
-                if (FULL || e < D) {
-#pragma unroll
-                    for (int i = 0; i < 4; ++i) {
-                        const float xh = (xv[j][c][i] - mu[j]) * rs[j];
-                        const float dgv = g[j][c][i] * gm[c][i];
-                        ag[c][i] += g[j][c][i] * xh;
-                        ab[c][i] += g[j][c][i];
-                        s1[j] += dgv; s2[j] += dgv * xh;
-                        xv[j][c][i] = xh; g[j][c][i] = dgv;
-                    }
-                }
-            }
-        }
-#pragma unroll
-        for (int o = 32; o > 0; o >>= 1) {
-#pragma unroll
-            for (int j = 0; j < RPW; ++j) { s1[j] += __shfl_xor(s1[j], o); s2[j] += __shfl_xor(s2[j], o); }
-        }
-#pragma unroll
-        for (int j = 0; j < RPW; ++j) {
-            if (!ok[j]) continue;
-            const float c1 = s1[j] * inv_d, c2 = s2[j] * inv_d;
-#pragma unroll
-            for (int c = 0; c < MAXCH; ++c) {
-                const int e = (lane + 64 * c) * 4;
-                if (FULL || e < D) {
-                    f32x4 o;
-#pragma unroll
-                    for (int i = 0; i < 4; ++i) o[i] = rs[j] * (g[j][c][i] - c1 - xv[j][c][i] * c2);
-                    store4(dx + row[j] * D + e, o);
-                    if (dx2) {
-                        o = o * dropout_mult4(seed, ((uint64_t)row[j] * D + e) >> 2, drop_p);
-                        store4(dx2 + row[j] * D + e, o);
-                    }
-                }
-            }
-        }
-    }
-#pragma unroll
-    for (int c0 = 0; c0 < MAXCH; c0 += GC) {
-        if (c0 * 256 >= D) break;
-        if (c0 > 0) __syncthreads();
-#pragma unroll
-        for (int c = 0; c < GC; ++c) {
-            if (c0 + c < MAXCH) {
-                *reinterpret_cast<f32x4*>(&red[0][wave][c * 256 + lane * 4]) = ag[c0 + c];
-                *reinterpret_cast<f32x4*>(&red[1][wave][c * 256 + lane * 4]) = ab[c0 + c];
-            }
-        }
-        __syncthreads();
-        for (int idx = threadIdx.x; idx < 2 * GC * 256; idx += NW * 64) {
-            const int kind = idx / (GC * 256), e = idx - kind * (GC * 256);
-            const int col = c0 * 256 + e;
-            if (col < D) {
-                float sacc = 0.f;
-#pragma unroll
-                for (int w = 0; w < NW; ++w) sacc += red[kind][w][e];
-                if (part) part[((int64_t)blockIdx.x * 2 + kind) * D + col] = sacc;
-                else atomicAdd((kind ? dbeta : dgamma) + col, sacc);
-            }
-        }
-    }
+        cbln::bwd_rows<T, MAXCH, RPW, FULL>(g, xv, mu, rs, ok, row, gm, ag, ab, lane, D, inv_d, dx, dx2, seed, drop_p);
+    }
+    cbln::colsum_flush<MAXCH, NW>(&red[0][0][0], ag, ab, threadIdx.x, D, part ? part + (int64_t)blockIdx.x * 2 * D : nullptr, dgamma, dbeta);
 }
 
 __global__ void __launch_bounds__(1024) ln_partials_reduce_kernel(const float* part, float* grad, const int64_t* off_gamma,
diff --git a/clipbert_amd/modeling/encoder.py b/clipbert_amd/modeling/encoder.py
--- a/clipbert_amd/modeling/encoder.py
+++ b/clipbert_amd/modeling/encoder.py
@@ -88,6 +88,19 @@
     if p_h > 0:
         ops.dropout(x, p_h, _seed(_SITE_EMB, 0, fwd_i), rt.seed_dev, out=x)
     layers = []
+    fuse_ln = "fwd" in rt.ln_rowop and dt == torch.bfloat16 and d == 768
+
+    def dense_ln(inp, lin, ln, k, res, site, li, out):
+        pre_ = torch.empty(M, d, dtype=dt, device=dev)
+        kw = dict(out=pre_, shift=lin.bias, residual=res, dropout_p=p_h, dropout_seed=_seed(site, li, fwd_i), seed_ptr=rt.seed_dev)
+        if not fuse_ln:
+            ops.gemm(inp, bank.compute(lin.weight), M, d, k, **kw)
+            return (pre_,) + ops.layernorm_fwd(pre_, ln.weight, ln.bias, eps, save_stats=save, out=out)
+        out = out if out is not None else torch.empty(M, d, dtype=dt, device=dev)
+        mean, rstd = torch.empty(2, M, dtype=torch.float32, device=dev) if save else (None, None)
+        ops.gemm(inp, bank.compute(lin.weight), M, d, k, **kw, ln_fwd=dict(gamma=ln.weight, beta=ln.bias, eps=eps, out=out, mean=mean, rstd=rstd))
+        return pre_, out, mean, rstd
+
     for li, layer in enumerate(model.encoder.layer):
         att, so, it, ou = layer.attention.self, layer.attention.output, layer.intermediate, layer.output
         wqkv = bank.compute_span(att.query.weight, att.value.weight, (3 * d, d))
@@ -96,20 +109,12 @@
         ops.gemm(x, wqkv, M, 3 * d, d, out=qkv, shift=bqkv)
         ctx, lse = ops.attention_fwd(qkv, key_mask, bsz, L, nh, save_lse=save, dropout_p=p_a,
                                      dropout_seed=_seed(_SITE_ATTN, li, fwd_i), seed_ptr=rt.seed_dev, out=stk.ctx[li] if save else None)
-        a_pre = torch.empty(M, d, dtype=dt, device=dev)
-        ops.gemm(ctx, bank.compute(so.dense.weight), M, d, d, out=a_pre, shift=so.dense.bias, residual=x, dropout_p=p_h,
-                 dropout_seed=_seed(_SITE_SELF_OUT, li, fwd_i), seed_ptr=rt.seed_dev)
-        a, mean1, rstd1 = ops.layernorm_fwd(a_pre, so.LayerNorm.weight, so.LayerNorm.bias, eps, save_stats=save,
-                                            out=stk.a[li] if save else None)
+        a_pre, a, mean1, rstd1 = dense_ln(ctx, so.dense, so.LayerNorm, d, x, _SITE_SELF_OUT, li, stk.a[li] if save else None)
         hact = stk.hact[li] if save else torch.empty(M, ff, dtype=dt, device=dev)
         hsave = torch.empty(M, ff, dtype=dt, device=dev) if save else None
         ops.gemm(a, bank.compute(it.dense.weight), M, ff, d, out=hact, shift=it.dense.bias,
                  act=ops.ACT_GELU_SAVE_GRAD if save else ACT_GELU, out2=hsave)
-        o_pre = torch.empty(M, d, dtype=dt, device=dev)
-        ops.gemm(hact, bank.compute(ou.dense.weight), M, d, ff, out=o_pre, shift=ou.dense.bias, residual=a, dropout_p=p_h,
-                 dropout_seed=_seed(_SITE_OUT, li, fwd_i), seed_ptr=rt.seed_dev)
-        out, mean2, rstd2 = ops.layernorm_fwd(o_pre, ou.LayerNorm.weight, ou.LayerNorm.bias, eps, save_stats=save,
-                                              out=stk.x[li + 1] if (save and li + 1 < nl) else None)
+        o_pre, out, mean2, rstd2 = dense_ln(hact, ou.dense, ou.LayerNorm, ff, a, _SITE_OUT, li, stk.x[li + 1] if (save and li + 1 < nl) else None)
         if save:
             layers.append(_LayerSaved(qkv, ctx, lse, a_pre, mean1, rstd1, hsave, o_pre, mean2, rstd2))
         x = out
@@ -248,12 +253,21 @@
     nl, stk = len(pk.layers), pk.stk
     ln_off = _ln_offsets(model, dev)
     nb = ops.ln_part_blocks(M)
-    ln_part = torch.empty(2 * nl, nb, 2, d, dtype=torch.float32, device=dev) if ln_off is not None else None
+    fuse_ln = "bwd" in rt.ln_rowop and dt == torch.bfloat16 and d == 768 and ln_off is not None
+    nfused = 2 * nl - 1 if fuse_ln else 0
+    part_f = torch.empty(nfused, ops.ln_part_rows(M), 2, d, dtype=torch.float32, device=dev) if fuse_ln else None
+    ln_part = torch.empty(2 * nl - nfused, nb, 2, d, dtype=torch.float32, device=dev) if ln_off is not None else None
+
+    def ln_rowop(slot, xpre, ln, mean, rstd, seed, g_out):
+        d_pre = torch.empty(M, d, dtype=dt, device=dev) if pk.p_h > 0 else g_out
+        arg = dict(gamma=ln.weight, x=xpre, mean=mean, rstd=rstd, dx=d_pre, dx2=g_out if pk.p_h > 0 else None, part=part_f[slot],
+                   dropout_p=pk.p_h, dropout_seed=seed, seed_ptr=rt.seed_dev)
+        return arg, d_pre, g_out
 
     def ln_bwd(slot, dy, xpre, ln, mean, rstd, seed, g_out):
         keep = dict(dx2=g_out) if pk.p_h > 0 else dict(dx=g_out)
         if ln_part is not None:
-            d_pre, d_drop = ops.layernorm_bwd_part(dy, xpre, ln.weight, mean, rstd, ln_part[slot], pk.p_h, seed, rt.seed_dev, **keep)
+            d_pre, d_drop = ops.layernorm_bwd_part(dy, xpre, ln.weight, mean, rstd, ln_part[slot - nfused], pk.p_h, seed, rt.seed_dev, **keep)
         else:
             d_pre, d_drop = ops.layernorm_bwd(dy, xpre, ln.weight, mean, rstd, bank.grad_image(ln.weight), bank.grad_image(ln.bias), pk.p_h,
                                               seed, rt.seed_dev, **keep)
@@ -261,26 +275,42 @@
 
     gs = SimpleNamespace(out=torch.empty(nl, M, d, dtype=dt, device=dev), hp=torch.empty(nl, M, ff, dtype=dt, device=dev),
                          att=torch.empty(nl, M, d, dtype=dt, device=dev), qkv=torch.empty(nl, M, 3 * d, dtype=dt, device=dev))
+    done2 = None
     for li in range(nl - 1, -1, -1):
         layer = model.encoder.layer[li]
         att, so, it, ou = layer.attention.self, layer.attention.output, layer.intermediate, layer.output
         sv = pk.layers[li]
-        d_o_pre, g = ln_bwd(2 * li + 1, dx, sv.o_pre, ou.LayerNorm, sv.mean2, sv.rstd2, _seed(_SITE_OUT, li, pk.fwd_i), gs.out[li])
+        if done2 is None:
+            d_o_pre, g = ln_bwd(2 * li + 1, dx, sv.o_pre, ou.LayerNorm, sv.mean2, sv.rstd2, _seed(_SITE_OUT, li, pk.fwd_i), gs.out[li])
+        else:
+            d_o_pre, g = done2
         dhp = gs.hp[li]
         ops.gemm(g, bank.compute(ou.dense.weight), M, ff, d, out=dhp, b_mode=KROW, gelu_grad_pre=sv.hsave,
                  act=ops.ACT_SAVED_GRAD)
         da = torch.empty(M, d, dtype=dt, device=dev)
-        ops.gemm(dhp, bank.compute(it.dense.weight), M, d, ff, out=da, b_mode=KROW, residual=d_o_pre)
-        d_a_pre, g = ln_bwd(2 * li, da, sv.a_pre, so.LayerNorm, sv.mean1, sv.rstd1, _seed(_SITE_SELF_OUT, li, pk.fwd_i), gs.att[li])
+        if fuse_ln:
+            arg, d_a_pre, g = ln_rowop(2 * li, sv.a_pre, so.LayerNorm, sv.mean1, sv.rstd1, _seed(_SITE_SELF_OUT, li, pk.fwd_i), gs.att[li])
+            ops.gemm(dhp, bank.compute(it.dense.weight), M, d, ff, out=da, b_mode=KROW, residual=d_o_pre, ln_bwd=arg)
+        else:
+            ops.gemm(dhp, bank.compute(it.dense.weight), M, d, ff, out=da, b_mode=KROW, residual=d_o_pre)
+            d_a_pre, g = ln_bwd(2 * li, da, sv.a_pre, so.LayerNorm, sv.mean1, sv.rstd1, _seed(_SITE_SELF_OUT, li, pk.fwd_i), gs.att[li])
         dctx = torch.empty(M, d, dtype=dt, device=dev)
         ops.gemm(g, bank.compute(so.dense.weight), M, d, d, out=dctx, b_mode=KROW)
         dqkv = ops.attention_bwd(sv.qkv, pk.key_mask, sv.ctx, dctx, sv.lse, bsz, L, nh, pk.p_a, _seed(_SITE_ATTN, li, pk.fwd_i), rt.seed_dev,
                                  out=gs.qkv[li])
         wqkv = bank.compute_span(att.query.weight, att.value.weight, (3 * d, d))
         dx = torch.empty(M, d, dtype=dt, device=dev)
-        ops.gemm(dqkv, wqkv, M, d, 3 * d, out=dx, b_mode=KROW, residual=d_a_pre)
+        if fuse_ln and li >= 1:
+            svp, lnp = pk.layers[li - 1], model.encoder.layer[li - 1].output.LayerNorm
+            arg, d_pre, g = ln_rowop(2 * li - 1, svp.o_pre, lnp, svp.mean2, svp.rstd2, _seed(_SITE_OUT, li - 1, pk.fwd_i), gs.out[li - 1])
+            ops.gemm(dqkv, wqkv, M, d, 3 * d, out=dx, b_mode=KROW, residual=d_a_pre, ln_bwd=arg)
+            done2 = (d_pre, g)
+        else:
+            ops.gemm(dqkv, wqkv, M, d, 3 * d, out=dx, b_mode=KROW, residual=d_a_pre)
+    if fuse_ln:
+        ops.ln_partials_reduce(part_f, bank.grad, ln_off[0][:nfused], ln_off[1][:nfused])
     if ln_part is not None:
-        ops.ln_partials_reduce(ln_part, bank.grad, ln_off[0], ln_off[1])
+        ops.ln_partials_reduce(ln_part, bank.grad, ln_off[0][nfused:], ln_off[1][nfused:])
     _encoder_wgrads(model, pk, gs, M)
     if pk.p_h > 0:
         dx = ops.dropout(dx, pk.p_h, _seed(_SITE_EMB, 0, pk.fwd_i), rt.seed_dev)
diff --git a/clipbert_amd/modeling/runtime.py b/clipbert_amd/modeling/runtime.py
--- a/clipbert_amd/modeling/runtime.py
+++ b/clipbert_amd/modeling/runtime.py
@@ -1,3 +1,4 @@
+import os
 from typing import Optional
 
 import torch
@@ -6,6 +7,8 @@
 from ..params import ParamBank
 
 _HOOK = {"encoder": "after_encoder_backward", "cnn": "after_res5_backward"}
+_LN_ROWOP_DEFAULT = "both"
+_LN_ROWOP = {"fwd": ("fwd",), "bwd": ("bwd",), "both": ("fwd", "bwd"), "none": ()}
 
 
 class Runtime:
@@ -23,6 +26,7 @@
         self.pending_cnn_nodes = 0
         self.prepare_args = None
         self._ln_off = None
+        self.ln_rowop = _LN_ROWOP[os.environ.get("CLIPBERT_LN_ROWOP", _LN_ROWOP_DEFAULT)]
         self.forward_count = 0
 
     def begin_step(self):
diff --git a/clipbert_amd/ops.py b/clipbert_amd/ops.py
--- a/clipbert_amd/ops.py
+++ b/clipbert_amd/ops.py
@@ -46,7 +46,8 @@
               sH=0, sW=0, flip_taps=False, c_rowmap=None, accumulate=False, split_k=1, act=ACT_NONE,
               scale=None, shift=None, residual=None, ldr=None, relu_after=False, mask=None, ldm=None,
               out2=None, ldc2=None, alpha=1.0, dropout_p=0.0, dropout_seed=0, seed_ptr=None, tile=0, gelu_grad_pre=None, a_rowsum=None, batch=1, batch_strides=None,
-              relu_bwd=False, post_scale=None, post_scale2=None, xcd_order=0, zero_fill_pitch=0, splitk_ws=None, schedule=0, sq_slots=None) -> GemmDesc:
+              relu_bwd=False, post_scale=None, post_scale2=None, xcd_order=0, zero_fill_pitch=0, splitk_ws=None, schedule=0, sq_slots=None,
+              ln_fwd=None, ln_bwd=None) -> GemmDesc:
     d = GemmDesc()
     d.dtype = dtype_code(a.dtype)
     assert b.dtype == a.dtype
@@ -108,7 +109,23 @@
     if sq_slots is not None:
         assert sq_slots.dtype == torch.float32 and sq_slots.is_contiguous()
         d.sq_slots, d.sq_slots_n = _ptr(sq_slots), sq_slots.numel()
-    d._refs = (a, b, out, a_tab, b_tab, c_rowmap, scale, shift, residual, mask, out2, seed_ptr, gelu_grad_pre, a_rowsum, post_scale,
+    ln_refs = ()
+    if ln_fwd is not None:
+        assert ln_bwd is None
+        d.row_op, d.ln_eps = _lib.ROWOP_LN_FWD, ln_fwd["eps"]
+        d.ln_gamma, d.ln_beta, d.ln_out = _ptr(ln_fwd["gamma"]), _ptr(ln_fwd["beta"]), _ptr(ln_fwd["out"])
+        d.ln_mean, d.ln_rstd = _ptr(ln_fwd.get("mean")), _ptr(ln_fwd.get("rstd"))
+        ln_refs = tuple(ln_fwd.values())
+    if ln_bwd is not None:
+        part = ln_bwd["part"]
+        assert part.dtype == torch.float32 and part.is_contiguous() and tuple(part.shape) == (ln_part_rows(M), 2, N)
+        d.row_op = _lib.ROWOP_LN_BWD
+        d.ln_gamma, d.ln_x, d.ln_mean, d.ln_rstd = _ptr(ln_bwd["gamma"]), _ptr(ln_bwd["x"]), _ptr(ln_bwd["mean"]), _ptr(ln_bwd["rstd"])
+        d.ln_out, d.ln_out2, d.ln_part = _ptr(ln_bwd["dx"]), _ptr(ln_bwd.get("dx2")), _ptr(part)
+        d.ln_dropout_p, d.ln_dropout_seed = ln_bwd.get("dropout_p", 0.0), ln_bwd.get("dropout_seed", 0)
+        d.ln_dropout_seed_ptr = _ptr(ln_bwd.get("seed_ptr"))
+        ln_refs = tuple(ln_bwd.values())
+    d._refs = ln_refs + (a, b, out, a_tab, b_tab, c_rowmap, scale, shift, residual, mask, out2, seed_ptr, gelu_grad_pre, a_rowsum, post_scale,
                post_scale2, splitk_ws, sq_slots)
     return d
 
@@ -124,6 +141,17 @@
     plan = (C.c_int32 * 4)()
     _chk(_lib.get().cb_gemm_plan(C.byref(d), 1 if use_table else 0, plan), "cb_gemm_plan")
     return tuple(plan)
+
+
+def gemm_plan_rowop(a: torch.Tensor, b: torch.Tensor, M: int, N: int, K: int, *, out: torch.Tensor, use_table: bool = True, **kw) -> bool:
+    d = gemm_desc(a, b, M, N, K, out=out, **kw)
+    plan = (C.c_int32 * 2)()
+    _chk(_lib.get().cb_gemm_plan_rowop(C.byref(d), 1 if use_table else 0, plan), "cb_gemm_plan_rowop")
+    return bool(plan[0])
+
+
+def ln_part_rows(rows: int) -> int:
+    return (rows + 63) // 64
 
 
 def gemm_group(descs, like: torch.Tensor):
diff --git a/include/clipbert_hip.h b/include/clipbert_hip.h
--- a/include/clipbert_hip.h
+++ b/include/clipbert_hip.h
@@ -10,6 +10,7 @@
 
 enum { CB_F32 = 0, CB_BF16 = 1 };
 enum { CB_SPLITK_WS_COUNTER_BYTES = 65536 };
+enum { CB_ROWOP_NONE = 0, CB_ROWOP_LN_FWD = 1, CB_ROWOP_LN_BWD = 2 };
 enum { CB_ACT_NONE = 0, CB_ACT_RELU = 1, CB_ACT_GELU = 2, CB_ACT_TANH = 3,
        CB_ACT_GELU_SAVE_GRAD = 4,
        CB_ACT_SAVED_GRAD = 5 };
@@ -67,10 +68,22 @@
     int64_t splitk_ws_bytes;
     float* sq_slots;
     int64_t sq_slots_n;
+    int32_t row_op;
+    float ln_eps;
+    const float* ln_gamma; const float* ln_beta;
+    void* ln_out; void* ln_out2;
+    float* ln_mean; float* ln_rstd;
+    const void* ln_x;
+    float* ln_part;
+    float ln_dropout_p;
+    int32_t ln_reserved;
+    uint64_t ln_dropout_seed;
+    const uint64_t* ln_dropout_seed_ptr;
 } cb_gemm_desc;
 
 int cb_gemm(const cb_gemm_desc* d, void* stream);
 int cb_gemm_plan(const cb_gemm_desc* d, int32_t use_table, int32_t* out4);
+int cb_gemm_plan_rowop(const cb_gemm_desc* d, int32_t use_table, int32_t* out2);
 int cb_gemm_workspace_bytes(const cb_gemm_desc* d, int64_t* bytes);
 int cb_gemm_group(const cb_gemm_desc* descs, int32_t n, void* stream);
 
```

New measurement: 3714 clips/s. 0.891x the previous value.
